# manoskary/analysisgnn

Hardware: AMD Instinct MI355X
Metric: subgraph-nodes/sec fwd+bwd, HybridGNN L=3 H=256 (higher is better)
Workload: dtype f32; 1 GPU; C2 (sampled, the batch a training step sees): HybridGNN L=3 H=256 out=128, 21 task heads, 32 neighbour-sampled subgraphs x (500 target notes + [5,5] hops) per GPU, per-hop counts passed (every layer trimmed); 16335 notes, 104099 edges per GPU; train step = fwd + objective (wloss) + bwd + allreduce + clip + AdamW, CSR rebuilt every step; hipGraph replay; workload_id=c2s, per_gpu_subgraphs=32, objective=wloss, parallelism=dp1, allreduce=none (one rank)

## Files before the change

### analysisgnn_amd/_lib.py

```python
from __future__ import annotations

import ctypes as C
import os
from typing import Optional, Sequence

import torch

from . import resident

_HERE = os.path.dirname(os.path.abspath(__file__))
LIB_PATH = os.path.join(_HERE, "libagnn_hip.so")
MAX_SEG = 32

SPMM_MEAN, SPMM_SKIP_SELF, SPMM_ACCUM = 1, 2, 4
INT32_MAX = 2 ** 31 - 1


class AgnnError(RuntimeError):
    pass


class CooSeg(C.Structure):
    _fields_ = [("row", C.c_void_p), ("col", C.c_void_p), ("etype", C.c_void_p),
                ("etype_code", C.c_int64), ("n_edges", C.c_int64), ("n_rows", C.c_int64)]


class RowendItem(C.Structure):
    _fields_ = [("rowptr", C.c_void_p), ("perm", C.c_void_p), ("rowend", C.c_void_p), ("n_rows", C.c_int32),
                ("e_limit", C.c_int32)]


ROWEND_MAX_ITEMS = 64


class Sampler(C.Structure):
    _fields_ = [("n_rel", C.c_int32), ("rowptr", C.c_void_p * 8), ("col", C.c_void_p * 8), ("win_start", C.c_void_p),
                ("n_sub", C.c_int32), ("n_targets", C.c_int32), ("n_hops", C.c_int32), ("fan", C.c_int32 * 4), ("cap", C.c_int32 * 4),
                ("rng", C.c_void_p), ("node_gid", C.c_void_p), ("edges", C.c_void_p * 8), ("e_cap", C.c_int64), ("status", C.c_void_p), ("drops", C.c_void_p), ("kept", C.c_void_p)]


class ReltItem(C.Structure):
    _fields_ = [("x", C.c_void_p), ("w", C.c_void_p), ("y", C.c_void_p), ("ld_x", C.c_int64), ("ld_y", C.c_int64)]


RELT_MAX_ITEMS = 4


class Rel(C.Structure):
    _fields_ = [("src", C.c_void_p), ("rowptr", C.c_void_p), ("rowend", C.c_void_p), ("col", C.c_void_p),
                ("ew", C.c_void_p), ("colscale", C.c_void_p), ("ld_src", C.c_int64)]


class HgtSrcItem(C.Structure):
    _fields_ = [("rowptr", C.c_void_p), ("rowend", C.c_void_p), ("col", C.c_void_p), ("perm", C.c_void_p), ("alpha", C.c_void_p),
                ("gs", C.c_void_p), ("dk", C.c_void_p), ("dv", C.c_void_p), ("ld_o", C.c_int64), ("n_src_rows", C.c_int32),
                ("col_limit", C.c_int32)]


class HgtDstItem(C.Structure):
    _fields_ = [("rels", C.c_void_p), ("n_rel", C.c_int32), ("q", C.c_void_p), ("ld_q", C.c_int64), ("n_rows", C.c_int64),
                ("out", C.c_void_p), ("ld_out", C.c_int64), ("m_out", C.c_void_p), ("linv_out", C.c_void_p)]


HGT_MAX_DST = 4


class HgtRel(C.Structure):
    _fields_ = [("k", C.c_void_p), ("v", C.c_void_p), ("rowptr", C.c_void_p), ("rowend", C.c_void_p),
                ("col", C.c_void_p), ("perm", C.c_void_p), ("pscale", C.c_void_p), ("ld", C.c_int64),
                ("alpha", C.c_void_p), ("gs", C.c_void_p), ("tdot", C.c_void_p), ("ld_tdot", C.c_int64)]


class Gated(C.Structure):
    _fields_ = [("rowptr", C.c_void_p), ("col", C.c_void_p), ("perm", C.c_void_p), ("a", C.c_void_p), ("b", C.c_void_p),
                ("h", C.c_void_p), ("c", C.c_void_p), ("ld", C.c_int64), ("ld_c", C.c_int64), ("n_rows", C.c_int64),
                ("H", C.c_int32)]


class WgradItem(C.Structure):
    _fields_ = [("dy", C.c_void_p), ("x", C.c_void_p), ("dw", C.c_void_p), ("db", C.c_void_p), ("ld_dy", C.c_int64), ("ld_x", C.c_int64),
                ("ld_dw", C.c_int64), ("n", C.c_int64), ("out_f", C.c_int32), ("in_f", C.c_int32)]


class ColsumItem(C.Structure):
    _fields_ = [("workspace", C.c_void_p), ("workspace_bytes", C.c_size_t), ("n", C.c_int64), ("H", C.c_int32), ("dgamma", C.c_void_p),
                ("dbeta", C.c_void_p)]


WGRAD_BATCH_MAX = 16
WGRAD_BATCH_MAX_ITEMS = 24
PACK_MAX_SRC = 8


class PackItem(C.Structure):
    _fields_ = [("dst", C.c_void_p), ("src", C.c_void_p * PACK_MAX_SRC), ("ld_dst", C.c_int64), ("ld_src", C.c_int64),
                ("rows", C.c_int32), ("cols", C.c_int32), ("n_src", C.c_int32), ("vec_ok", C.c_int32)]


LR_CONSTANT, LR_WARMUP_COSINE, LR_WARMUP_EXP = 0, 1, 2


class LrSchedule(C.Structure):
    _fields_ = [("kind", C.c_int32), ("warmup_steps", C.c_int32), ("count_offset", C.c_int32), ("swa_period", C.c_int32),
                ("swa_start", C.c_int64), ("swa_anneal", C.c_int32), ("base_lr", C.c_double), ("warmup_start_lr", C.c_double),
                ("eta_min", C.c_double), ("cos_a", C.c_double), ("cos_b", C.c_double), ("gamma", C.c_double),
                ("decay_steps", C.c_double), ("swa_lr", C.c_double)]


_lib: Optional[C.CDLL] = None

SIGNATURES = {
    "agnn_last_error": (C.c_char_p, []),
    "agnn_version": (C.c_int, []),
    "agnn_csr_workspace_bytes": (C.c_size_t, [C.c_int64, C.c_int64]),
    "agnn_csr_build": (C.c_int, [C.c_int, C.POINTER(CooSeg), C.c_void_p, C.c_void_p, C.c_void_p,
                                 C.c_void_p, C.c_size_t, C.c_void_p, C.c_void_p]),
    "agnn_check_status": (C.c_int, [C.c_void_p, C.c_void_p]),
    "agnn_csr_rowend": (C.c_int, [C.c_void_p, C.c_void_p, C.c_int64, C.c_int64, C.c_void_p, C.c_void_p]),
    "agnn_csr_rowend_batch": (C.c_int, [C.c_int, C.POINTER(RowendItem), C.c_void_p]),
    "agnn_spmm_f32": (C.c_int, [C.c_int, C.POINTER(Rel), C.c_int64, C.c_int32, C.c_void_p, C.c_int64,
                                C.c_int64, C.c_void_p, C.c_int64, C.c_void_p, C.c_int32, C.c_uint32,
                                C.c_void_p]),
    "agnn_spmm_root_f32": (C.c_int, [C.c_int, C.POINTER(Rel), C.c_int64, C.c_int32, C.c_void_p, C.c_int64,
                                     C.c_int64, C.c_void_p, C.c_int64, C.c_int64, C.c_void_p, C.c_int32, C.c_uint32,
                                     C.c_void_p]),
    "agnn_gru_fwd_f32": (C.c_int, [C.c_void_p, C.c_void_p, C.c_void_p, C.c_int64, C.c_int64, C.c_int32,
                                   C.c_void_p, C.c_void_p, C.c_void_p, C.c_void_p, C.c_void_p]),
    "agnn_gru_bwd_f32": (C.c_int, [C.c_void_p, C.c_void_p, C.c_void_p, C.c_void_p, C.c_int64, C.c_int64,
                                   C.c_int32, C.c_void_p, C.c_void_p, C.c_void_p, C.c_void_p, C.c_void_p]),
    "agnn_heads_fwd_f32": (C.c_int, [C.c_void_p, C.c_int64, C.c_int64, C.c_int32, C.c_int32, C.c_int32, C.c_void_p, C.c_void_p,
                                     C.c_void_p, C.c_void_p, C.c_float, C.c_void_p, C.c_void_p, C.c_void_p, C.POINTER(C.c_int32),
                                     C.c_void_p, C.c_void_p, C.c_int64, C.c_void_p, C.c_void_p, C.c_void_p, C.c_int64, C.c_void_p]),
    "agnn_gru_hprev_f32": (C.c_int, [C.c_void_p, C.c_int64, C.c_int64, C.c_int32, C.c_void_p, C.c_void_p]),
    "agnn_hgt_attn_fwd_multi_f32": (C.c_int, [C.c_int32, C.c_void_p, C.c_int32, C.c_int32, C.c_void_p]),
    "agnn_hgt_attn_fwd_f32": (C.c_int, [C.c_int, C.POINTER(HgtRel), C.c_void_p, C.c_int64, C.c_int64, C.c_int32,
                                        C.c_int32, C.c_void_p, C.c_int64, C.c_void_p, C.c_void_p, C.c_void_p]),
    "agnn_hgt_attn_bwd_dst_f32": (C.c_int, [C.c_int, C.POINTER(HgtRel), C.c_void_p, C.c_int64, C.c_void_p, C.c_int64,
                                            C.c_void_p, C.c_int64, C.c_void_p, C.c_void_p, C.c_int64, C.c_int32,
                                            C.c_int32, C.c_void_p, C.c_int64, C.c_void_p]),
    "agnn_hgt_attn_bwd_src_batch_f32": (C.c_int, [C.c_int32, C.POINTER(HgtSrcItem), C.c_void_p, C.c_int64, C.c_void_p, C.c_int64,
                                                  C.c_int32, C.c_int32, C.c_void_p]),
    "agnn_sampler_num_nodes": (C.c_int64, [C.POINTER(Sampler)]),
    "agnn_sampler_edge_capacity": (C.c_int64, [C.POINTER(Sampler)]),
    "agnn_sample_hops": (C.c_int, [C.POINTER(Sampler), C.c_void_p]),
    "agnn_sample_members": (C.c_int, [C.c_void_p, C.c_int64, C.c_void_p, C.c_void_p, C.c_void_p, C.c_int32, C.c_int32, C.c_int32,
                                      C.POINTER(C.c_int32), C.c_int32, C.c_void_p, C.c_void_p, C.c_void_p, C.c_void_p]),
    "agnn_sample_compact_nodes": (C.c_int64, [C.POINTER(Sampler), C.POINTER(C.c_int32)]),
    "agnn_sample_compact": (C.c_int, [C.POINTER(Sampler), C.POINTER(C.c_int32), C.c_void_p, C.c_void_p, C.c_void_p]),
    "agnn_gather_rows_f32": (C.c_int, [C.c_void_p, C.c_int64, C.c_void_p, C.c_int64, C.c_int32, C.c_void_p, C.c_int64, C.c_void_p]),
    "agnn_gather_i64": (C.c_int, [C.c_void_p, C.c_int64, C.c_void_p, C.c_int64, C.c_int32, C.c_int64, C.c_void_p, C.c_int64, C.c_void_p]),
    "agnn_relt_fwd_f32": (C.c_int, [C.c_int, C.POINTER(ReltItem), C.c_int32, C.c_int32, C.c_int32, C.c_int64, C.c_void_p]),
    "agnn_relt_bwd_f32": (C.c_int, [C.c_int, C.POINTER(ReltItem), C.c_int32, C.c_int32, C.c_int32, C.c_int64, C.c_void_p]),
    "agnn_relt_dw_workspace_bytes": (C.c_size_t, [C.c_int, C.c_int32, C.c_int32, C.c_int32, C.c_int64]),
    "agnn_relt_dw_f32": (C.c_int, [C.c_int, C.POINTER(ReltItem), C.c_int32, C.c_int32, C.c_int32, C.c_int64, C.c_void_p, C.c_size_t,
                                  C.c_void_p]),
    "agnn_wgrad_batch_workspace_bytes": (C.c_size_t, [C.c_int32, C.POINTER(WgradItem)]),
    "agnn_wgrad_batch_f32": (C.c_int, [C.c_int32, C.POINTER(WgradItem), C.c_void_p, C.c_size_t, C.c_void_p]),
    "agnn_gemm_nt_f32": (C.c_int, [C.c_void_p, C.c_int64, C.c_void_p, C.c_int64, C.c_void_p, C.c_int64, C.c_int32, C.c_int32, C.c_void_p,
                                   C.c_int64, C.c_void_p]),
    "agnn_gemm_nn_f32": (C.c_int, [C.c_void_p, C.c_int64, C.c_void_p, C.c_int64, C.c_void_p, C.c_int64, C.c_int32, C.c_int32, C.c_void_p,
                                   C.c_int64, C.c_void_p]),
    "agnn_gemm_nt2_f32": (C.c_int, [C.c_void_p, C.c_int64, C.c_int32, C.c_void_p, C.c_int64, C.c_int32, C.c_void_p, C.c_int64, C.c_void_p,
                                    C.c_int64, C.c_int32, C.c_void_p, C.c_int64, C.c_void_p]),
    "agnn_pool_cat_norm_f32": (C.c_int, [C.POINTER(Rel), C.c_void_p, C.c_int64, C.c_int64, C.c_int64, C.c_int32, C.c_int32, C.c_void_p,
                                         C.c_void_p, C.c_float, C.c_void_p, C.c_int64, C.c_void_p, C.c_int64, C.c_void_p, C.c_void_p,
                                         C.c_void_p, C.c_void_p]),
    "agnn_pool_cat_bwd_f32": (C.c_int, [C.POINTER(Rel), C.c_void_p, C.c_int64, C.c_void_p, C.c_int64, C.c_int64, C.c_int32, C.c_void_p,
                                        C.c_int64, C.c_void_p]),
    "agnn_absdiff_fwd_f32": (C.c_int, [C.c_void_p, C.c_void_p, C.c_void_p, C.c_int64, C.c_int64, C.c_int32, C.c_void_p, C.c_void_p, C.c_int64,
                                       C.c_void_p]),
    "agnn_absdiff_bwd_f32": (C.c_int, [C.c_void_p, C.c_void_p, C.c_void_p, C.c_int64, C.c_int64, C.c_int32, C.c_void_p, C.c_void_p, C.c_int64,
                                       C.c_int32, C.c_int32, C.c_void_p, C.c_int64, C.c_void_p]),
    "agnn_gated_fwd_f32": (C.c_int, [C.POINTER(Gated), C.c_void_p, C.c_int64, C.c_void_p]),
    "agnn_gated_bwd_dst_f32": (C.c_int, [C.POINTER(Gated), C.c_void_p, C.c_int64, C.c_void_p, C.c_void_p, C.c_void_p]),
    "agnn_gated_bwd_src_f32": (C.c_int, [C.POINTER(Gated), C.c_void_p, C.c_int64, C.c_void_p, C.c_void_p, C.c_void_p]),
    "agnn_norm_act_workspace_bytes": (C.c_size_t, [C.c_int32]),
    "agnn_norm_act_fwd_f32": (C.c_int, [C.c_void_p, C.c_int64, C.c_void_p, C.c_void_p, C.c_int32, C.c_int64, C.c_int32, C.c_float, C.c_float,
                                        C.c_uint32, C.c_void_p, C.c_uint32, C.c_void_p, C.c_int64, C.c_void_p, C.c_void_p, C.c_void_p,
                                        C.c_void_p]),
    "agnn_norm_act_bwd_f32": (C.c_int, [C.c_void_p, C.c_int64, C.c_void_p, C.c_void_p, C.c_int32, C.c_int64, C.c_int32, C.c_float, C.c_float,
                                        C.c_uint32, C.c_void_p, C.c_uint32, C.c_void_p, C.c_int64, C.c_void_p, C.c_void_p, C.c_void_p,
                                        C.c_int64, C.c_void_p, C.c_void_p, C.c_void_p, C.c_size_t, C.c_void_p]),
    "agnn_norm_act_colsum_batch_f32": (C.c_int, [C.c_int32, C.POINTER(ColsumItem), C.c_void_p]),
    "agnn_skip_act_workspace_bytes": (C.c_size_t, []),
    "agnn_skip_act_fwd_f32": (C.c_int, [C.c_void_p, C.c_int64, C.c_void_p, C.c_int64, C.c_void_p, C.c_int64, C.c_int32, C.c_float, C.c_uint32,
                                        C.c_void_p, C.c_uint32, C.c_void_p, C.c_int64, C.c_void_p, C.c_void_p]),
    "agnn_skip_act_bwd_f32": (C.c_int, [C.c_void_p, C.c_int64, C.c_void_p, C.c_int64, C.c_void_p, C.c_int64, C.c_int32, C.c_float, C.c_uint32,
                                        C.c_void_p, C.c_uint32, C.c_void_p, C.c_int64, C.c_void_p, C.c_int64, C.c_void_p, C.c_int64, C.c_void_p,
                                        C.c_void_p, C.c_size_t, C.c_void_p]),
    "agnn_norm_act_colsum_f32": (C.c_int, [C.c_void_p, C.c_size_t, C.c_int64, C.c_int32, C.c_void_p, C.c_void_p, C.c_void_p]),
    "agnn_wgrad_workspace_bytes": (C.c_size_t, [C.c_int64, C.c_int32, C.c_int32]),
    "agnn_wgrad_f32": (C.c_int, [C.c_void_p, C.c_int64, C.c_void_p, C.c_int64, C.c_int64, C.c_int32, C.c_int32, C.c_void_p,
                                 C.c_int64, C.c_void_p, C.c_void_p, C.c_size_t, C.c_void_p]),
    "agnn_pack_f32": (C.c_int, [C.c_int32, C.POINTER(PackItem), C.c_void_p]),
    "agnn_debug_stamp": (C.c_int, [C.c_void_p, C.c_void_p]),
    "agnn_gproj_fwd_f32": (C.c_int, [C.c_void_p, C.c_int64, C.c_void_p, C.c_void_p, C.c_void_p, C.c_int32, C.c_int32, C.c_int32,
                                     C.c_int64, C.c_void_p, C.c_int64, C.c_void_p]),
    "agnn_gproj_workspace_bytes": (C.c_size_t, [C.c_int64, C.c_int32, C.c_int32, C.c_int32]),
    "agnn_gproj_bwd_f32": (C.c_int, [C.c_void_p, C.c_int64, C.c_void_p, C.c_int64, C.c_void_p, C.c_void_p, C.c_int32, C.c_int32,
                                     C.c_int32, C.c_int32, C.c_int64, C.c_void_p, C.c_int64, C.c_void_p, C.c_void_p, C.c_void_p,
                                     C.c_size_t, C.c_void_p]),
    "agnn_spmm_self_grad_f32": (C.c_int, [C.c_void_p, C.c_int64, C.c_int64, C.c_int32, C.c_void_p, C.c_int64, C.c_int64, C.c_int32,
                                          C.c_void_p, C.c_int64, C.c_int32, C.c_void_p]),
    "agnn_embed_cat_fwd_f32": (C.c_int, [C.c_void_p, C.c_int64, C.c_int32, C.c_int64, C.c_int32, C.POINTER(C.c_void_p),
                                         C.POINTER(C.c_void_p), C.POINTER(C.c_int32), C.c_int32, C.c_void_p, C.c_int64, C.c_void_p]),
    "agnn_embed_workspace_bytes": (C.c_size_t, [C.c_int32, C.POINTER(C.c_int32), C.c_int32]),
    "agnn_embed_cat_bwd_f32": (C.c_int, [C.c_void_p, C.c_int64, C.c_int32, C.c_int64, C.c_int32, C.POINTER(C.c_void_p),
                                         C.POINTER(C.c_int32), C.c_int32, C.c_void_p, C.c_void_p, C.c_size_t, C.c_void_p]),
    "agnn_train_loss_workspace_bytes": (C.c_size_t, []),
    "agnn_train_loss_f32": (C.c_int, [C.c_void_p, C.c_int64, C.c_void_p, C.c_int32, C.c_void_p, C.c_int64, C.c_float, C.c_int64,
                                      C.c_void_p, C.c_int64, C.c_int32, C.c_float, C.c_void_p, C.c_float, C.c_void_p, C.c_void_p,
                                      C.c_void_p, C.c_void_p, C.c_void_p, C.c_void_p, C.c_void_p, C.c_void_p, C.c_size_t,
                                      C.c_void_p]),
    "agnn_train_loss_final_f32": (C.c_int, [C.c_void_p, C.c_int64, C.c_void_p, C.c_int32, C.c_void_p, C.c_int64, C.c_float, C.c_int64,
                                            C.c_void_p, C.c_int64, C.c_int32, C.c_float, C.c_void_p, C.c_float, C.c_void_p, C.c_void_p,
                                            C.c_void_p, C.c_void_p, C.c_void_p, C.c_void_p, C.c_void_p, C.c_void_p, C.c_int64, C.c_void_p,
                                            C.c_size_t, C.c_void_p]),
    "agnn_train_loss_bwd_f32": (C.c_int, [C.c_void_p, C.c_int64, C.c_void_p, C.c_int32, C.c_int64, C.c_int32, C.c_void_p, C.c_void_p,
                                          C.c_void_p, C.c_int64, C.c_void_p, C.c_int64, C.c_int32, C.c_float, C.c_void_p, C.c_int64,
                                          C.c_void_p]),
    "agnn_adamw_workspace_bytes": (C.c_size_t, []),
    "agnn_adamw_f32": (C.c_int, [C.c_void_p, C.c_void_p, C.c_void_p, C.c_void_p, C.c_int64, C.c_float, C.c_float, C.c_float,
                                 C.c_float, C.c_float, C.c_float, C.c_void_p, C.c_void_p, C.c_int32, C.c_void_p, C.c_size_t,
                                 C.c_void_p]),
    "agnn_lr_schedule_at": (C.c_double, [C.POINTER(LrSchedule), C.c_int64]),
    "agnn_adamw_sched_workspace_bytes": (C.c_size_t, []),
    "agnn_adamw_sched_f32": (C.c_int, [C.c_void_p, C.c_void_p, C.c_void_p, C.c_void_p, C.c_int64, C.POINTER(LrSchedule), C.c_float,
                                       C.c_float, C.c_float, C.c_float, C.c_float, C.c_void_p, C.c_void_p, C.c_void_p, C.c_void_p,
                                       C.c_int32, C.c_void_p, C.c_size_t, C.c_void_p]),
    "agnn_multitask_ce_f32": (C.c_int, [C.c_void_p, C.c_int64, C.c_void_p, C.c_int32, C.c_void_p, C.c_int64, C.c_float,
                                        C.c_int64, C.c_void_p, C.c_void_p, C.c_void_p, C.c_void_p, C.c_void_p]),
    "agnn_multitask_ce_scale_f32": (C.c_int, [C.c_void_p, C.c_int64, C.c_void_p, C.c_int32, C.c_int64, C.c_int32, C.c_void_p,
                                              C.c_void_p, C.c_int64, C.c_void_p]),
    "agnn_kd_workspace_bytes": (C.c_size_t, [C.c_int64, C.c_int32]),
    "agnn_multitask_kd_f32": (C.c_int, [C.c_void_p, C.c_int64, C.c_void_p, C.c_int64, C.c_void_p, C.c_void_p, C.c_int32, C.c_int64,
                                        C.c_int32, C.c_float, C.c_float, C.c_void_p, C.c_int64, C.c_void_p, C.c_void_p, C.c_void_p,
                                        C.c_size_t, C.c_void_p]),
    "agnn_ewc_workspace_bytes": (C.c_size_t, []),
    "agnn_ewc_f32": (C.c_int, [C.c_void_p, C.c_void_p, C.c_void_p, C.c_int64, C.c_float, C.c_void_p, C.c_void_p, C.c_void_p,
                               C.c_size_t, C.c_void_p]),
    "agnn_fisher_accum_f32": (C.c_int, [C.c_void_p, C.c_int64, C.c_float, C.c_void_p, C.c_void_p]),
    "agnn_eval_counts_len": (C.c_size_t, [C.c_int32, C.c_int32]),
    "agnn_multitask_eval_f32": (C.c_int, [C.c_void_p, C.c_int64, C.c_void_p, C.c_void_p, C.c_int32, C.c_int32, C.c_void_p, C.c_int64,
                                          C.c_int64, C.c_void_p, C.c_int32, C.c_uint32, C.c_void_p, C.c_void_p, C.c_void_p]),
}


def load() -> C.CDLL:
    global _lib
    if _lib is not None:
        return _lib
    if not os.path.exists(LIB_PATH):
        raise AgnnError(
            f"{LIB_PATH} not found: build it with `python -c 'import __graft_entry__ as g; g.build()'` "
            "(or `make -C analysisgnn_amd/csrc`). analysisgnn_amd has no CPU fallback.")
    lib = C.CDLL(LIB_PATH)
    for name, (res, args) in SIGNATURES.items():
        fn = getattr(lib, name)
        fn.restype = res
        fn.argtypes = args
    _lib = lib
    return lib


def check(rc: int, what: str) -> None:
    if rc != 0:
        msg = load().agnn_last_error()
        raise AgnnError(f"{what} failed ({rc}): {msg.decode() if msg else ''}")


def require_gpu(*tensors: Optional[torch.Tensor]) -> torch.device:
    dev = None
    for t in tensors:
        if t is None:
            continue
        if not t.is_cuda:
            raise AgnnError("analysisgnn_amd ops need tensors on a HIP device (no CPU fallback); "
                            f"got a tensor on {t.device}")
        if dev is None:
            dev = t.device
        elif t.device != dev:
            raise AgnnError(f"tensors on different devices: {dev} vs {t.device}")
    if dev is None:
        raise AgnnError("no tensor given")
    return dev


def status_word(device: torch.device) -> torch.Tensor:
    return resident.value(device, ("status word",), lambda: torch.zeros(1, dtype=torch.int32, device=device))


def check_device_status(device: torch.device) -> None:
    check(load().agnn_check_status(status_word(device).data_ptr(), stream_ptr(device)), "agnn_check_status")


def stream_ptr(device: torch.device) -> int:
    return torch.cuda.current_stream(device).cuda_stream


def ptr(t: Optional[torch.Tensor]) -> Optional[int]:
    return None if t is None else t.data_ptr()


def f32c(t: torch.Tensor) -> torch.Tensor:
    if t.dtype != torch.float32:
        raise AgnnError(f"fp32 expected, got {t.dtype}")
    if t.dim() != 2:
        raise AgnnError(f"2-D feature matrix expected, got shape {tuple(t.shape)}")
    if t.stride(1) != 1 or t.stride(0) % 4 != 0 or t.data_ptr() % 16 != 0 or (t.shape[0] > 1 and t.stride(0) < t.shape[1]):
        t = t.contiguous()
    return t


def make_rels(items: Sequence[dict]):
    arr = (Rel * len(items))()
    for i, it in enumerate(items):
        arr[i].src = it["src"]
        arr[i].rowptr = it["rowptr"]
        arr[i].rowend = it.get("rowend")
        arr[i].col = it["col"]
        arr[i].ew = it.get("ew")
        arr[i].colscale = it.get("colscale")
        arr[i].ld_src = it["ld_src"]
    return arr


STAMPS = {"on": bool(os.environ.get("AGNN_STAMPS")), "names": [], "buf": None,
          "only": [w for w in os.environ.get("AGNN_STAMPS", "").split(",") if w not in ("", "1", "all")]}


def stamp(name: str, device) -> None:
    if not STAMPS["on"] or (STAMPS["only"] and not any(w in name for w in STAMPS["only"])):
        return
    if STAMPS["buf"] is None:
        STAMPS["buf"] = torch.zeros(256, dtype=torch.int64, device=device)
    if name not in STAMPS["names"]:
        STAMPS["names"].append(name)
    k = STAMPS["names"].index(name)
    check(load().agnn_debug_stamp(STAMPS["buf"].data_ptr() + 8 * k, stream_ptr(torch.device(device))), "agnn_debug_stamp")
```

### analysisgnn_amd/csrc/pack.hip

```cpp
#include "agnn_common.h"

namespace {

struct PackTable {
  agnn_pack_item_t it[AGNN_PACK_MAX_ITEMS];
  int32_t first_block[AGNN_PACK_MAX_ITEMS + 1];
  int32_t n;
};

constexpr int kElemsPerBlock = 4096;

__global__ __launch_bounds__(256) void k_pack(PackTable t) {
  int i = 0;
  while (i + 1 < t.n && static_cast<int>(blockIdx.x) >= t.first_block[i + 1]) ++i;
  const agnn_pack_item_t& it = t.it[i];
  const int64_t total = static_cast<int64_t>(it.rows) * it.cols;
  const int64_t base = static_cast<int64_t>(blockIdx.x - t.first_block[i]) * kElemsPerBlock;
  const bool vec = (it.cols & 3) == 0 && it.vec_ok;
  if (vec) {
    const int c4 = it.cols >> 2;
#pragma unroll
    for (int u = 0; u < kElemsPerBlock / 1024; ++u) {
      const int64_t e = (base >> 2) + u * 256 + threadIdx.x;
      if (e >= (total >> 2)) break;
      const int64_t r = static_cast<uint32_t>(e) / static_cast<uint32_t>(c4);
      const int c = static_cast<int>(e - r * c4) * 4;
      float4 s = make_float4(0.f, 0.f, 0.f, 0.f);
      if (it.n_src > 0) s = *reinterpret_cast<const float4*>(it.src[0] + r * it.ld_src + c);
      for (int k = 1; k < it.n_src; ++k) {
        const float4 v = *reinterpret_cast<const float4*>(it.src[k] + r * it.ld_src + c);
        s.x += v.x; s.y += v.y; s.z += v.z; s.w += v.w;
      }
      *reinterpret_cast<float4*>(it.dst + r * it.ld_dst + c) = s;
    }
  } else {
#pragma unroll 4
    for (int u = 0; u < kElemsPerBlock / 256; ++u) {
      const int64_t e = base + u * 256 + threadIdx.x;
      if (e >= total) break;
      const int64_t r = static_cast<uint32_t>(e) / static_cast<uint32_t>(it.cols);
      const int c = static_cast<int>(e - r * it.cols);
      float s = it.n_src > 0 ? it.src[0][r * it.ld_src + c] : 0.f;
      for (int k = 1; k < it.n_src; ++k) s += it.src[k][r * it.ld_src + c];
      it.dst[r * it.ld_dst + c] = s;
    }
  }
}

}

extern "C" int agnn_pack_f32(int32_t n_items, const agnn_pack_item_t* items, agnn_stream_t stream_) {
  using namespace agnn;
  if (n_items < 0) return fail(AGNN_EINVAL, "pack: negative item count");
  if (n_items > 0 && !items) return fail(AGNN_EINVAL, "pack: null item table");
  hipStream_t s = static_cast<hipStream_t>(stream_);
  for (int32_t at = 0; at < n_items; at += AGNN_PACK_MAX_ITEMS) {
    PackTable t;
    t.n = 0;
    int32_t blocks = 0;
    for (int32_t i = at; i < n_items && t.n < AGNN_PACK_MAX_ITEMS; ++i) {
      agnn_pack_item_t it = items[i];
      if (it.rows < 0 || it.cols < 0 || it.n_src < 0 || it.n_src > AGNN_PACK_MAX_SRC)
        return fail(AGNN_EINVAL, "pack: item %d has rows=%d cols=%d n_src=%d", i, it.rows, it.cols, it.n_src);
      if (it.rows == 0 || it.cols == 0) continue;
      if (static_cast<int64_t>(it.rows) * it.cols >= (int64_t{1} << 31)) return fail(AGNN_EINVAL, "pack: item %d has 2^31 or more elements", i);
      if (!it.dst || it.ld_dst < it.cols || (it.n_src > 0 && it.ld_src < it.cols)) return fail(AGNN_EINVAL, "pack: item %d: null dst or ld < cols", i);
      if (it.n_src == 0) it.ld_src = it.ld_dst;
      bool v = aligned16(it.dst) && (it.ld_dst & 3) == 0 && (it.ld_src & 3) == 0;
      for (int k = 0; k < it.n_src; ++k) {
        if (!it.src[k]) return fail(AGNN_EINVAL, "pack: item %d: null source %d", i, k);
        v = v && aligned16(it.src[k]);
      }
      it.vec_ok = v ? 1 : 0;
      t.first_block[t.n] = blocks;
      const int64_t total = static_cast<int64_t>(it.rows) * it.cols;
      blocks += static_cast<int32_t>((total + kElemsPerBlock - 1) / kElemsPerBlock);
      t.it[t.n++] = it;
    }
    if (t.n == 0) continue;
    t.first_block[t.n] = blocks;
    hipLaunchKernelGGL(k_pack, dim3(blocks), dim3(256), 0, s, t);
    if (int rc = check_launch("pack")) return rc;
  }
  return AGNN_OK;
}

namespace {
__global__ void k_stamp(unsigned long long* slot) { *slot = wall_clock64(); }
}

extern "C" int agnn_debug_stamp(uint64_t* slot, agnn_stream_t stream_) {
  using namespace agnn;
  if (!slot) return fail(AGNN_EINVAL, "debug_stamp: null slot");
  hipLaunchKernelGGL(k_stamp, dim3(1), dim3(1), 0, static_cast<hipStream_t>(stream_), reinterpret_cast<unsigned long long*>(slot));
  return check_launch("debug_stamp");
}
```

### analysisgnn_amd/csrc/wgrad.hip

```cpp
#include "agnn_common.h"

namespace {

typedef float f32x16 __attribute__((ext_vector_type(16)));

struct WgArgs {
  const float* dy;
  const float* x;
  int64_t ld_dy, ld_x;
  int32_t n, out_f, in_f;
  int32_t rows_per_slice;
  int32_t tiles_in;
  float* slab;
  float* slab_b;
  int32_t out_pad, in_pad;
};

__device__ __forceinline__ void wgrad_tile(const WgArgs& a, const int tile, const int slice) {
  const int lane = threadIdx.x & 63;
  const int wave = threadIdx.x >> 6;
  const int wm = wave >> 1, wn = wave & 1;
  const int to = tile / a.tiles_in, ti = tile - to * a.tiles_in;
  const int kk = lane >> 5, c32 = lane & 31;
  const int ocol = to * 128 + wm * 64 + 2 * c32;
  const int icol = ti * 128 + wn * 64 + 2 * c32;
  const bool o_ok = ocol < a.out_f;
  const bool i_ok = icol < a.in_f;
  const int r0 = slice * a.rows_per_slice;
  int r1 = r0 + a.rows_per_slice;
  if (r1 > a.n) r1 = a.n;

  f32x16 acc00 = {0}, acc01 = {0}, acc10 = {0}, acc11 = {0};
  float bs0 = 0.f, bs1 = 0.f;
  const float* dy_s = a.dy + static_cast<int64_t>(r0) * a.ld_dy;
  const float* x_s = a.x + static_cast<int64_t>(r0) * a.ld_x;
  const uint32_t ldb_dy = static_cast<uint32_t>(a.ld_dy) * 4u, ldb_x = static_cast<uint32_t>(a.ld_x) * 4u;
  const uint32_t cb_dy = (o_ok ? ocol : 0) * 4u, cb_x = (i_ok ? icol : 0) * 4u;
  const int rel_last = a.n - 1 - r0;
  constexpr int CH = 8;
  constexpr int STEP = 2 * CH;
  float2 a0[CH], b0[CH], a1[CH], b1[CH], a2[CH], b2[CH];
  uint32_t o_dy = static_cast<uint32_t>(kk) * ldb_dy + cb_dy, o_x = static_cast<uint32_t>(kk) * ldb_x + cb_x;
  const uint32_t s_dy = 2u * ldb_dy, s_x = 2u * ldb_x;
  auto fetch_fast = [&](float2* ao, float2* bo) {
#pragma unroll
    for (int u = 0; u < CH; ++u) {
      ao[u] = *reinterpret_cast<const float2*>(reinterpret_cast<const char*>(dy_s) + o_dy);
      bo[u] = *reinterpret_cast<const float2*>(reinterpret_cast<const char*>(x_s) + o_x);
      o_dy += s_dy;
      o_x += s_x;
    }
    __builtin_amdgcn_sched_barrier(0);
  };
  auto fetch = [&](int chunk, float2* ao, float2* bo) {
#pragma unroll
    for (int u = 0; u < CH; ++u) {
      const uint32_t rel = static_cast<uint32_t>(min(chunk * STEP + 2 * u + kk, rel_last));
      ao[u] = *reinterpret_cast<const float2*>(reinterpret_cast<const char*>(dy_s) + (rel * ldb_dy + cb_dy));
      bo[u] = *reinterpret_cast<const float2*>(reinterpret_cast<const char*>(x_s) + (rel * ldb_x + cb_x));
    }
    o_dy += CH * s_dy;
    o_x += CH * s_x;
    __builtin_amdgcn_sched_barrier(0);
  };
  auto mma = [&](const float2* av, const float2* bv) {
#pragma unroll
    for (int u = 0; u < CH; ++u) {
      acc00 = __builtin_amdgcn_mfma_f32_32x32x2f32(av[u].x, bv[u].x, acc00, 0, 0, 0);
      acc01 = __builtin_amdgcn_mfma_f32_32x32x2f32(av[u].x, bv[u].y, acc01, 0, 0, 0);
      acc10 = __builtin_amdgcn_mfma_f32_32x32x2f32(av[u].y, bv[u].x, acc10, 0, 0, 0);
      acc11 = __builtin_amdgcn_mfma_f32_32x32x2f32(av[u].y, bv[u].y, acc11, 0, 0, 0);
      asm volatile("v_add_f32 %0, %0, %1" : "+v"(bs0) : "v"(av[u].x));
      asm volatile("v_add_f32 %0, %0, %1" : "+v"(bs1) : "v"(av[u].y));
    }
  };
  auto mma_tail = [&](int chunk, const float2* av, const float2* bv) {
#pragma unroll
    for (int u = 0; u < CH; ++u) {
      const float m = (r0 + chunk * STEP + 2 * u + kk < r1) ? 1.f : 0.f;
      const float ax = av[u].x * m, ay = av[u].y * m;
      acc00 = __builtin_amdgcn_mfma_f32_32x32x2f32(ax, bv[u].x, acc00, 0, 0, 0);
      acc01 = __builtin_amdgcn_mfma_f32_32x32x2f32(ax, bv[u].y, acc01, 0, 0, 0);
      acc10 = __builtin_amdgcn_mfma_f32_32x32x2f32(ay, bv[u].x, acc10, 0, 0, 0);
      acc11 = __builtin_amdgcn_mfma_f32_32x32x2f32(ay, bv[u].y, acc11, 0, 0, 0);
      bs0 += ax;
      bs1 += ay;
    }
  };
  const int nfull = (r1 - r0) / STEP;
  const int nchunks = (r1 - r0 + STEP - 1) / STEP;
  fetch(0, a0, b0);
  fetch(1, a1, b1);
  int c = 0;
  const int safe = (rel_last + 1) / STEP;
  for (; c + 3 <= nfull && c + 5 <= safe; c += 3) {
    fetch_fast(a2, b2);
    mma(a0, b0);
    fetch_fast(a0, b0);
    mma(a1, b1);
    fetch_fast(a1, b1);
    mma(a2, b2);
  }
  for (; c + 3 <= nfull; c += 3) {
    fetch(c + 2, a2, b2);
    mma(a0, b0);
    fetch(c + 3, a0, b0);
    mma(a1, b1);
    fetch(c + 4, a1, b1);
    mma(a2, b2);
  }
  fetch(c + 2, a2, b2);
  if (c < nchunks) mma_tail(c, a0, b0);
  if (c + 1 < nchunks) mma_tail(c + 1, a1, b1);
  if (c + 2 < nchunks) mma_tail(c + 2, a2, b2);
  float* slab = a.slab + (static_cast<int64_t>(slice) * a.out_pad) * a.in_pad;
  const int ob = to * 128 + wm * 64, ib = ti * 128 + wn * 64;
#pragma unroll
  for (int r = 0; r < 16; ++r) {
    const int i = (r & 3) + 8 * (r >> 2) + 4 * kk;
    float* row0 = slab + static_cast<int64_t>(ob + 2 * i) * a.in_pad + ib + 2 * c32;
    float* row1 = row0 + a.in_pad;
    *reinterpret_cast<float2*>(row0) = make_float2(acc00[r], acc01[r]);
    *reinterpret_cast<float2*>(row1) = make_float2(acc10[r], acc11[r]);
  }
  if (a.slab_b != nullptr && wn == 0) {
    bs0 += __shfl_xor(bs0, 32, 64);
    bs1 += __shfl_xor(bs1, 32, 64);
    if (kk == 0 && ti == 0)
      *reinterpret_cast<float2*>(a.slab_b + static_cast<int64_t>(slice) * a.out_pad + ocol) = make_float2(bs0, bs1);
  }
}

__global__ __launch_bounds__(256) void k_wgrad(WgArgs a) { wgrad_tile(a, blockIdx.x, blockIdx.y); }

constexpr int kWgBatchMax = 24;

struct WgBatch {
  WgArgs it[kWgBatchMax];
  int32_t first[kWgBatchMax + 1];
  int32_t tiles[kWgBatchMax];
  int32_t n;
};

__global__ __launch_bounds__(256) void k_wgrad_batch(WgBatch b) {
  int i = 0;
  const int blk = blockIdx.x;
  while (i + 1 < b.n && blk >= b.first[i + 1]) ++i;
  const int local = blk - b.first[i];
  const int tiles = b.tiles[i];
  const int slice = local / tiles;
  wgrad_tile(b.it[i], local - slice * tiles, slice);
}


__device__ __forceinline__ void wgrad_reduce_blocks(const float* __restrict__ slab, const float* __restrict__ slab_b, int S, int out_f, int in_f,
                                                    int out_pad, int in_pad, float* __restrict__ dw, int64_t ld_dw, float* __restrict__ db,
                                                    const int block, const int n_blocks) {
  __shared__ float2 part[8][32];
  const int col = threadIdx.x & 31, sg = threadIdx.x >> 5;
  const int half_in = in_f >> 1;
  const int64_t total = static_cast<int64_t>(out_f) * half_in;
  const int64_t plane = static_cast<int64_t>(out_pad) * in_pad;
  for (int64_t e0 = static_cast<int64_t>(block) * 32; e0 < total; e0 += static_cast<int64_t>(n_blocks) * 32) {
    const int64_t e = e0 + col;
    float2 s = make_float2(0.f, 0.f);
    int o = 0, i = 0;
    if (e < total) {
      o = static_cast<int>(e / half_in);
      i = static_cast<int>(e - static_cast<int64_t>(o) * half_in) * 2;
      const float* p = slab + static_cast<int64_t>(o) * in_pad + i;
      for (int k = sg; k < S; k += 8) {
        const float2 v = *reinterpret_cast<const float2*>(p + k * plane);
        s.x += v.x;
        s.y += v.y;
      }
    }
    part[sg][col] = s;
    __syncthreads();
    if (sg == 0 && e < total) {
      float2 t = part[0][col];
#pragma unroll
      for (int g = 1; g < 8; ++g) { t.x += part[g][col].x; t.y += part[g][col].y; }
      *reinterpret_cast<float2*>(dw + static_cast<int64_t>(o) * ld_dw + i) = t;
    }
    __syncthreads();
  }
  if (db != nullptr) {
    __shared__ float partb[8][32];
    for (int e0 = block * 32; e0 < out_f; e0 += n_blocks * 32) {
      const int e = e0 + col;
      float s = 0.f;
      if (e < out_f)
        for (int k = sg; k < S; k += 8) s += slab_b[static_cast<int64_t>(k) * out_pad + e];
      partb[sg][col] = s;
      __syncthreads();
      if (sg == 0 && e < out_f) {
        float t = partb[0][col];
#pragma unroll
        for (int g = 1; g < 8; ++g) t += partb[g][col];
        db[e] = t;
      }
      __syncthreads();
    }
  }
}

__global__ __launch_bounds__(256) void k_wgrad_reduce(const float* __restrict__ slab, const float* __restrict__ slab_b, int S,
                                                      int out_f, int in_f, int out_pad, int in_pad, float* __restrict__ dw,
                                                      int64_t ld_dw, float* __restrict__ db) {
  wgrad_reduce_blocks(slab, slab_b, S, out_f, in_f, out_pad, in_pad, dw, ld_dw, db, blockIdx.x, gridDim.x);
}

struct RedItem {
  const float* slab;
  const float* slab_b;
  float* dw;
  float* db;
  int64_t ld_dw;
  int32_t S, out_f, in_f, out_pad, in_pad;
};
struct RedBatch {
  RedItem it[kWgBatchMax];
  int32_t first[kWgBatchMax + 1];
  int32_t n;
};

__global__ __launch_bounds__(256) void k_wgrad_reduce_batch(RedBatch b) {
  int i = 0;
  const int blk = blockIdx.x;
  while (i + 1 < b.n && blk >= b.first[i + 1]) ++i;
  const RedItem& r = b.it[i];
  wgrad_reduce_blocks(r.slab, r.slab_b, r.S, r.out_f, r.in_f, r.out_pad, r.in_pad, r.dw, r.ld_dw, r.db, blk - b.first[i], b.first[i + 1] - b.first[i]);
}

struct Plan {
  int tiles_out, tiles_in, S, rows_per_slice, out_pad, in_pad;
};

Plan make_plan(int64_t n, int out_f, int in_f) {
  Plan p;
  p.tiles_out = (out_f + 127) / 128;
  p.tiles_in = (in_f + 127) / 128;
  p.out_pad = p.tiles_out * 128;
  p.in_pad = p.tiles_in * 128;
  const int tiles = p.tiles_out * p.tiles_in;
  int64_t S = 512 / tiles;
  const int64_t max_s = (n + 63) / 64;
  if (S > max_s) S = max_s;
  if (S > 64) S = 64;
  if (S < 1) S = 1;
  int64_t rps = (n + S - 1) / S;
  rps = (rps + 1) & ~int64_t{1};
  p.rows_per_slice = static_cast<int>(rps);
  p.S = static_cast<int>((n + rps - 1) / rps);
  return p;
}

}

int agnn::launch_slab_reduce(const float* slab, const float* slab_b, int S, int out_f, int in_f, int out_pad, int in_pad,
                             float* dw, int64_t ld_dw, float* db, hipStream_t s) {
  const int64_t total = static_cast<int64_t>(out_f) * (in_f >> 1);
  int blocks = static_cast<int>((total + 31) / 32);
  if (blocks > 4096) blocks = 4096;
  if (blocks < 1) blocks = 1;
  hipLaunchKernelGGL(k_wgrad_reduce, dim3(blocks), dim3(256), 0, s, slab, slab_b, S, out_f, in_f, out_pad, in_pad, dw, ld_dw, db);
  return check_launch("slab_reduce");
}

extern "C" size_t agnn_wgrad_workspace_bytes(int64_t n, int32_t out_f, int32_t in_f) {
  if (n <= 0 || out_f <= 0 || in_f <= 0) return 0;
  const Plan p = make_plan(n, out_f, in_f);
  return (static_cast<size_t>(p.S) * p.out_pad * p.in_pad + static_cast<size_t>(p.S) * p.out_pad) * sizeof(float) + 256;
}

extern "C" int agnn_wgrad_f32(const float* dy, int64_t ld_dy, const float* x, int64_t ld_x, int64_t n, int32_t out_f,
                              int32_t in_f, float* dw, int64_t ld_dw, float* db, void* workspace, size_t workspace_bytes,
                              agnn_stream_t stream_) {
  using namespace agnn;
  if (n <= 0 || n >= (int64_t{1} << 31) || out_f <= 0 || in_f <= 0) return fail(AGNN_EINVAL, "wgrad: bad sizes n=%lld out=%d in=%d", (long long)n, out_f, in_f);
  if ((out_f & 1) || (in_f & 1) || (ld_dy & 1) || (ld_x & 1) || (ld_dw & 1)) return fail(AGNN_EALIGN, "wgrad: widths and leading dimensions must be even");
  if (!dy || !x || !dw || !workspace) return fail(AGNN_EINVAL, "wgrad: null argument");
  if ((reinterpret_cast<uintptr_t>(dy) | reinterpret_cast<uintptr_t>(x) | reinterpret_cast<uintptr_t>(dw) | reinterpret_cast<uintptr_t>(db)) & 7u)
    return fail(AGNN_EALIGN, "wgrad: pointers must be 8-byte aligned");
  if (ld_dy < out_f || ld_x < in_f || ld_dw < in_f) return fail(AGNN_EINVAL, "wgrad: leading dimension smaller than the width");
  const size_t need = agnn_wgrad_workspace_bytes(n, out_f, in_f);
  if (workspace_bytes < need) return fail(AGNN_ENOMEM, "wgrad: workspace %zu < %zu bytes", workspace_bytes, need);
  const Plan p = make_plan(n, out_f, in_f);
  if ((static_cast<int64_t>(p.rows_per_slice) + 128) * (ld_dy > ld_x ? ld_dy : ld_x) * 4 >= (int64_t{1} << 32))
    return fail(AGNN_EINVAL, "wgrad: a row slice (%d rows x ld) exceeds the kernel's 32-bit byte offsets", p.rows_per_slice);
  char* ws = reinterpret_cast<char*>((reinterpret_cast<uintptr_t>(workspace) + 255) & ~uintptr_t{255});
  float* slab = reinterpret_cast<float*>(ws);
  float* slab_b = slab + static_cast<size_t>(p.S) * p.out_pad * p.in_pad;
  WgArgs a{dy, x, ld_dy, ld_x, static_cast<int32_t>(n), out_f, in_f, p.rows_per_slice, p.tiles_in, slab,
           db ? slab_b : nullptr, p.out_pad, p.in_pad};
  hipStream_t s = static_cast<hipStream_t>(stream_);
  hipLaunchKernelGGL(k_wgrad, dim3(p.tiles_out * p.tiles_in, p.S), dim3(256), 0, s, a);
  if (int rc = check_launch("wgrad")) return rc;
  return launch_slab_reduce(slab, db ? slab_b : nullptr, p.S, out_f, in_f, p.out_pad, p.in_pad, dw, ld_dw, db, s);
}

namespace {
struct BatchPlan {
  int n;
  int tiles_out[kWgBatchMax], tiles_in[kWgBatchMax], S[kWgBatchMax], rps[kWgBatchMax];
  size_t slab_off[kWgBatchMax], slabb_off[kWgBatchMax], total_floats;
};

int batch_plan(int n_items, const agnn_wgrad_item_t* items, BatchPlan& bp) {
  using namespace agnn;
  if (n_items <= 0 || n_items > kWgBatchMax || !items) return fail(AGNN_EINVAL, "wgrad_batch: %d items (1 .. %d)", n_items, kWgBatchMax);
  bp.n = n_items;
  int64_t tiles = 0;
  for (int i = 0; i < n_items; ++i) {
    const agnn_wgrad_item_t& it = items[i];
    if (it.n <= 0 || it.n >= (int64_t{1} << 31) || it.out_f <= 0 || it.in_f <= 0) return fail(AGNN_EINVAL, "wgrad_batch: item %d: bad sizes", i);
    bp.tiles_out[i] = (it.out_f + 127) / 128;
    bp.tiles_in[i] = (it.in_f + 127) / 128;
    tiles += static_cast<int64_t>(bp.tiles_out[i]) * bp.tiles_in[i];
  }
  int64_t S = 384 / tiles;
  if (S > 64) S = 64;
  if (S < 1) S = 1;
  size_t off = 0;
  for (int i = 0; i < n_items; ++i) {
    const agnn_wgrad_item_t& it = items[i];
    int64_t s_i = S;
    const int64_t max_s = (it.n + 63) / 64;
    if (s_i > max_s) s_i = max_s;
    int64_t rps = (it.n + s_i - 1) / s_i;
    rps = (rps + 1) & ~int64_t{1};
    bp.rps[i] = static_cast<int>(rps);
    bp.S[i] = static_cast<int>((it.n + rps - 1) / rps);
    const size_t plane = static_cast<size_t>(bp.tiles_out[i]) * 128 * bp.tiles_in[i] * 128;
    bp.slab_off[i] = off;
    off += static_cast<size_t>(bp.S[i]) * plane;
    bp.slabb_off[i] = off;
    off += static_cast<size_t>(bp.S[i]) * bp.tiles_out[i] * 128;
    off = (off + 63) & ~size_t{63};
  }
  bp.total_floats = off;
  return AGNN_OK;
}
}

extern "C" size_t agnn_wgrad_batch_workspace_bytes(int32_t n_items, const agnn_wgrad_item_t* items) {
  BatchPlan bp;
  if (batch_plan(n_items, items, bp) != AGNN_OK) return 0;
  return bp.total_floats * sizeof(float) + 256;
}

extern "C" int agnn_wgrad_batch_f32(int32_t n_items, const agnn_wgrad_item_t* items, void* workspace, size_t workspace_bytes,
                                    agnn_stream_t stream_) {
  using namespace agnn;
  BatchPlan bp;
  if (int rc = batch_plan(n_items, items, bp)) return rc;
  if (!workspace || workspace_bytes < bp.total_floats * sizeof(float) + 256) return fail(AGNN_ENOMEM, "wgrad_batch: workspace too small");
  float* ws = reinterpret_cast<float*>((reinterpret_cast<uintptr_t>(workspace) + 255) & ~uintptr_t{255});
  WgBatch wb{};
  RedBatch rb{};
  wb.n = rb.n = n_items;
  int wg = 0, red = 0;
  for (int i = 0; i < n_items; ++i) {
    const agnn_wgrad_item_t& it = items[i];
    if ((it.out_f & 1) || (it.in_f & 1) || (it.ld_dy & 1) || (it.ld_x & 1) || (it.ld_dw & 1)) return fail(AGNN_EALIGN, "wgrad_batch: item %d: widths and leading dimensions must be even", i);
    if (!it.dy || !it.x || !it.dw) return fail(AGNN_EINVAL, "wgrad_batch: item %d: null argument", i);
    if ((reinterpret_cast<uintptr_t>(it.dy) | reinterpret_cast<uintptr_t>(it.x) | reinterpret_cast<uintptr_t>(it.dw) | reinterpret_cast<uintptr_t>(it.db)) & 7u)
      return fail(AGNN_EALIGN, "wgrad_batch: item %d: pointers must be 8-byte aligned", i);
    if (it.ld_dy < it.out_f || it.ld_x < it.in_f || it.ld_dw < it.in_f) return fail(AGNN_EINVAL, "wgrad_batch: item %d: leading dimension smaller than the width", i);
    if ((static_cast<int64_t>(bp.rps[i]) + 128) * (it.ld_dy > it.ld_x ? it.ld_dy : it.ld_x) * 4 >= (int64_t{1} << 32))
      return fail(AGNN_EINVAL, "wgrad_batch: item %d: a row slice (%d rows x ld) exceeds the kernel's 32-bit byte offsets", i, bp.rps[i]);
    const int out_pad = bp.tiles_out[i] * 128, in_pad = bp.tiles_in[i] * 128;
    float* slab = ws + bp.slab_off[i];
    float* slab_b = ws + bp.slabb_off[i];
    wb.it[i] = WgArgs{it.dy, it.x, it.ld_dy, it.ld_x, static_cast<int32_t>(it.n), it.out_f, it.in_f, bp.rps[i], bp.tiles_in[i], slab,
                      it.db ? slab_b : nullptr, out_pad, in_pad};
    wb.tiles[i] = bp.tiles_out[i] * bp.tiles_in[i];
    wb.first[i] = wg;
    wg += wb.tiles[i] * bp.S[i];
    rb.it[i] = RedItem{slab, it.db ? slab_b : nullptr, it.dw, it.db, it.ld_dw, bp.S[i], it.out_f, it.in_f, out_pad, in_pad};
    rb.first[i] = red;
    int64_t blocks = (static_cast<int64_t>(it.out_f) * (it.in_f >> 1) + 31) / 32;
    if (blocks > 1024) blocks = 1024;
    red += static_cast<int>(blocks);
  }
  wb.first[n_items] = wg;
  rb.first[n_items] = red;
  hipStream_t s = static_cast<hipStream_t>(stream_);
  hipLaunchKernelGGL(k_wgrad_batch, dim3(static_cast<unsigned>(wg)), dim3(256), 0, s, wb);
  if (int rc = check_launch("wgrad_batch")) return rc;
  hipLaunchKernelGGL(k_wgrad_reduce_batch, dim3(static_cast<unsigned>(red)), dim3(256), 0, s, rb);
  return check_launch("wgrad_batch(reduce)");
}
```

### analysisgnn_amd/dp.py

```python
from __future__ import annotations

import os
from typing import Iterable, List, Optional, Sequence

import torch
import torch.distributed as dist


def init_distributed(backend: Optional[str] = None) -> tuple:
    world = int(os.environ.get("WORLD_SIZE", "1"))
    rank = int(os.environ.get("RANK", "0"))
    local = int(os.environ.get("LOCAL_RANK", "0"))
    if world > 1 and not dist.is_initialized():
        os.environ.setdefault("MASTER_ADDR", "127.0.0.1")
        os.environ.setdefault("MASTER_PORT", "29500")
        if backend is None:
            backend = os.environ.get("AGNN_DIST_BACKEND") or ("nccl" if torch.cuda.is_available() else "gloo")
        if backend == "nccl":
            torch.cuda.set_device(local)
            dist.init_process_group(backend, rank=rank, world_size=world, device_id=torch.device("cuda", local))
        else:
            dist.init_process_group(backend, rank=rank, world_size=world)
    return rank, local, world


def shard_units(n_units: int, rank: int, world: int) -> List[int]:
    return list(range(rank, n_units, world))


def _aligned_offsets(sizes: Sequence[int], align: int = 4, tight: Optional[Sequence[bool]] = None) -> List[int]:
    offs, end = [], 0
    for i, k in enumerate(sizes):
        start = end if (tight is not None and tight[i] and i > 0) else (end + align - 1) // align * align
        offs.append(start)
        end = start + k
    offs.append((end + align - 1) // align * align)
    return offs


def plan_parameters(model: torch.nn.Module, late: Iterable[torch.nn.Parameter] = ()):
    groups = []
    for m in model.modules():
        fn = getattr(m, "adjacent_parameter_groups", None)
        if fn is not None:
            groups.extend([[p for p in g] for g in fn()])
    late_ids = {id(p) for p in late}
    seen, params, tight = set(), [], set()
    for g in groups:
        if any(id(p) in late_ids for p in g):
            raise ValueError("plan_parameters: an adjacency group cannot hold late parameters")
        g = [p for p in g if p.requires_grad and id(p) not in seen]
        for i, p in enumerate(g):
            seen.add(id(p))
            params.append(p)
            if i > 0:
                tight.add(id(p))
    for want_late in (False, True):
        for p in model.parameters():
            if p.requires_grad and id(p) not in seen and (id(p) in late_ids) == want_late:
                seen.add(id(p))
                params.append(p)
    return params, tight


class FlatGradBuffer:

    def __init__(self, params: Iterable[torch.nn.Parameter], views: bool = True, tight: Optional[set] = None,
                 late: Iterable[torch.nn.Parameter] = ()):
        self.params: List[torch.nn.Parameter] = [p for p in params if p.requires_grad]
        if not self.params:
            raise ValueError("no trainable parameters")
        dev = self.params[0].device
        self.sizes = [p.numel() for p in self.params]
        self.offsets = _aligned_offsets(self.sizes, tight=[tight is not None and id(p) in tight for p in self.params])
        n = self.offsets[-1]
        self.views = views
        for p in self.params:
            if p.dtype != torch.float32 or p.device != dev:
                raise ValueError("FlatGradBuffer: fp32 parameters on one device expected")
        self.flat = torch.zeros(n, dtype=torch.float32, device=dev)
        self._pad = torch.zeros(4, dtype=torch.float32, device=dev)
        self._none = torch.zeros(max(self.sizes) if self.sizes else 1, dtype=torch.float32, device=dev)
        late_ids = {id(p) for p in late}
        self.n_early = len(self.params)
        if late_ids:
            flags = [id(p) in late_ids for p in self.params]
            self.n_early = flags.index(True) if True in flags else len(flags)
            if not all(flags[self.n_early:]) or sum(flags) != len(late_ids):
                raise ValueError("FlatGradBuffer: the late parameters must be the last ones of the buffer (dp.plan_parameters(model, late=...))")
        self.cut = self.offsets[self.n_early]
        if views:
            self._assign_views()

    def _assign_views(self) -> None:
        for p, k, o in zip(self.params, self.sizes, self.offsets):
            p.grad = self.flat[o:o + k].view_as(p)

    def zero(self) -> None:
        if self.views:
            self.flat.zero_()
        else:
            for p in self.params:
                p.grad = None
            self._packed = set()

    def pack(self, part: Optional[str] = None) -> None:
        from .linear import join_wgrad
        join_wgrad()
        if self.views:
            return
        done = getattr(self, "_packed", set())
        if not isinstance(done, set):
            done = {"early", "late"} if done else set()
        for name, lo, hi in (("early", 0, self.n_early), ("late", self.n_early, len(self.params))):
            if (part is not None and part != name) or name in done or lo == hi:
                done.add(name) if lo == hi else None
                continue
            parts = []
            for i in range(lo, hi):
                p, k, o, o_next = self.params[i], self.sizes[i], self.offsets[i], self.offsets[i + 1]
                parts.append(p.grad.reshape(-1) if p.grad is not None else self._none[:k])
                if o_next - o > k:
                    parts.append(self._pad[: o_next - o - k])
            torch.cat(parts, out=self.flat[self.offsets[lo]:self.offsets[hi]])
            for i in range(lo, hi):
                p, k, o = self.params[i], self.sizes[i], self.offsets[i]
                p.grad = self.flat[o:o + k].view_as(p)
            done.add(name)
        self._packed = done

    def all_reduce_mean(self, world: Optional[int] = None) -> None:
        self.pack()
        if dist.is_initialized() and dist.get_world_size() > 1:
            dist.all_reduce(self.flat, op=dist.ReduceOp.SUM)
            self.flat.div_(dist.get_world_size())

    def all_reduce_early_async(self):
        self.pack("early")
        if dist.is_initialized() and dist.get_world_size() > 1 and self.cut > 0:
            return dist.all_reduce(self.flat[:self.cut], op=dist.ReduceOp.SUM, async_op=True)
        return None

    def all_reduce_late_and_finish(self, work) -> None:
        self.pack("late")
        if dist.is_initialized() and dist.get_world_size() > 1:
            if self.cut < self.flat.numel():
                dist.all_reduce(self.flat[self.cut:], op=dist.ReduceOp.SUM)
            if work is not None:
                work.wait()
            self.flat.div_(dist.get_world_size())

    def clip_norm_(self, max_norm: float) -> torch.Tensor:
        total = torch.linalg.vector_norm(self.flat)
        self.flat.mul_(torch.clamp(max_norm / (total + 1e-6), max=1.0))
        return total


class LRSchedule:
    FIELDS = ("kind", "warmup_steps", "count_offset", "base_lr", "warmup_start_lr", "eta_min", "cos_a", "cos_b", "gamma", "decay_steps")

    def __init__(self, kind: int, base_lr: float, warmup_steps: int = 0, count_offset: int = 0, warmup_start_lr: float = 0.0,
                 eta_min: float = 0.0, cos_a: float = 0.0, cos_b: float = 1.0, gamma: float = 1.0, decay_steps: float = 1.0):
        self.kind, self.warmup_steps, self.count_offset = int(kind), int(warmup_steps), int(count_offset)
        self.base_lr, self.warmup_start_lr, self.eta_min = float(base_lr), float(warmup_start_lr), float(eta_min)
        self.cos_a, self.cos_b, self.gamma, self.decay_steps = float(cos_a), float(cos_b), float(gamma), float(decay_steps)
        self.lr_at(0)

    @classmethod
    def constant(cls, lr: float) -> "LRSchedule":
        from . import _lib
        return cls(_lib.LR_CONSTANT, lr)

    @classmethod
    def warmup_cosine(cls, base_lr: float, warmup_steps: int, total_steps: int, eta_min: float = 0.0) -> "LRSchedule":
        from . import _lib
        return cls(_lib.LR_WARMUP_COSINE, base_lr, warmup_steps, 0, 0.0, eta_min, cos_a=warmup_steps, cos_b=total_steps)

    @classmethod
    def reference_cosine(cls, base_lr: float, warmup_steps: int, max_epochs: int, eta_min: float = 0.0,
                         warmup_start_lr: float = 0.0) -> "LRSchedule":
        from . import _lib
        if warmup_steps < 3:
            raise ValueError(f"reference_cosine: warmup_steps={warmup_steps}: the reference's class fails for warm-ups shorter than 3 "
                             "steps (it reads steps_per_epoch before its third step() call has set it)")
        return cls(_lib.LR_WARMUP_COSINE, base_lr, warmup_steps, 1, warmup_start_lr, eta_min, cos_a=warmup_steps / 3.0, cos_b=max_epochs)

    @classmethod
    def reference_exponential(cls, base_lr: float, warmup_steps: int, decay_steps: int, gamma: float = 0.999, eta_min: float = 0.0,
                              warmup_start_lr: float = 0.0) -> "LRSchedule":
        from . import _lib
        return cls(_lib.LR_WARMUP_EXP, base_lr, warmup_steps, 1, warmup_start_lr, eta_min, gamma=gamma, decay_steps=decay_steps)

    def to_dict(self) -> dict:
        return {k: getattr(self, k) for k in self.FIELDS}

    @classmethod
    def from_dict(cls, d: dict) -> "LRSchedule":
        return cls(**{k: d[k] for k in cls.FIELDS})

    def struct(self, swa: Optional["SWA"] = None):
        from . import _lib
        s = _lib.LrSchedule(**self.to_dict())
        s.swa_start, s.swa_period, s.swa_anneal, s.swa_lr = -1, 1, 0, 0.0
        if swa is not None:
            s.swa_start, s.swa_period, s.swa_anneal, s.swa_lr = swa.start_step, swa.period, swa.anneal_epochs, swa.swa_lr
        return s

    def lr_at(self, k: int, swa: Optional["SWA"] = None) -> float:
        import ctypes
        import math
        from . import _lib
        lib = _lib.load()
        lr = float(lib.agnn_lr_schedule_at(ctypes.byref(self.struct(swa)), int(k)))
        if math.isnan(lr):
            raise _lib.AgnnError(f"agnn_lr_schedule_at failed: {(lib.agnn_last_error() or b'').decode()}")
        return lr


class SWA:

    def __init__(self, start_step: int, period: int, anneal_epochs: int = 10, swa_lr: float = 5e-5):
        if start_step < 0 or period <= 0 or anneal_epochs < 0:
            raise ValueError(f"SWA: start_step={start_step}, period={period}, anneal_epochs={anneal_epochs}")
        self.start_step, self.period, self.anneal_epochs, self.swa_lr = int(start_step), int(period), int(anneal_epochs), float(swa_lr)

    def to_dict(self) -> dict:
        return dict(start_step=self.start_step, period=self.period, anneal_epochs=self.anneal_epochs, swa_lr=self.swa_lr)


class FlatAdamW:

    def __init__(self, params: Iterable[torch.nn.Parameter], grads: FlatGradBuffer, lr=1e-3, betas=(0.9, 0.999),
                 eps=1e-8, weight_decay=1e-2, swa: Optional[SWA] = None):
        self.params = [p for p in params if p.requires_grad]
        assert [id(p) for p in self.params] == [id(p) for p in grads.params], "same parameter order as the gradient buffer"
        self.grads = grads
        self.lr, self.betas, self.eps, self.wd = lr, betas, eps, weight_decay
        dev = self.params[0].device
        self.flat = torch.zeros(grads.offsets[-1], dtype=torch.float32, device=dev)
        for p, o in zip(self.params, grads.offsets):
            self.flat[o:o + p.numel()] = p.detach().reshape(-1)
            p.data = self.flat[o:o + p.numel()].view_as(p)
        self.m = torch.zeros_like(self.flat)
        self.v = torch.zeros_like(self.flat)
        self.schedule = lr if isinstance(lr, LRSchedule) else None
        self.swa = swa
        if self.schedule is None:
            if swa is not None:
                raise ValueError("FlatAdamW: swa needs lr=LRSchedule (LRSchedule.constant(lr) for a fixed rate)")
            return
        self._sched = self.schedule.struct(swa)
        self._t = torch.zeros((), dtype=torch.float32, device=dev)
        self._state = torch.zeros(2, dtype=torch.float32, device=dev)
        self._state[0] = self.schedule.lr_at(0, swa)
        self.last_norm = torch.zeros((), dtype=torch.float32, device=dev)
        self.swa_flat = torch.zeros_like(self.flat) if swa is not None else None
        if self.flat.is_cuda:
            from . import _lib
            self._ws = torch.empty(int(_lib.load().agnn_adamw_sched_workspace_bytes()), dtype=torch.uint8, device=dev)

    @property
    def last_lr(self) -> torch.Tensor:
        return self._scheduled("last_lr")._state[0]

    @property
    def n_averaged(self) -> torch.Tensor:
        return self._scheduled("n_averaged")._state[1]

    def current_lr(self) -> float:
        if self.schedule is None:
            return float(self.lr)
        return self.schedule.lr_at(int(self._t.item()), self.swa)

    def _scheduled(self, what: str) -> "FlatAdamW":
        if self.schedule is None:
            raise AttributeError(f"FlatAdamW.{what} needs lr=LRSchedule")
        return self

    @torch.no_grad()
    def swap_swa_(self) -> None:
        if self.swa is None:
            raise AttributeError("FlatAdamW.swap_swa_ needs swa=SWA(...)")
# ... 123 lines not shown
```

### analysisgnn_amd/fused.py

```python
from __future__ import annotations

import itertools
from typing import Optional

import torch
import torch.nn as nn
import torch.nn.functional as F

from . import _lib, resident
from .linear import ColsumItem, all_steal, defer, deferring, leaf_refs

PRE_RELU, POST_RELU = 1, 2
ENABLED = True
_CALL_IDS = itertools.count(1)


def rng_state(device) -> torch.Tensor:
    return resident.value(device, ("dropout counter",), lambda: torch.tensor([int(torch.initial_seed()) & 0x7FFFFFFFFFFFFFFF, 0],
                                                                             dtype=torch.int64, device=device))


def advance_rng(device) -> None:
    rng_state(device)[1:2].add_(1)


def _al16(t: torch.Tensor) -> torch.Tensor:
    return t if t.data_ptr() % 16 == 0 else t.clone()


class _NormAct(torch.autograd.Function):
    @staticmethod
    def forward(ctx, x, gamma, beta, eps, p, flags, call_id, seg=0, defer_ok=False, steal_refs=None, pre=None):
        dev = _lib.require_gpu(x, gamma, beta)
        ctx.defer_ok = bool(defer_ok) or (gamma.is_leaf and beta.is_leaf)
        ctx.steal_refs = leaf_refs(gamma, beta) if steal_refs is None else tuple(steal_refs)
        lib = _lib.load()
        x = x if (x.stride(1) == 1 and x.stride(0) % 4 == 0 and x.data_ptr() % 16 == 0) else x.contiguous()
        n, H = x.shape
        seg = int(seg) if seg else H
        rng = rng_state(dev) if p > 0 else None
        used = torch.empty(2, dtype=torch.int64, device=dev) if p > 0 else None
        gamma, beta = _al16(gamma.contiguous()), _al16(beta.contiguous())
        if pre is not None:
            y, mean, rstd = pre
        else:
            y = torch.empty((n, H), dtype=torch.float32, device=dev)
            mean = torch.empty((max(n, 1) * (H // seg),), dtype=torch.float32, device=dev)
            rstd = torch.empty((max(n, 1) * (H // seg),), dtype=torch.float32, device=dev)
            _lib.check(lib.agnn_norm_act_fwd_f32(x.data_ptr(), x.stride(0), gamma.data_ptr(), beta.data_ptr(), seg, n, H, float(eps), float(p),
                                                 int(flags), _lib.ptr(rng), int(call_id), y.data_ptr(), y.stride(0), mean.data_ptr(),
                                                 rstd.data_ptr(), _lib.ptr(used), _lib.stream_ptr(dev)), "agnn_norm_act_fwd_f32")
        ctx.save_for_backward(x, gamma, beta, mean, rstd, *([used] if used is not None else []))
        ctx.cfg = (float(eps), float(p), int(flags), int(call_id), seg)
        return y

    @staticmethod
    def backward(ctx, dy):
        x, gamma, beta, mean, rstd, *used = ctx.saved_tensors
        eps, p, flags, call_id, seg = ctx.cfg
        dev = dy.device
        lib = _lib.load()
        dy = dy if (dy.stride(1) == 1 and dy.stride(0) % 4 == 0 and dy.data_ptr() % 16 == 0) else dy.contiguous()
        n, H = x.shape
        dx = torch.empty_like(x)
        dgamma = torch.empty_like(gamma)
        dbeta = torch.empty_like(beta)
        nws = int(lib.agnn_norm_act_workspace_bytes(H))
        ws = torch.empty(nws, dtype=torch.uint8, device=dev)
        rng = used[0] if p > 0 else None
        later = ctx.defer_ok and deferring(dy) and all_steal(ctx.steal_refs)
        _lib.check(lib.agnn_norm_act_bwd_f32(x.data_ptr(), x.stride(0), gamma.data_ptr(), beta.data_ptr(), seg, n, H, eps, p, flags,
                                             _lib.ptr(rng), call_id, dy.data_ptr(), dy.stride(0), mean.data_ptr(), rstd.data_ptr(),
                                             dx.data_ptr(), dx.stride(0), None if later else dgamma.data_ptr(),
                                             None if later else dbeta.data_ptr(), ws.data_ptr(), nws, _lib.stream_ptr(dev)),
                   "agnn_norm_act_bwd_f32")
        if later:
            dg_k, db_k = dgamma.detach(), dbeta.detach()
            defer(ColsumItem(ws, n, H, dg_k, db_k), dev)
        return dx, dgamma, dbeta, None, None, None, None, None, None, None, None


def _ok16(t: torch.Tensor) -> bool:
    return t.dtype == torch.float32 and t.dim() == 2 and t.stride(1) == 1 and t.stride(0) % 4 == 0 and t.data_ptr() % 16 == 0


class _SkipAct(torch.autograd.Function):

    @staticmethod
    def forward(ctx, o, x, skip, relu: bool, p: float, call_id: int):
        dev = _lib.require_gpu(o)
        lib = _lib.load()
        o = o if _ok16(o) else o.float().contiguous()
        if x is not None:
            x = x if _ok16(x) else x.float().contiguous()
        n, H = o.shape
        z = torch.empty((n, H), dtype=torch.float32, device=dev)
        rng = rng_state(dev) if p > 0 else None
        used = torch.empty(2, dtype=torch.int64, device=dev) if p > 0 else None
        sk = skip.detach().reshape(-1)[:1].contiguous() if skip is not None else None
        flags = 1 if relu else 0
        _lib.check(lib.agnn_skip_act_fwd_f32(_lib.ptr(x), x.stride(0) if x is not None else 0, o.data_ptr(), o.stride(0), _lib.ptr(sk), n, H,
                                             float(p), flags, _lib.ptr(rng), int(call_id), z.data_ptr(), z.stride(0), _lib.ptr(used),
                                             _lib.stream_ptr(dev)), "agnn_skip_act_fwd_f32")
        ctx.save_for_backward(o, *([x, sk] if x is not None else []), *([used] if used is not None else []))
        ctx.cfg = (bool(relu), float(p), int(call_id), x is not None, tuple(skip.shape) if skip is not None else None)
        ctx.set_materialize_grads(False)
        return z

    @staticmethod
    def backward(ctx, dz):
        if dz is None:
            return None, None, None, None, None, None
        relu, p, call_id, has_x, skip_shape = ctx.cfg
        saved = list(ctx.saved_tensors)
        o = saved.pop(0)
        x, sk = (saved.pop(0), saved.pop(0)) if has_x else (None, None)
        used = saved.pop(0) if p > 0 else None
        dev = dz.device
        lib = _lib.load()
        dz = dz if _ok16(dz) else dz.float().contiguous()
        n, H = o.shape
        do = torch.empty_like(o)
        want_dx = has_x and ctx.needs_input_grad[1]
        want_ds = has_x and ctx.needs_input_grad[2]
        dx = torch.empty((n, H), dtype=torch.float32, device=dev) if want_dx else None
        ds = torch.empty(1, dtype=torch.float32, device=dev) if want_ds else None
        ws = resident.scratch(dev, "skip_act", int(lib.agnn_skip_act_workspace_bytes()), zeroed=True) if want_ds else None
        _lib.check(lib.agnn_skip_act_bwd_f32(_lib.ptr(x), x.stride(0) if has_x else 0, o.data_ptr(), o.stride(0), _lib.ptr(sk), n, H, p,
                                             1 if relu else 0, _lib.ptr(used), call_id, dz.data_ptr(), dz.stride(0), _lib.ptr(dx),
                                             dx.stride(0) if dx is not None else 0, do.data_ptr(), do.stride(0), _lib.ptr(ds), _lib.ptr(ws),
                                             int(lib.agnn_skip_act_workspace_bytes()) if ws is not None else 0, _lib.stream_ptr(dev)),
                   "agnn_skip_act_bwd_f32")
        return do, dx, (ds.reshape(skip_shape) if ds is not None else None), None, None, None


def skip_act(o: torch.Tensor, x: Optional[torch.Tensor], skip: Optional[torch.Tensor], relu: bool, p: float, training: bool) -> torch.Tensor:
    p = float(p) if training else 0.0
    if not (ENABLED and o.is_cuda and o.dim() == 2 and o.shape[1] % 4 == 0 and o.shape[1] <= 2048 and o.shape[0] > 0 and
            (x is None or tuple(x.shape) == tuple(o.shape))):
        y = o if x is None else torch.lerp(x, o, torch.sigmoid(skip))
        y = F.relu(y) if relu else y
        return F.dropout(y, p, True) if p > 0 else y
    if x is None and not relu and p == 0.0:
        return o
    return _SkipAct.apply(o, x, skip if x is not None else None, relu, p, next(_CALL_IDS) & 0xFFFFFFFF)


def norm_act(x: torch.Tensor, ln: nn.LayerNorm, pre_relu: bool = False, post_relu: bool = False, p: float = 0.0,
             training: bool = False, pre=None) -> torch.Tensor:
    H = x.shape[-1]
    usable = (ENABLED and x.is_cuda and x.dtype == torch.float32 and H % 4 == 0 and H <= 1024 and ln.elementwise_affine
              and tuple(ln.normalized_shape) == (H,))
    if pre is not None:
        if not usable or pre_relu or post_relu or (p > 0 and training) or x.dim() != 2:
            raise _lib.AgnnError("norm_act: precomputed results stand for a plain LayerNorm on the kernel path")
        if not (torch.is_grad_enabled() and (x.requires_grad or ln.weight.requires_grad or ln.bias.requires_grad)):
            return pre[0]
        return _NormAct.apply(x, ln.weight, ln.bias, ln.eps, 0.0, 0, next(_CALL_IDS) & 0xFFFFFFFF, 0, False, None, pre)
    if not usable:
        y = F.relu(x) if pre_relu else x
        y = ln(y)
        y = F.relu(y) if post_relu else y
        return F.dropout(y, p, training)
    x2 = x.reshape(-1, H)
    flags = (PRE_RELU if pre_relu else 0) | (POST_RELU if post_relu else 0)
    y = _NormAct.apply(x2, ln.weight, ln.bias, ln.eps, p if training else 0.0, flags, next(_CALL_IDS) & 0xFFFFFFFF)
    return y.view(x.shape)


def grouped_norm_act(x: torch.Tensor, gamma: torch.Tensor, beta: torch.Tensor, eps: float, pre_relu: bool = False, pre=None) -> torch.Tensor:
    N, G, H = x.shape
    W = G * H
    gl = H // 4
    ok = (ENABLED and x.is_cuda and x.dtype == torch.float32 and H % 4 == 0 and 256 % H == 0 and (gl & (gl - 1)) == 0 and W <= 2048)
    if not ok:
        if pre is not None:
            raise _lib.AgnnError("grouped_norm_act: precomputed results need the kernel path")
        y = F.relu(x) if pre_relu else x
        return F.layer_norm(y, (H,), None, None, eps) * gamma + beta
    view_only = all(t.is_leaf or getattr(t, "_agnn_wgrad_deferrable", False) for t in (gamma, beta))
    y = _NormAct.apply(x.reshape(N, W), gamma.reshape(W), beta.reshape(W), eps, 0.0, PRE_RELU if pre_relu else 0,
                       next(_CALL_IDS) & 0xFFFFFFFF, H, view_only, leaf_refs(gamma, beta), pre)
    return y.view(N, G, H)


class FusedSequential(nn.Sequential):

    def forward(self, x, pre=None):
        mods = list(self)
        i = 0
        if pre is not None:
            if not mods or not isinstance(mods[0], nn.LayerNorm) or (len(mods) > 1 and isinstance(mods[1], (nn.ReLU, nn.Dropout))):
                raise _lib.AgnnError("FusedSequential: precomputed results need a leading plain LayerNorm")
            x = norm_act(x, mods[0], pre=pre)
            i = 1
        while i < len(mods):
            m = mods[i]
            nxt = mods[i + 1] if i + 1 < len(mods) else None
            nn2 = mods[i + 2] if i + 2 < len(mods) else None
            if isinstance(m, nn.ReLU) and isinstance(nxt, nn.LayerNorm):
                p, used = (nn2.p, 3) if isinstance(nn2, nn.Dropout) else (0.0, 2)
                x = norm_act(x, nxt, pre_relu=True, p=p, training=self.training)
                i += used
            elif isinstance(m, nn.LayerNorm):
                post = isinstance(nxt, nn.ReLU)
                d = mods[i + 1 + int(post)] if i + 1 + int(post) < len(mods) else None
                p = d.p if isinstance(d, nn.Dropout) else 0.0
                x = norm_act(x, m, post_relu=post, p=p, training=self.training)
                i += 1 + int(post) + int(isinstance(d, nn.Dropout))
            else:
                x = m(x)
                i += 1
        return x
```

### analysisgnn_amd/gru.py

```python
from __future__ import annotations

import torch
import torch.nn as nn
import torch.nn.functional as F

from . import _lib, resident
from .linear import (WgItem, all_steal, defer, defer_home, deferring, leaf_refs, mark_wgrad_async, weight_grad, weight_grad_batch,
                     wgrad_stream)

KERNEL_HIDDEN = (64, 128)


YIELD_TO_PROJECTIONS = True
PROJECTION_EVENTS: list = []


def wait_for_projections(device) -> None:
    device = torch.device(device)
    if device.type != "cuda":
        return
    idx = device.index if device.index is not None else torch.cuda.current_device()
    mine = [e for e in PROJECTION_EVENTS if e[0] == idx]
    PROJECTION_EVENTS[:] = [e for e in PROJECTION_EVENTS if e[0] != idx]
    for _, ev in mine:
        torch.cuda.current_stream(device).wait_event(ev)


class _GRULayer(torch.autograd.Function):
    @staticmethod
    def forward(ctx, x, w_ih, w_hh, b_ih, b_hh, last_in_backward=False, drop_scale=None):
        ctx.last_in_backward = bool(last_in_backward)
        dev = _lib.require_gpu(x, w_ih, w_hh, b_ih, b_hh)
        B, T, I = x.shape
        Hh = w_hh.shape[2]
        x2 = x.reshape(B * T, I)
        gi = torch.addmm(b_ih.reshape(-1), x2, w_ih.reshape(6 * Hh, I).t())
        dev_idx = dev.index if dev.index is not None else torch.cuda.current_device()
        if last_in_backward:
            PROJECTION_EVENTS[:] = [e for e in PROJECTION_EVENTS if e[0] != dev_idx]
        elif YIELD_TO_PROJECTIONS:
            ev = torch.cuda.Event()
            ev.record(torch.cuda.current_stream(dev))
            PROJECTION_EVENTS.append((dev_idx, ev))
        w_hh_c = w_hh.contiguous()
        b_hh_c = b_hh.contiguous()
        y = torch.empty((B, T, 2 * Hh), dtype=torch.float32, device=dev)
        saved = torch.empty((B, T, 2, 4, Hh), dtype=torch.float32, device=dev)
        lib = _lib.load()
        out = y
        if drop_scale is not None:
            if tuple(drop_scale.shape) != (B, T, 2 * Hh) or drop_scale.dtype != torch.float32 or not drop_scale.is_contiguous():
                raise _lib.AgnnError("gru: drop_scale must be a contiguous fp32 [B, T, 2*hidden] tensor")
            out = torch.empty_like(y)
        _lib.check(lib.agnn_gru_fwd_f32(gi.data_ptr(), w_hh_c.data_ptr(), b_hh_c.data_ptr(), B, T, Hh,
                                        y.data_ptr(), saved.data_ptr(), _lib.ptr(drop_scale), out.data_ptr() if drop_scale is not None else None,
                                        _lib.stream_ptr(dev)), "agnn_gru_fwd_f32")
        ctx.save_for_backward(x2, w_ih, w_hh_c, y, saved, *([drop_scale] if drop_scale is not None else []))
        ctx.dims = (B, T, I, Hh)
        ctx.wg_async = all(getattr(t, "_agnn_wgrad_async", False) or t.is_leaf for t in (w_ih, w_hh, b_ih, b_hh))
        ctx.steal_refs = leaf_refs(w_ih, w_hh, b_ih, b_hh)
        return out

    @staticmethod
    def backward(ctx, dy):
        x2, w_ih, w_hh, y, saved, *drop = ctx.saved_tensors
        drop_scale = drop[0] if drop else None
        B, T, I, Hh = ctx.dims
        dev = dy.device
        dy = dy.contiguous()
        dgi = torch.empty((B, T, 2, 3 * Hh), dtype=torch.float32, device=dev)
        dgh = torch.empty((B, T, 2, 3 * Hh), dtype=torch.float32, device=dev)
        hp = torch.empty((B, T, 2, Hh), dtype=torch.float32, device=dev)
        lib = _lib.load()
        _lib.check(lib.agnn_gru_bwd_f32(dy.data_ptr(), y.data_ptr(), saved.data_ptr(), w_hh.data_ptr(), B, T, Hh,
                                        dgi.data_ptr(), dgh.data_ptr(), _lib.ptr(drop_scale), hp.data_ptr(), _lib.stream_ptr(dev)), "agnn_gru_bwd_f32")
        dgi2 = dgi.view(B * T, 6 * Hh)
        wf = w_ih.reshape(6 * Hh, I)
        dx = (dgi2 @ wf).view(B, T, I) if ctx.needs_input_grad[0] else None
        dw_ih = torch.empty((6 * Hh, I), dtype=torch.float32, device=dev)
        db_ih = torch.empty((6 * Hh,), dtype=torch.float32, device=dev)
        dw_hh = torch.empty((2, 3 * Hh, Hh), dtype=torch.float32, device=dev)
        db_hh = torch.empty((2, 3 * Hh), dtype=torch.float32, device=dev)

        def weight_grads():
            items = []
            if I % 2 == 0:
                items.append(WgItem(dgi2, x2, True, dw_ih, db_ih))
            else:
                dw, db = weight_grad(dgi2, x2, True)
                dw_ih.copy_(dw)
                db_ih.copy_(db)
            dgh2, hp2 = dgh.view(B * T, 6 * Hh), hp.view(B * T, 2 * Hh)
            for d in range(2):
                items.append(WgItem(dgh2[:, d * 3 * Hh:(d + 1) * 3 * Hh], hp2[:, d * Hh:(d + 1) * Hh], True, dw_hh[d], db_hh[d]))
            weight_grad_batch(items)

        off_chain = ctx.wg_async and all_steal(ctx.steal_refs)

        def forked():
            with wgrad_stream(dev, dgi, dgh, y, x2, hp, dw_ih, db_ih, dw_hh, db_hh, active=off_chain, kind="sequence"):
                weight_grads()
        if ctx.last_in_backward and off_chain and deferring(dy):
            defer(forked, dev)
        elif not (off_chain and deferring(dy) and defer_home(weight_grads, dev, (dgi, dgh, y, x2, hp, dw_ih, db_ih, dw_hh, db_hh))):
            forked()
        return dx, dw_ih.view(2, 3 * Hh, I), dw_hh, db_ih.view(2, 3 * Hh), db_hh, None, None


def kernel_applicable(rnn: nn.GRU) -> bool:
    return (isinstance(rnn, nn.GRU) and rnn.hidden_size in KERNEL_HIDDEN and rnn.bidirectional and rnn.batch_first
            and rnn.bias and getattr(rnn, "proj_size", 0) == 0)


def gru_forward(rnn: nn.GRU, x: torch.Tensor, training: bool) -> torch.Tensor:
    _lib.require_gpu(x)
    if not kernel_applicable(rnn):
        return rnn(x)[0]
    y = x
    stacked = _stack_gru_params(rnn)
    for layer in range(rnn.num_layers):
        w_ih, w_hh, b_ih, b_hh = stacked[4 * layer:4 * layer + 4]
        drop = None
        if layer < rnn.num_layers - 1 and rnn.dropout > 0 and training:
            B, T = y.shape[0], y.shape[1]
            drop = F.dropout(_ones((B, T, 2 * rnn.hidden_size), y.device), rnn.dropout, True)
        y = _GRULayer.apply(y.contiguous(), w_ih, w_hh, b_ih, b_hh, layer == 0, drop)
    return y


def _ones(shape, device) -> torch.Tensor:
    return resident.value(device, ("ones", tuple(shape)), lambda: torch.ones(shape, dtype=torch.float32, device=device), fill=True)


class _StackPairs(torch.autograd.Function):

    @staticmethod
    def forward(ctx, *params):
        from .params import pack
        dev = params[0].device
        outs, items = [], []
        for i in range(0, len(params), 2):
            a, b = params[i], params[i + 1]
            o = torch.empty((2,) + tuple(a.shape), dtype=torch.float32, device=dev)
            outs.append(o)
            for k, src in enumerate((a, b)):
                src = src.detach()
                items.append((o[k].reshape(1, -1) if src.dim() == 1 else o[k], [src.reshape(1, -1) if src.dim() == 1 else src]))
        pack(items, dev)
        return tuple(outs)

    @staticmethod
    def backward(ctx, *grads):
        out = []
        for g in grads:
            out.extend(g.unbind(0))
        return tuple(out)


def _stack_gru_params(rnn: nn.GRU):
    names = ("weight_ih", "weight_hh", "bias_ih", "bias_hh")
    flat = []
    for layer in range(rnn.num_layers):
        for n in names:
            flat.append(getattr(rnn, f"{n}_l{layer}"))
            flat.append(getattr(rnn, f"{n}_l{layer}_reverse"))
    from .params import adjacent, stack_rows
    if all(adjacent(flat[i:i + 2]) for i in range(0, len(flat), 2)):
        outs = tuple(stack_rows(flat[i:i + 2]) for i in range(0, len(flat), 2))
        leaves = all(t.is_leaf for t in flat)
    elif flat[0].is_cuda and all(t.is_contiguous() and t.dtype == torch.float32 for t in flat):
        outs = _StackPairs.apply(*flat)
        leaves = all(t.is_leaf for t in flat)
    else:
        outs = tuple(torch.stack((flat[i], flat[i + 1])) for i in range(0, len(flat), 2))
        leaves = all(t.is_leaf for t in flat)
    if leaves:
        for i, o in enumerate(outs):
            mark_wgrad_async(o, leaves=flat[2 * i:2 * i + 2])
    return outs
```

### analysisgnn_amd/heads.py

```python
from __future__ import annotations

from typing import Dict, List, Optional, Sequence, Tuple

import torch
import torch.nn as nn
import torch.nn.functional as F

from . import _lib, resident
from .fused import grouped_norm_act
from .linear import all_steal, defer, deferring, leaf_refs, linear, mark_wgrad_async, wgrad_stream
from .params import cat_rows, stack_rows


def fused_head_logits(clf_dict: nn.ModuleDict, x: torch.Tensor, tasks: Sequence[str]) -> Tuple[torch.Tensor, List[int]]:
    mods = [clf_dict[t] for t in tasks]
    T = len(mods)
    h2 = mods[0][0].out_features
    W1 = _cat_params([m[0].weight for m in mods])
    b1 = _cat_params([m[0].bias for m in mods])
    gamma = _cat_params([m[2].weight for m in mods], stack=True)
    beta = _cat_params([m[2].bias for m in mods], stack=True)
    offs = [0]
    for m in mods:
        offs.append(offs[-1] + m[3].out_features)
    b2 = _cat_params([m[3].bias for m in mods])
    eps = mods[0][2].eps
    if (HEADS_FUSED and x.is_cuda and x.dim() == 2 and x.dtype == torch.float32 and x.shape[1] == HEADS_IN and h2 == HEADS_HIDDEN
            and T <= _lib.MAX_SEG and x.shape[0] > 0 and x.shape[0] * max(T * h2, offs[-1]) < 2 ** 30 - 2 ** 20):
        W2 = _cat_params([m[3].weight for m in mods])
        z, y, mean, rstd, logits = heads_forward(x, W1, b1, gamma, beta, eps, W2, b2, offs, h2)
        a = linear(x, W1, b1, pre=[z])
        a = grouped_norm_act(a.view(-1, T, h2), gamma, beta, eps, pre_relu=True, pre=[y, mean, rstd])
        return grouped_projection(a.reshape(-1, T * h2), W2, b2, offs, h2, pre=[logits]), offs
    a = linear(x, W1, b1)
    a = grouped_norm_act(a.view(-1, T, h2), gamma, beta, eps, pre_relu=True)
    a = a.reshape(-1, T * h2)
    if a.is_cuda and h2 in GPROJ_K and T <= _lib.MAX_SEG and GPROJ_ENABLED:
        W2 = _cat_params([m[3].weight for m in mods])
        logits = grouped_projection(a, W2, b2, offs, h2)
    else:
        W2 = torch.block_diag(*[m[3].weight for m in mods])
        logits = linear(a, W2, b2)
    return logits, offs


def _cat_params(ps, stack: bool = False) -> torch.Tensor:
    ps = list(ps)
    t = stack_rows(ps) if stack else cat_rows(ps)
    return mark_wgrad_async(t, deferrable=True, leaves=ps) if all(p.is_leaf for p in ps) else t


HEADS_FUSED = False
HEADS_IN, HEADS_HIDDEN = 128, 64
_OFFS_HOST: dict = {}


def heads_forward(x, W1, b1, gamma, beta, eps, W2, b2, offs, h2):
    dev = _lib.require_gpu(x, W1, W2)
    with torch.no_grad():
        xc = x.detach()
        xc = xc if (xc.stride(1) == 1 and xc.stride(0) % 4 == 0 and xc.data_ptr() % 16 == 0) else xc.contiguous()
        al = lambda t: t if (t.is_contiguous() and t.data_ptr() % 16 == 0) else t.contiguous().clone()
        w1, w2 = al(W1.detach()), al(W2.detach())
        c = lambda t: t.detach().reshape(-1).contiguous()
        T = len(offs) - 1
        N = xc.shape[0]
        key = tuple(int(o) for o in offs)
        oh = _OFFS_HOST.get(key)
        if oh is None:
            oh = _OFFS_HOST[key] = (_lib.C.c_int32 * len(key))(*key)
        z = torch.empty((N, T * h2), dtype=torch.float32, device=dev)
        y = torch.empty((N, T * h2), dtype=torch.float32, device=dev)
        mean = torch.empty((N * T,), dtype=torch.float32, device=dev)
        rstd = torch.empty((N * T,), dtype=torch.float32, device=dev)
        logits = torch.empty((N, key[-1]), dtype=torch.float32, device=dev)
        b2c = c(b2) if b2 is not None else None
        _lib.check(_lib.load().agnn_heads_fwd_f32(xc.data_ptr(), xc.stride(0), N, xc.shape[1], h2, T, w1.data_ptr(), c(b1).data_ptr(),
                                                  c(gamma).data_ptr(), c(beta).data_ptr(), float(eps), w2.data_ptr(), _lib.ptr(b2c),
                                                  _offs_tensor(offs, dev).data_ptr(), oh, z.data_ptr(), y.data_ptr(), z.stride(0),
                                                  mean.data_ptr(), rstd.data_ptr(), logits.data_ptr(), logits.stride(0),
                                                  _lib.stream_ptr(dev)), "agnn_heads_fwd_f32")
    return z, y, mean, rstd, logits


GPROJ_K = (32, 64, 128)
GPROJ_ENABLED = True


def _offs_tensor(offs: Sequence[int], device) -> torch.Tensor:
    return resident.value(device, ("offset table", tuple(offs)), lambda: torch.tensor(list(offs), dtype=torch.int32, device=device))


class _GroupedProj(torch.autograd.Function):
    @staticmethod
    def forward(ctx, a, w, b, offs_t, offs, K, pre=None):
        dev = _lib.require_gpu(a, w, offs_t)
        ctx._wg_async_in = all(t is None or t.is_leaf or getattr(t, "_agnn_wgrad_async", False) for t in (w, b))
        ctx._wg_defer_in = all(t is None or t.is_leaf or getattr(t, "_agnn_wgrad_deferrable", False) for t in (w, b))
        ctx.steal_refs = leaf_refs(w, b)
        a = _lib.f32c(a)
        w = _lib.f32c(w)
        if w.data_ptr() % 16:
            w = w.clone()
        G = len(offs) - 1
        sum_c = offs[-1]
        tiles = sum((offs[i + 1] - offs[i] + 31) // 32 for i in range(G))
        N = a.shape[0]
        if pre is not None:
            out = pre[0]
        else:
            out = torch.empty((N, sum_c), dtype=torch.float32, device=dev)
            lib = _lib.load()
            bb = b.float().contiguous() if b is not None else None
            _lib.check(lib.agnn_gproj_fwd_f32(a.data_ptr(), a.stride(0), w.data_ptr(), _lib.ptr(bb), offs_t.data_ptr(), G, K, tiles, N,
                                              out.data_ptr(), out.stride(0), _lib.stream_ptr(dev)), "agnn_gproj_fwd_f32")
        ctx.save_for_backward(a, w, offs_t)
        ctx.meta = (G, K, tiles, sum_c, b is not None)
        ctx.wg_async = ctx._wg_async_in
        ctx.wg_defer = ctx._wg_defer_in
        return out

    @staticmethod
    def backward(ctx, dout):
        a, w, offs_t = ctx.saved_tensors
        G, K, tiles, sum_c, has_b = ctx.meta
        dev = a.device
        dout = _lib.f32c(dout)
        N = a.shape[0]
        lib = _lib.load()
        need_w = ctx.needs_input_grad[1] or (has_b and ctx.needs_input_grad[2])
        dw = db = None
        if need_w:
            dw = torch.empty_like(w)
            db = torch.empty((sum_c,), dtype=torch.float32, device=dev) if has_b else None
            dw_k, db_k = dw.detach(), (db.detach() if db is not None else None)

            def weight_grads():
                nws = int(lib.agnn_gproj_workspace_bytes(N, sum_c, K, tiles))
                ws = torch.empty(max(nws, 1), dtype=torch.uint8, device=dev)
                _lib.check(lib.agnn_gproj_bwd_f32(dout.data_ptr(), dout.stride(0), a.data_ptr(), a.stride(0), w.data_ptr(),
                                                  offs_t.data_ptr(), G, K, tiles, sum_c, N, None, 0, dw_k.data_ptr(), _lib.ptr(db_k),
                                                  ws.data_ptr(), nws, _lib.stream_ptr(dev)), "agnn_gproj_bwd_f32")
            off_chain = ctx.wg_async and all_steal(ctx.steal_refs)
            if off_chain and ctx.wg_defer and deferring(dout):
                defer(weight_grads, dev)
            else:
                with wgrad_stream(dev, dout, a, dw_k, db_k, active=off_chain):
                    weight_grads()
        da = None
        if ctx.needs_input_grad[0]:
            da = torch.empty_like(a)
            _lib.check(lib.agnn_gproj_bwd_f32(dout.data_ptr(), dout.stride(0), a.data_ptr(), a.stride(0), w.data_ptr(),
                                              offs_t.data_ptr(), G, K, tiles, sum_c, N, da.data_ptr(), da.stride(0), None, None,
                                              None, 0, _lib.stream_ptr(dev)), "agnn_gproj_bwd_f32")
        return da, dw, db, None, None, None, None


def grouped_projection(a: torch.Tensor, w: torch.Tensor, b: Optional[torch.Tensor], offs: Sequence[int], K: int, pre=None) -> torch.Tensor:
    return _GroupedProj.apply(a, w, b, _offs_tensor(offs, a.device), tuple(int(o) for o in offs), int(K), pre)


class _GroupedInProj(torch.autograd.Function):

    @staticmethod
    def forward(ctx, x, w, offs_t, offs, K):
        dev = _lib.require_gpu(x, w, offs_t)
        x = _lib.f32c(x)
        w = _lib.f32c(w)
        if w.data_ptr() % 16:
            w = w.clone()
        G = len(offs) - 1
        sum_c = offs[-1]
        tiles = sum((offs[i + 1] - offs[i] + 31) // 32 for i in range(G))
        N = x.shape[0]
        out = torch.empty((N, G * K), dtype=torch.float32, device=dev)
        lib = _lib.load()
        _lib.check(lib.agnn_gproj_bwd_f32(x.data_ptr(), x.stride(0), out.data_ptr(), out.stride(0), w.data_ptr(), offs_t.data_ptr(), G, K,
                                          tiles, sum_c, N, out.data_ptr(), out.stride(0), None, None, None, 0, _lib.stream_ptr(dev)),
                   "agnn_gproj_bwd_f32(dx as forward)")
        ctx.save_for_backward(x, w, offs_t)
        ctx.meta = (G, K, tiles, sum_c)
        return out

    @staticmethod
    def backward(ctx, dout):
        x, w, offs_t = ctx.saved_tensors
        G, K, tiles, sum_c = ctx.meta
        dev = x.device
        dout = _lib.f32c(dout)
        N = x.shape[0]
        lib = _lib.load()
        dx = dw = None
        if ctx.needs_input_grad[0]:
            dx = torch.empty_like(x)
            _lib.check(lib.agnn_gproj_fwd_f32(dout.data_ptr(), dout.stride(0), w.data_ptr(), None, offs_t.data_ptr(), G, K, tiles, N,
                                              dx.data_ptr(), dx.stride(0), _lib.stream_ptr(dev)), "agnn_gproj_fwd_f32(as input gradient)")
        if ctx.needs_input_grad[1]:
            dw = torch.empty_like(w)
            nws = int(lib.agnn_gproj_workspace_bytes(N, sum_c, K, tiles))
            ws = torch.empty(max(nws, 1), dtype=torch.uint8, device=dev)
            _lib.check(lib.agnn_gproj_bwd_f32(x.data_ptr(), x.stride(0), dout.data_ptr(), dout.stride(0), w.data_ptr(), offs_t.data_ptr(),
                                              G, K, tiles, sum_c, N, None, 0, dw.data_ptr(), None, ws.data_ptr(), nws,
                                              _lib.stream_ptr(dev)), "agnn_gproj_bwd_f32(dw)")
        return dx, dw, None, None, None


def grouped_in_projection(x: torch.Tensor, w: torch.Tensor, offs: Sequence[int], K: int) -> torch.Tensor:
    return _GroupedInProj.apply(x, w, _offs_tensor(offs, x.device), tuple(int(o) for o in offs), int(K))


class CrossTaskTransformer(nn.Module):

    def __init__(self, proj_dim, num_heads=4, dropout=0.1):
        super().__init__()
        self.multihead_attn = nn.MultiheadAttention(proj_dim, num_heads, dropout=dropout, batch_first=True)
        self.norm = nn.LayerNorm(proj_dim)

    def forward(self, task_projections):
        from .fused import norm_act
        mha = self.multihead_attn
        N, T, E = task_projections.shape
        h = mha.num_heads
        x2 = task_projections.reshape(N * T, E)
        qkv = linear(x2, mha.in_proj_weight, mha.in_proj_bias).view(N, T, 3, h, E // h)
        q, k, v = (qkv[:, :, i].transpose(1, 2) for i in range(3))
        att = F.scaled_dot_product_attention(q, k, v, dropout_p=mha.dropout if self.training else 0.0)
        att = att.transpose(1, 2).reshape(N * T, E)
        out = linear(att, mha.out_proj.weight, mha.out_proj.bias, acc=x2)
        return norm_act(out, self.norm).view(N, T, E)


def fused_logit_fusion(proj_layers: nn.ModuleDict, transformer: nn.Module, fusion_layers: nn.ModuleDict, logits: torch.Tensor,
                       offs: Sequence[int], tasks: Sequence[str], training: bool) -> torch.Tensor:
    T = len(tasks)
    pm = [proj_layers[t] for t in tasks]
    K = pm[0][0].out_features
    N = logits.shape[0]
    _lib.require_gpu(logits)
    if not (K in GPROJ_K and T <= _lib.MAX_SEG):
        proj = [pm[i](logits[:, offs[i]:offs[i + 1]]) for i in range(T)]
        enh = transformer(torch.stack(proj, dim=1))
        return torch.cat([fusion_layers[t](enh[:, i]) for i, t in enumerate(tasks)], dim=1)
    Wp = torch.cat([m[0].weight.t() for m in pm], dim=0)
    bp = cat_rows([m[0].bias for m in pm])
    a = grouped_in_projection(logits, Wp, offs, K) + bp
    gamma = _cat_params([m[2].weight for m in pm], stack=True)
    beta = _cat_params([m[2].bias for m in pm], stack=True)
    a = grouped_norm_act(a.view(N, T, K), gamma, beta, pm[0][2].eps, pre_relu=True)
    enh = transformer(a)
    Wf = cat_rows([fusion_layers[t].weight for t in tasks])
    bf = cat_rows([fusion_layers[t].bias for t in tasks])
    return grouped_projection(enh.reshape(N, T * K), Wf, bf, offs, K)


class _MultiTaskCE(torch.autograd.Function):
    @staticmethod
    def forward(ctx, logits, labels, offs_t, eps: float, ignore_index: int, full_cover: bool = False):
        dev = _lib.require_gpu(logits, labels, offs_t)
        if logits.dtype != torch.float32 or logits.stride(1) != 1:
            logits = logits.float().contiguous()
        N = logits.shape[0]
        T = offs_t.numel() - 1
        labels = _check_labels(labels, T, N)
        row_loss = torch.empty((T, N), dtype=torch.float32, device=dev)
        loss = torch.zeros((T,), dtype=torch.float32, device=dev)
        inv_cnt = torch.ones((T,), dtype=torch.float32, device=dev)
        dlogits = torch.empty_like(logits) if full_cover else torch.zeros_like(logits)
        lib = _lib.load()
        _lib.check(lib.agnn_multitask_ce_f32(logits.data_ptr(), logits.stride(0), offs_t.data_ptr(), T, labels.data_ptr(), N,
                                             float(eps), int(ignore_index), row_loss.data_ptr(), dlogits.data_ptr(),
                                             loss.data_ptr(), inv_cnt.data_ptr(), _lib.stream_ptr(dev)), "agnn_multitask_ce_f32")
        ctx.save_for_backward(dlogits, offs_t, inv_cnt)
        return loss

    @staticmethod
    def backward(ctx, g):
        dlogits, offs_t, inv_cnt = ctx.saved_tensors
        dev = dlogits.device
        T = offs_t.numel() - 1
        scale = (g.to(torch.float32) * inv_cnt).contiguous()
        out = torch.empty_like(dlogits)
        lib = _lib.load()
        _lib.check(lib.agnn_multitask_ce_scale_f32(dlogits.data_ptr(), dlogits.stride(0), offs_t.data_ptr(), T, dlogits.shape[0],
                                                   dlogits.shape[1], scale.data_ptr(), out.data_ptr(), out.stride(0),
                                                   _lib.stream_ptr(dev)),
                   "agnn_multitask_ce_scale_f32")
        return out, None, None, None, None, None


def multitask_cross_entropy(logits: torch.Tensor, offs: Sequence[int], labels: torch.Tensor, label_smoothing: float = 0.1,
                            ignore_index: int = -1) -> torch.Tensor:
    full = len(offs) > 1 and offs[0] == 0 and offs[-1] == logits.shape[1] and all(offs[i] < offs[i + 1] for i in range(len(offs) - 1))
    return _MultiTaskCE.apply(logits, labels, _offs_tensor(offs, logits.device), label_smoothing, ignore_index, full)


def _check_labels(labels: torch.Tensor, T: int, N: int) -> torch.Tensor:
# ... 140 lines not shown
```

### analysisgnn_amd/linear.py

```python
from __future__ import annotations

from typing import Optional

import torch
import torch.nn as nn
import torch.nn.functional as F

from . import _lib, resident

MIN_ROWS = 2048
MAX_OUT_IN = 512 * 1024
ENABLED = True


_WG = {"enabled": False, "scope": "all", "dirty": set()}


def enable_wgrad_overlap(flag: bool = True, scope="all") -> None:
    _WG["enabled"] = bool(flag)
    _WG["scope"] = scope if scope == "all" else frozenset([scope] if isinstance(scope, str) else scope)


def wgrad_overlap_enabled() -> bool:
    return _WG["enabled"]


def mark_wgrad_async(t: torch.Tensor, deferrable: bool = False, leaves=()) -> torch.Tensor:
    t._agnn_wgrad_async = True
    t._agnn_wgrad_deferrable = bool(deferrable)
    t._agnn_leaves = tuple(leaves)
    return t


def _deferrable(t: Optional[torch.Tensor]) -> bool:
    return t is None or t.is_leaf or getattr(t, "_agnn_wgrad_deferrable", False)


def _async_ok(t: Optional[torch.Tensor]) -> bool:
    return t is None or t.is_leaf or getattr(t, "_agnn_wgrad_async", False)


def _steals(p: Optional[torch.Tensor]) -> bool:
    if p is None:
        return True
    if not p.is_leaf:
        return all(_steals(q) for q in getattr(p, "_agnn_leaves", ()))
    return p.grad is None and not p._backward_hooks and not getattr(p, "_post_accumulate_grad_hooks", None)


def leaf_refs(*ts) -> tuple:
    out = []
    for t in ts:
        if t is None:
            continue
        out.extend((t,) if t.is_leaf else getattr(t, "_agnn_leaves", ()))
    return tuple(out)


def all_steal(refs) -> bool:
    if all(_steals(p) for p in refs):
        return True
    if _DEFER["pending"] or _WG["dirty"] or _WG.get("join"):
        join_wgrad()
    return False


class wgrad_stream:

    def __init__(self, dev, *inputs, active: bool = True, kind: str = "linear"):
        self.on = bool(_WG["enabled"] and active and torch.device(dev).type == "cuda" and (_WG["scope"] == "all" or kind in _WG["scope"]))
        self.dev, self.inputs = torch.device(dev), inputs

    def __enter__(self):
        if not self.on:
            return self
        idx = resident.device_index(self.dev)
        ws = resident.stream(idx, "wgrad")
        cur = torch.cuda.current_stream(self.dev)
        if cur.cuda_stream != ws.cuda_stream:
            ws.wait_stream(cur)
        self.ws = ws
        self.ctx = torch.cuda.stream(ws)
        self.ctx.__enter__()
        _WG["dirty"].add(idx)
        return self

    def __exit__(self, *exc):
        if self.on:
            self.ctx.__exit__(*exc)
            for t in self.inputs:
                if t is not None:
                    t.record_stream(self.ws)
        return False


_DEFER = {"on": False, "pending": {}}


def defer_weight_grads(flag: bool = True) -> None:
    _DEFER["on"] = bool(flag)
    if not flag:
        flush_all_deferred()


def deferring(t: torch.Tensor) -> bool:
    return bool(_DEFER["on"] and t.is_cuda)


def defer(fn, dev, here: bool = False) -> None:
    s = torch.cuda.current_stream(dev)
    home = _DEFER.get("home")
    if ITEMS_HOME and not here and isinstance(fn, (WgItem, ColsumItem)) and home is not None and (home.device.index, home.cuda_stream) != (s.device.index, s.cuda_stream):
        fn.event = torch.cuda.Event()
        fn.event.record(s)
        defer_on(home, fn)
        return
    _DEFER["pending"].setdefault((s.device.index, s.cuda_stream), (s, []))[1].append(fn)


ITEMS_HOME = True


def defer_on(stream, fn) -> None:
    _DEFER["pending"].setdefault((stream.device.index, stream.cuda_stream), (stream, []))[1].append(fn)


def set_home_stream(stream) -> None:
    _DEFER["home"] = stream


def defer_home(fn, dev, tensors=()) -> bool:
    home = _DEFER.get("home")
    cur = torch.cuda.current_stream(dev)
    if home is None or (home.device.index, home.cuda_stream) == (cur.device.index, cur.cuda_stream):
        return False
    ev = torch.cuda.Event()
    ev.record(cur)

    def run():
        here = torch.cuda.current_stream(dev)
        here.wait_event(ev)
        fn()
        for t in tensors:
            if t is not None:
                t.record_stream(here)
    run.handed_over = True
    defer_on(home, run)
    return True


def _run_deferred(fns) -> None:
    items = [f for f in fns if isinstance(f, WgItem)]
    sums = [f for f in fns if isinstance(f, ColsumItem)]
    foreign = [f for f in items + sums if f.event is not None]
    if foreign:
        here = torch.cuda.current_stream(foreign[0].tensors()[0].device)
        for f in foreign:
            here.wait_event(f.event)
            for t in f.tensors():
                if t is not None:
                    t.record_stream(here)
    with torch.no_grad():
        if items:
            weight_grad_batch(items)
        if sums:
            colsum_batch(sums)
        for fn in fns:
            if not isinstance(fn, (WgItem, ColsumItem)):
                fn()


FLUSH_KEEP = 1.0


def _spill(fns, keep: float, other) -> list:
    cost = lambda u: sum(2.0 * f.dy.shape[0] * f.dy.shape[1] * f.x.shape[1] for f in u if isinstance(f, WgItem))
    units, cur = [], []
    for f in fns:
        if isinstance(f, WgItem) and not (f.follows and cur and isinstance(cur[-1], WgItem) and cur[-1].dy is f.dy):
            units.append(cur)
            cur = [f]
        else:
            cur.append(f)
    units.append(cur)
    movable = lambda u: (u and isinstance(u[0], WgItem) and u[0].event is None
                         and not any(getattr(f, "event", None) is not None or getattr(f, "handed_over", False) for f in u[1:]))
    total = sum(cost(u) for u in units if u and isinstance(u[0], WgItem))
    if total <= 0:
        return fns
    moved, out = 0.0, set()
    for i in range(len(units) - 1, 0, -1):
        u = units[i]
        if not movable(u):
            continue
        if moved + cost(u) > (1.0 - keep) * total + 1e-9:
            break
        moved += cost(u)
        out.add(i)
    if not out:
        return fns
    ev = torch.cuda.Event()
    ev.record(torch.cuda.current_stream(other.device))
    for i in sorted(out):
        for f in units[i]:
            if isinstance(f, (WgItem, ColsumItem)):
                f.event = ev
            defer_on(other, f)
    return [f for i, u in enumerate(units) if i not in out for f in u]


def flush_deferred(dev=None, spill_to=None) -> None:
    s = torch.cuda.current_stream(dev)
    entry = _DEFER["pending"].pop((s.device.index, s.cuda_stream), None)
    if entry is not None:
        fns = entry[1]
        if spill_to is not None and FLUSH_KEEP < 1.0:
            fns = _spill(fns, FLUSH_KEEP, spill_to)
        _run_deferred(fns)
        join_later(s)


def flush_all_deferred() -> None:
    cur = torch.cuda.current_stream() if torch.cuda.is_available() else None
    for key in list(_DEFER["pending"]):
        s, fns = _DEFER["pending"].pop(key)
        with torch.cuda.stream(s):
            _run_deferred(fns)
        if cur is not None and (s.device.index, s.cuda_stream) != (cur.device.index, cur.cuda_stream):
            torch.cuda.current_stream(s.device).wait_stream(s)


def join_later(stream) -> None:
    _WG.setdefault("join", {})[(stream.device.index, stream.cuda_stream)] = stream


def join_wgrad() -> None:
    flush_all_deferred()
    for idx in list(_WG["dirty"]):
        torch.cuda.current_stream(idx).wait_stream(resident.stream(idx, "wgrad"))
    _WG["dirty"].clear()
    for s in list(_WG.get("join", {}).values()):
        cur = torch.cuda.current_stream(s.device)
        if (cur.device.index, cur.cuda_stream) != (s.device.index, s.cuda_stream):
            cur.wait_stream(s)
    _WG.get("join", {}).clear()


def _ok(t: torch.Tensor) -> bool:
    return (t.dtype == torch.float32 and t.dim() == 2 and t.stride(1) == 1 and t.stride(0) % 2 == 0
            and t.shape[1] % 2 == 0 and t.data_ptr() % 8 == 0)


def _dw_ok(dw: torch.Tensor) -> bool:
    return dw.dim() == 2 and dw.stride(1) == 1 and dw.stride(0) >= dw.shape[1] and dw.stride(0) % 2 == 0 and dw.data_ptr() % 8 == 0


def weight_grad(dy: torch.Tensor, x: torch.Tensor, want_bias: bool, dw_out: Optional[torch.Tensor] = None,
                db_out: Optional[torch.Tensor] = None):
    n, out_f = dy.shape
    in_f = x.shape[1]
    in_k = in_f
    if in_f & 1 and x.dim() == 2 and x.stride(1) == 1 and x.stride(0) > in_f:
        in_k = in_f + 1
        x = x.as_strided((n, in_k), (x.stride(0), 1), x.storage_offset())
    if not (ENABLED and dy.is_cuda and n >= MIN_ROWS and out_f * in_k <= MAX_OUT_IN and _ok(dy) and _ok(x)):
        if in_k != in_f:
            x = x[:, :in_f]
        if dw_out is not None:
            torch.mm(dy.t(), x, out=dw_out)
            if want_bias:
                torch.sum(dy, dim=0, out=db_out)
            return dw_out, (db_out if want_bias else None)
        return dy.t() @ x, (dy.sum(dim=0) if want_bias else None)
    lib = _lib.load()
    dev = dy.device
    if dw_out is not None:
        if in_k != in_f or tuple(dw_out.shape) != (out_f, in_f) or not _dw_ok(dw_out) or (want_bias and (db_out is None or not db_out.is_contiguous())):
            raise _lib.AgnnError("weight_grad: dw_out / db_out must be [out, in] (rows contiguous, even stride) / contiguous [out] with an even `in`")
        dw, db = dw_out, (db_out if want_bias else None)
    else:
        dw = torch.empty((out_f, in_k), dtype=torch.float32, device=dev)
        db = torch.empty((out_f,), dtype=torch.float32, device=dev) if want_bias else None
    nws = int(lib.agnn_wgrad_workspace_bytes(n, out_f, in_k))
    ws = torch.empty(nws, dtype=torch.uint8, device=dev)
    _lib.check(lib.agnn_wgrad_f32(dy.data_ptr(), dy.stride(0), x.data_ptr(), x.stride(0), n, out_f, in_k, dw.data_ptr(),
                                  dw.stride(0), _lib.ptr(db), ws.data_ptr(), nws, _lib.stream_ptr(dev)), "agnn_wgrad_f32")
    return (dw if in_k == in_f else dw[:, :in_f].contiguous()), db


class WgItem:
    __slots__ = ("dy", "x", "want_bias", "dw_out", "db_out", "event", "follows")

    def __init__(self, dy, x, want_bias, dw_out, db_out, follows=False):
        self.dy, self.x, self.want_bias, self.dw_out, self.db_out, self.event = dy, x, bool(want_bias), dw_out, db_out, None
        self.follows = bool(follows)

    def tensors(self):
        return (self.dy, self.x, self.dw_out, self.db_out)

    def __call__(self):
        weight_grad(self.dy, self.x, self.want_bias, dw_out=self.dw_out, db_out=self.db_out)


class ColsumItem:
    __slots__ = ("ws", "n", "H", "dgamma", "dbeta", "event")

    def __init__(self, ws, n, H, dgamma, dbeta):
        self.ws, self.n, self.H, self.dgamma, self.dbeta, self.event = ws, int(n), int(H), dgamma, dbeta, None

    def tensors(self):
        return (self.ws, self.dgamma, self.dbeta)

    def __call__(self):
        _lib.check(_lib.load().agnn_norm_act_colsum_f32(self.ws.data_ptr(), self.ws.numel(), self.n, self.H, self.dgamma.data_ptr(),
                                                        self.dbeta.data_ptr(), _lib.stream_ptr(self.ws.device)), "agnn_norm_act_colsum_f32")


def colsum_batch(items) -> None:
    if not BATCH or len(items) == 1:
        for it in items:
            it()
        return
    lib = _lib.load()
    for i in range(0, len(items), _lib.WGRAD_BATCH_MAX):
        grp = items[i:i + _lib.WGRAD_BATCH_MAX]
        arr = (_lib.ColsumItem * len(grp))()
        for a, it in zip(arr, grp):
            a.workspace, a.workspace_bytes, a.n, a.H = it.ws.data_ptr(), it.ws.numel(), it.n, it.H
            a.dgamma, a.dbeta = it.dgamma.data_ptr(), it.dbeta.data_ptr()
        _lib.check(lib.agnn_norm_act_colsum_batch_f32(len(grp), arr, _lib.stream_ptr(grp[0].ws.device)), "agnn_norm_act_colsum_batch_f32")


BATCH = True


def weight_grad_batch(items) -> None:
    lib = None
    group = []
    products = 0

    def fits(it):
        n, out_f = it.dy.shape
        in_f = it.x.shape[1]
        return (BATCH and ENABLED and it.dy.is_cuda and it.dy.dim() == 2 and it.x.dim() == 2 and n >= MIN_ROWS and out_f * in_f <= MAX_OUT_IN and in_f % 2 == 0
                and _ok(it.dy) and _ok(it.x) and it.dw_out is not None and tuple(it.dw_out.shape) == (out_f, in_f) and _dw_ok(it.dw_out)
                and (not it.want_bias or (it.db_out is not None and it.db_out.is_contiguous() and it.db_out.data_ptr() % 8 == 0)))

    def run(group):
        if len(group) == 1:
            group[0]()
            return
        nonlocal lib
        lib = lib or _lib.load()
        dev = group[0].dy.device
        arr = (_lib.WgradItem * len(group))()
        for a, it in zip(arr, group):
            a.dy, a.x, a.dw = it.dy.data_ptr(), it.x.data_ptr(), it.dw_out.data_ptr()
            a.db = it.db_out.data_ptr() if it.want_bias else None
            a.ld_dy, a.ld_x, a.ld_dw, a.n = it.dy.stride(0), it.x.stride(0), it.dw_out.stride(0), it.dy.shape[0]
            a.out_f, a.in_f = it.dy.shape[1], it.x.shape[1]
        nws = int(lib.agnn_wgrad_batch_workspace_bytes(len(group), arr))
        ws = torch.empty(nws, dtype=torch.uint8, device=dev)
        _lib.check(lib.agnn_wgrad_batch_f32(len(group), arr, ws.data_ptr(), nws, _lib.stream_ptr(dev)), "agnn_wgrad_batch_f32")

    for it in items:
        if fits(it):
            joins = it.follows and group and group[-1].dy is it.dy
            if group and ((products == _lib.WGRAD_BATCH_MAX and not joins) or len(group) == _lib.WGRAD_BATCH_MAX_ITEMS):
                run(group)
                group, products, joins = [], 0, False
            group.append(it)
            products += 0 if joins else 1
        else:
            it()
    if group:
        run(group)


HAND_GEMM = True
HAND_GEMM_DX = False
HAND_GEMM_MIN_ROWS = 4096
HAND_GEMM_MIN_K, HAND_GEMM_MIN_N = 256, 256
HAND_GEMM_MAX_K = 1536


def _hand_gemm_dx_ok(dy, w) -> bool:
    return (dy.is_cuda and dy.dim() == 2 and dy.dtype == torch.float32 and w.dtype == torch.float32 and dy.shape[0] >= HAND_GEMM_MIN_ROWS
            and w.shape[1] % 64 == 0 and w.shape[0] % 16 == 0 and dy.stride(1) == 1 and w.stride(1) == 1 and dy.stride(0) % 4 == 0
            and w.stride(0) % 4 == 0 and dy.stride(0) >= dy.shape[1] and w.stride(0) >= w.shape[1] and dy.data_ptr() % 16 == 0 and w.data_ptr() % 16 == 0)


def _hand_gemm_ok(x, w, b) -> bool:
    return (x.is_cuda and x.dim() == 2 and x.dtype == torch.float32 and w.dtype == torch.float32 and x.shape[0] >= HAND_GEMM_MIN_ROWS
            and HAND_GEMM_MIN_K <= x.shape[1] <= HAND_GEMM_MAX_K and w.shape[0] >= HAND_GEMM_MIN_N and w.shape[0] % 64 == 0 and x.shape[1] % 16 == 0 and x.stride(1) == 1 and w.stride(1) == 1 and x.stride(0) % 4 == 0
            and w.stride(0) % 4 == 0 and x.stride(0) >= x.shape[1] and w.stride(0) >= w.shape[1] and x.data_ptr() % 16 == 0 and w.data_ptr() % 16 == 0 and (b is None or (b.dtype == torch.float32 and b.is_contiguous())))


def hand_gemm(x: torch.Tensor, w: torch.Tensor, b: Optional[torch.Tensor]) -> torch.Tensor:
    y = torch.empty((x.shape[0], w.shape[0]), dtype=torch.float32, device=x.device)
    _lib.check(_lib.load().agnn_gemm_nt_f32(x.data_ptr(), x.stride(0), w.data_ptr(), w.stride(0), _lib.ptr(b), x.shape[0], w.shape[0], x.shape[1],
                                            y.data_ptr(), y.stride(0), _lib.stream_ptr(x.device)), "agnn_gemm_nt_f32")
    return y


class _LinearFn(torch.autograd.Function):
    @staticmethod
    def forward(ctx, x, w, b, acc, pre=None):
        ctx.save_for_backward(x, w)
        ctx.has_bias = b is not None
        ctx.wg_async = _async_ok(w) and _async_ok(b)
        ctx.wg_defer = _deferrable(w) and _deferrable(b)
        ctx.steal_refs = leaf_refs(w, b)
        ctx.grad_cols = getattr(x, "_agnn_grad_cols", None) if x.dim() == 2 else None
        ctx.set_materialize_grads(False)
        if pre is not None:
            return pre[0]
        if acc is not None:
            y = torch.addmm(acc, x, w.t())
            return y + b if b is not None else y
        if HAND_GEMM and _hand_gemm_ok(x, w, b):
            return hand_gemm(x, w, b)
        return torch.addmm(b, x, w.t()) if b is not None else x @ w.t()

    @staticmethod
    def backward(ctx, dy):
        if dy is None:
            return None, None, None, None, None
        x, w = ctx.saved_tensors
        dw = db = None
        want_w = ctx.needs_input_grad[1] or (ctx.has_bias and ctx.needs_input_grad[2])
        want_b = ctx.has_bias and ctx.needs_input_grad[2]
        steals = ctx.wg_async and all_steal(ctx.steal_refs)
        in_f = x.shape[1]
        padded = bool(in_f & 1) and x.dim() == 2 and x.stride(1) == 1 and x.stride(0) > in_f
        if want_w and steals and ctx.wg_defer and (in_f % 2 == 0 or padded) and deferring(dy):
            dw = torch.empty((dy.shape[1], in_f), dtype=torch.float32, device=dy.device)
            db = torch.empty((dy.shape[1],), dtype=torch.float32, device=dy.device) if want_b else None
            dw_k, db_k = dw.detach(), (db.detach() if db is not None else None)
            if padded:
                dw_wide = torch.empty((dy.shape[1], in_f + 1), dtype=torch.float32, device=dy.device)
                defer(WgItem(dy, x.as_strided((x.shape[0], in_f + 1), (x.stride(0), 1), x.storage_offset()), want_b, dw_wide, db_k), dy.device, here=True)
                defer(lambda: dw_k.copy_(dw_wide[:, :in_f]), dy.device)
            else:
                defer(WgItem(dy, x, want_b, dw_k, db_k), dy.device)
        elif want_w:
            with wgrad_stream(dy.device, dy, x, active=steals):
                dw, db = weight_grad(dy, x, want_b)
        dx = None
        if ctx.needs_input_grad[0]:
            gc = ctx.grad_cols
            if gc is not None and x.stride(1) == 1 and x.stride(0) >= x.shape[1] and w.stride(1) == 1 and dy.is_cuda:
                c0, c1 = gc
                full = torch.empty((dy.shape[0], x.stride(0)), dtype=dy.dtype, device=dy.device)
                torch.mm(dy, w[:, c0:c1], out=full[:, c0:c1])
                dx = full[:, :x.shape[1]]
            elif HAND_GEMM and HAND_GEMM_DX and _hand_gemm_dx_ok(dy, w):
                dx = torch.empty((dy.shape[0], w.shape[1]), dtype=torch.float32, device=dy.device)
                _lib.check(_lib.load().agnn_gemm_nn_f32(dy.data_ptr(), dy.stride(0), w.data_ptr(), w.stride(0), None, dy.shape[0], w.shape[1], w.shape[0],
                                                        dx.data_ptr(), dx.stride(0), _lib.stream_ptr(dy.device)), "agnn_gemm_nn_f32")
            else:
                dx = dy @ w
        return dx, dw, db, (dy if ctx.needs_input_grad[3] else None), None


def linear(x: torch.Tensor, w: torch.Tensor, b: Optional[torch.Tensor] = None, acc: Optional[torch.Tensor] = None, pre=None) -> torch.Tensor:
    if pre is not None:
        if torch.is_grad_enabled() and (x.requires_grad or w.requires_grad or (b is not None and b.requires_grad)):
            return _LinearFn.apply(x, w, b, None, pre)
        return pre[0]
    if x.is_cuda and torch.is_grad_enabled() and (w.requires_grad or (b is not None and b.requires_grad)):
        if x.dim() == 2 and x.shape[0] >= MIN_ROWS:
            return _LinearFn.apply(x, w, b, acc)
        if x.dim() == 3 and x.shape[0] * x.shape[1] >= MIN_ROWS and acc is None:
            return _LinearFn.apply(x.reshape(-1, x.shape[-1]), w, b, None).view(x.shape[0], x.shape[1], -1)
    y = F.linear(x, w, b)
    return y + acc if acc is not None else y


def _hand_gemm2_ok(x0, x1, w, b) -> bool:
    k0, k1 = x0.shape[1], x1.shape[1]
    blk = lambda t: (t.is_cuda and t.dim() == 2 and t.dtype == torch.float32 and t.shape[1] % 16 == 0 and t.shape[1] > 0 and t.stride(1) == 1
                     and t.stride(0) % 4 == 0 and t.stride(0) >= t.shape[1] and t.data_ptr() % 16 == 0)
    return (blk(x0) and blk(x1) and x0.shape[0] == x1.shape[0] and x0.shape[0] >= HAND_GEMM_MIN_ROWS and w.dtype == torch.float32 and w.dim() == 2
            and w.shape[1] == k0 + k1 and HAND_GEMM_MIN_K <= k0 + k1 <= HAND_GEMM_MAX_K and w.shape[0] >= HAND_GEMM_MIN_N and w.shape[0] % 64 == 0
            and w.stride(1) == 1 and w.stride(0) % 4 == 0 and w.stride(0) >= w.shape[1] and w.data_ptr() % 16 == 0
            and (b is None or (b.dtype == torch.float32 and b.is_contiguous())))


def hand_gemm2(x0: torch.Tensor, x1: torch.Tensor, w: torch.Tensor, b: Optional[torch.Tensor]) -> torch.Tensor:
    y = torch.empty((x0.shape[0], w.shape[0]), dtype=torch.float32, device=x0.device)
    _lib.check(_lib.load().agnn_gemm_nt2_f32(x0.data_ptr(), x0.stride(0), x0.shape[1], x1.data_ptr(), x1.stride(0), x1.shape[1], w.data_ptr(),
                                             w.stride(0), _lib.ptr(b), x0.shape[0], w.shape[0], y.data_ptr(), y.stride(0),
                                             _lib.stream_ptr(x0.device)), "agnn_gemm_nt2_f32")
    return y


class _Linear2Fn(torch.autograd.Function):

    @staticmethod
    def forward(ctx, x0, x1, w, b):
        ctx.save_for_backward(x0, x1, w)
        ctx.has_bias = b is not None
        ctx.wg_async = _async_ok(w) and _async_ok(b)
        ctx.wg_defer = _deferrable(w) and _deferrable(b)
        ctx.steal_refs = leaf_refs(w, b)
        ctx.set_materialize_grads(False)
        return hand_gemm2(x0, x1, w, b)

    @staticmethod
    def backward(ctx, dy):
        if dy is None:
            return None, None, None, None
        x0, x1, w = ctx.saved_tensors
        k0 = x0.shape[1]
        dw = db = None
        want_w = ctx.needs_input_grad[2] or (ctx.has_bias and ctx.needs_input_grad[3])
        want_b = ctx.has_bias and ctx.needs_input_grad[3]
        steals = ctx.wg_async and all_steal(ctx.steal_refs)
        if want_w:
            dw = torch.empty((dy.shape[1], w.shape[1]), dtype=torch.float32, device=dy.device)
            db = torch.empty((dy.shape[1],), dtype=torch.float32, device=dy.device) if want_b else None
            dw_k, db_k = dw.detach(), (db.detach() if db is not None else None)
            if steals and ctx.wg_defer and deferring(dy):
                defer(WgItem(dy, x0, want_b, dw_k[:, :k0], db_k), dy.device)
                defer(WgItem(dy, x1, False, dw_k[:, k0:], None, follows=True), dy.device)
            else:
                with wgrad_stream(dy.device, dy, x0, x1, active=steals):
                    weight_grad(dy, x0, want_b, dw_out=dw_k[:, :k0], db_out=db_k)
                    weight_grad(dy, x1, False, dw_out=dw_k[:, k0:])
        dx0 = dx1 = None
        if ctx.needs_input_grad[0] or ctx.needs_input_grad[1]:
            dx = dy @ w
            dx0 = dx[:, :k0] if ctx.needs_input_grad[0] else None
            dx1 = dx[:, k0:] if ctx.needs_input_grad[1] else None
        return dx0, dx1, dw, db


def linear2(x0: torch.Tensor, x1: torch.Tensor, w: torch.Tensor, b: Optional[torch.Tensor] = None) -> Optional[torch.Tensor]:
    if not (HAND_GEMM and _hand_gemm2_ok(x0, x1, w, b)):
        return None
    if torch.is_grad_enabled() and (x0.requires_grad or x1.requires_grad or w.requires_grad or (b is not None and b.requires_grad)):
        return _Linear2Fn.apply(x0, x1, w, b)
    return hand_gemm2(x0, x1, w, b)


class Linear(nn.Linear):
    def forward(self, x):
        return linear(x, self.weight, self.bias)
```

### analysisgnn_amd/params.py

```python
from __future__ import annotations

from typing import List, Sequence, Tuple

import torch

from . import _lib
from .linear import all_steal, defer, deferring, mark_wgrad_async, wgrad_stream


def pack(items: Sequence[Tuple[torch.Tensor, Sequence[torch.Tensor]]], device) -> None:
    arr = (_lib.PackItem * len(items))()
    for i, (dst, srcs) in enumerate(items):
        if len(srcs) > _lib.PACK_MAX_SRC:
            raise _lib.AgnnError(f"pack: {len(srcs)} sources (max {_lib.PACK_MAX_SRC})")
        rows, cols = dst.shape
        ld_src = (srcs[0].stride(0) if rows > 1 else max(cols, 1)) if srcs else max(cols, 1)
        for t in (dst, *srcs):
            if t.dtype != torch.float32 or t.dim() != 2 or (cols > 1 and t.stride(1) != 1) or tuple(t.shape) != (rows, cols):
                raise _lib.AgnnError("pack: fp32 2-D pieces of one shape with unit inner stride expected")
        for k, t in enumerate(srcs):
            if rows > 1 and t.stride(0) != ld_src:
                raise _lib.AgnnError("pack: the sources of an item must share their row stride")
            arr[i].src[k] = t.data_ptr()
        arr[i].dst = dst.data_ptr()
        arr[i].ld_dst = dst.stride(0) if rows > 1 else max(cols, 1)
        arr[i].ld_src = ld_src
        arr[i].rows, arr[i].cols, arr[i].n_src = rows, cols, len(srcs)
    lib = _lib.load()
    _lib.check(lib.agnn_pack_f32(len(items), arr, _lib.stream_ptr(device)), "agnn_pack_f32")


class _SageOperands(torch.autograd.Function):

    @staticmethod
    def forward(ctx, R: int, *params):
        w_l, b_l, w_r = params[:R], params[R:2 * R], params[2 * R:]
        dev = _lib.require_gpu(*params)
        out_f, in_f = w_l[0].shape
        W_l = torch.empty((out_f, R * in_f), dtype=torch.float32, device=dev)
        b = torch.empty((out_f,), dtype=torch.float32, device=dev)
        W_r = torch.empty((out_f, in_f), dtype=torch.float32, device=dev)
        items = [(W_l[:, r * in_f:(r + 1) * in_f], [w_l[r].detach()]) for r in range(R)]
        items.append((b.view(1, -1), [t.detach().view(1, -1) for t in b_l]))
        items.append((W_r, [t.detach() for t in w_r]))
        pack(items, dev)
        ctx.R = R
        ctx.shape = (out_f, in_f)
        ctx.leaves = all(t.is_leaf for t in params)
        ctx.param_refs = tuple(params)
        return W_l, b, W_r

    @staticmethod
    def backward(ctx, dW_l, db, dW_r):
        R = ctx.R
        out_f, in_f = ctx.shape
        dev = dW_l.device
        G_l = torch.empty((R, out_f, in_f), dtype=torch.float32, device=dev)
        G_b = torch.empty((R, out_f), dtype=torch.float32, device=dev)
        G_r = torch.empty((R, out_f, in_f), dtype=torch.float32, device=dev)
        def fan_out():
            dW_l_, db_, dW_r_ = _lib.f32c(dW_l), db.contiguous(), _lib.f32c(dW_r)
            items = []
            for r in range(R):
                items.append((G_l[r], [dW_l_[:, r * in_f:(r + 1) * in_f]]))
                items.append((G_b[r].view(1, -1), [db_.view(1, -1)]))
                items.append((G_r[r], [dW_r_]))
            pack(items, dev)
        off_chain = ctx.leaves and all_steal(ctx.param_refs)
        if off_chain and deferring(dW_l):
            defer(fan_out, dev)
        else:
            with wgrad_stream(dev, dW_l, db, dW_r, active=off_chain):
                fan_out()
        return (None, *G_l.unbind(0), *G_b.unbind(0), *G_r.unbind(0))


class _SageOperandsCat(torch.autograd.Function):

    @staticmethod
    def forward(ctx, R: int, with_l: bool, *params):
        w_l, b_l, w_r = params[:R], params[R:2 * R], params[2 * R:]
        dev = _lib.require_gpu(*params)
        out_f, in_f = w_r[0].shape
        nl = R if with_l else 0
        W = torch.empty((out_f, (nl + 1) * in_f), dtype=torch.float32, device=dev)
        b = torch.empty((out_f,), dtype=torch.float32, device=dev)
        items = [(W[:, r * in_f:(r + 1) * in_f], [w_l[r].detach()]) for r in range(nl)]
        items.append((b.view(1, -1), [t.detach().view(1, -1) for t in b_l]))
        items.append((W[:, nl * in_f:], [t.detach() for t in w_r]))
        pack(items, dev)
        ctx.R, ctx.nl = R, nl
        ctx.shape = (out_f, in_f)
        ctx.leaves = all(t.is_leaf for t in params)
        ctx.param_refs = tuple(params)
        return W, b

    @staticmethod
    def backward(ctx, dW, db):
        R, nl = ctx.R, ctx.nl
        out_f, in_f = ctx.shape
        dev = dW.device
        G_l = torch.empty((nl, out_f, in_f), dtype=torch.float32, device=dev)
        G_b = torch.empty((R, out_f), dtype=torch.float32, device=dev)
        G_r = torch.empty((R, out_f, in_f), dtype=torch.float32, device=dev)
        if not nl:
            G_l = torch.zeros((R, out_f, in_f), dtype=torch.float32, device=dev)

        def fan_out():
            dW_, db_ = _lib.f32c(dW), db.contiguous()
            items = []
            for r in range(R):
                if r < nl:
                    items.append((G_l[r], [dW_[:, r * in_f:(r + 1) * in_f]]))
                items.append((G_b[r].view(1, -1), [db_.view(1, -1)]))
                items.append((G_r[r], [dW_[:, nl * in_f:]]))
            pack(items, dev)
        off_chain = ctx.leaves and all_steal(ctx.param_refs)
        if off_chain and deferring(dW):
            defer(fan_out, dev)
        else:
            with wgrad_stream(dev, dW, db, active=off_chain):
                fan_out()
        return (None, None, *G_l.unbind(0), *G_b.unbind(0), *G_r.unbind(0))


def sage_operands_cat(w_l: List[torch.Tensor], b_l: List[torch.Tensor], w_r: List[torch.Tensor], with_l: bool = True):
    R = len(w_l)
    ok = (w_l[0].is_cuda and R <= _lib.PACK_MAX_SRC and all(t is not None for t in b_l)
          and all(t.shape == w_l[0].shape and t.is_contiguous() for t in (*w_l, *w_r)))
    if not ok:
        return None
    ops_ = _SageOperandsCat.apply(R, with_l, *w_l, *b_l, *w_r)
    if all(t.is_leaf for t in (*w_l, *b_l, *w_r)):
        for t in ops_:
            mark_wgrad_async(t, deferrable=True, leaves=(*w_l, *b_l, *w_r))
    return ops_


def sage_operands(w_l: List[torch.Tensor], b_l: List[torch.Tensor], w_r: List[torch.Tensor]):
    R = len(w_l)
    ok = (w_l[0].is_cuda and R <= _lib.PACK_MAX_SRC and all(t is not None for t in b_l)
          and all(t.shape == w_l[0].shape and t.is_contiguous() for t in (*w_l, *w_r)))
    if not ok:
        return torch.cat(w_l, dim=1), (sum(b_l) if all(t is not None for t in b_l) else None), sum(w_r)
    ops_ = _SageOperands.apply(R, *w_l, *b_l, *w_r)
    if all(t.is_leaf for t in (*w_l, *b_l, *w_r)):
        for t in ops_:
            mark_wgrad_async(t, deferrable=True, leaves=(*w_l, *b_l, *w_r))
    return ops_


def adjacent(ts: Sequence[torch.Tensor]) -> bool:
    t0 = ts[0]
    if not all(t.is_contiguous() and t.dtype == t0.dtype and t.device == t0.device for t in ts):
        return False
    base = t0.untyped_storage().data_ptr()
    off = t0.storage_offset()
    for t in ts:
        if t.untyped_storage().data_ptr() != base or t.storage_offset() != off:
            return False
        off += t.numel()
    return True


class _AdjacentCat(torch.autograd.Function):

    @staticmethod
    def forward(ctx, *params):
        p0 = params[0]
        rows = [int(p.shape[0]) for p in params]
        ctx.rows = rows
        return p0.detach().as_strided((sum(rows),) + tuple(p0.shape[1:]), p0.stride(), p0.storage_offset())

    @staticmethod
    def backward(ctx, g):
        return tuple(g.split(ctx.rows, dim=0))


def cat_rows(params: Sequence[torch.Tensor]) -> torch.Tensor:
    if len(params) > 1 and all(p.shape[1:] == params[0].shape[1:] for p in params) and adjacent(params):
        return _AdjacentCat.apply(*params)
    return torch.cat(list(params), dim=0)


def stack_rows(params: Sequence[torch.Tensor]) -> torch.Tensor:
    if len(params) > 1 and all(p.shape == params[0].shape for p in params) and adjacent(params):
        return _AdjacentCat.apply(*[p.unsqueeze(0) for p in params])
    return torch.stack(list(params))
```

### include/agnn.h

```cpp
#ifndef AGNN_H_
#define AGNN_H_

#include <stddef.h>
#include <stdint.h>

#ifdef __cplusplus
extern "C" {
#endif

typedef void* agnn_stream_t;

#define AGNN_OK        0
#define AGNN_EINVAL  (-22)
#define AGNN_EALIGN  (-14)
#define AGNN_ENOMEM  (-12)
#define AGNN_ERUNTIME (-5)

#define AGNN_MAX_SEG 32

const char* agnn_last_error(void);
int agnn_version(void);

typedef struct {
  const int64_t* row;
// ... 63 lines not shown
                          int64_t pool_rows, int32_t H, float* dx, int64_t ld_dx, agnn_stream_t stream);

int agnn_gru_fwd_f32(const float* gi, const float* w_hh, const float* b_hh, int64_t B, int64_t T,
                     int32_t hidden, float* y, float* saved, const float* drop_scale, float* y_drop,
                     agnn_stream_t stream);
int agnn_gru_bwd_f32(const float* dy, const float* y, const float* saved, const float* w_hh,
                     int64_t B, int64_t T, int32_t hidden, float* dgi, float* dgh, const float* drop_scale, float* hprev,
                     agnn_stream_t stream);
int agnn_gru_hprev_f32(const float* y, int64_t B, int64_t T, int32_t hidden, float* hp, agnn_stream_t stream);

typedef struct {
  const float* k;
  const float* v;
  const int32_t* rowptr;
  const int32_t* rowend;
  const int32_t* col;
  const int32_t* perm;
  const float* pscale;
  int64_t ld;
  float* alpha;
  float* gs;
  float* tdot;
  int64_t ld_tdot;
} agnn_hgt_rel_t;

int agnn_hgt_attn_fwd_f32(int n_rel, const agnn_hgt_rel_t* rels , const float* q, int64_t ld_q,
                          int64_t n_rows, int32_t H, int32_t heads, float* out, int64_t ld_out,
                          float* m_out, float* linv_out, agnn_stream_t stream);
#define AGNN_HGT_MAX_DST 4
typedef struct {
  const agnn_hgt_rel_t* rels;
  int32_t n_rel;
  const float* q;
  int64_t ld_q;
  int64_t n_rows;
  float* out;
  int64_t ld_out;
  float* m_out;
  float* linv_out;
} agnn_hgt_dst_item_t;
int agnn_hgt_attn_fwd_multi_f32(int32_t n_items, const agnn_hgt_dst_item_t* items , int32_t H, int32_t heads,
                                agnn_stream_t stream);
int agnn_hgt_attn_bwd_dst_f32(int n_rel, const agnn_hgt_rel_t* rels , const float* q, int64_t ld_q,
                              const float* dm, int64_t ld_dm, const float* out, int64_t ld_out,
                              const float* m_in, const float* linv_in, int64_t n_rows, int32_t H,
                              int32_t heads, float* dq, int64_t ld_dq, agnn_stream_t stream);
typedef struct {
  const int32_t* rowptr;
  const int32_t* rowend;
  const int32_t* col;
  const int32_t* perm;
  const float* alpha;
  const float* gs;
  float* dk;
  float* dv;
  int64_t ld_o;
  int32_t n_src_rows;
  int32_t col_limit;
} agnn_hgt_src_item_t;
int agnn_hgt_attn_bwd_src_batch_f32(int32_t n_items, const agnn_hgt_src_item_t* items , const float* q, int64_t ld_q,
                                    const float* dm, int64_t ld_dm, int32_t H, int32_t heads, agnn_stream_t stream);


typedef struct {
  const int32_t* rowptr;
  const int32_t* col;
  const int32_t* perm;
  const float* a;
  const float* b;
  const float* h;
  const float* c;
  int64_t ld, ld_c;
  int64_t n_rows;
  int32_t H;
} agnn_gated_t;

int agnn_gated_fwd_f32(const agnn_gated_t* g , float* out, int64_t ld_out, agnn_stream_t stream);
int agnn_gated_bwd_dst_f32(const agnn_gated_t* g , const float* ds, int64_t ld_ds, float* da,
                           float* dc, agnn_stream_t stream);
int agnn_gated_bwd_src_f32(const agnn_gated_t* g , const float* ds, int64_t ld_ds, float* db,
                           float* dh, agnn_stream_t stream);

int agnn_gemm_nn_f32(const float* a, int64_t ld_a, const float* w , int64_t ld_w, const float* bias, int64_t M, int32_t N,
                     int32_t K, float* c, int64_t ld_c, agnn_stream_t stream);
int agnn_gemm_nt_f32(const float* a, int64_t ld_a, const float* w, int64_t ld_w, const float* bias, int64_t M, int32_t N,
                     int32_t K, float* c, int64_t ld_c, agnn_stream_t stream);
int agnn_gemm_nt2_f32(const float* a0, int64_t ld_a0, int32_t K0, const float* a1, int64_t ld_a1, int32_t K1, const float* w,
                      int64_t ld_w, const float* bias, int64_t M, int32_t N, float* c, int64_t ld_c, agnn_stream_t stream);

int agnn_absdiff_fwd_f32(const int32_t* rowptr, const int32_t* col, const float* h, int64_t ld, int64_t n_rows, int32_t H,
                         float* out_s, float* out_d, int64_t ld_out, agnn_stream_t stream);
int agnn_absdiff_bwd_f32(const int32_t* rowptr, const int32_t* col, const float* h, int64_t ld, int64_t n_rows, int32_t H,
                         const float* gd, const float* gs, int64_t ld_g, int32_t by_col, int32_t accumulate, float* out,
                         int64_t ld_out, agnn_stream_t stream);

#define AGNN_NA_PRE_RELU  1u
#define AGNN_NA_POST_RELU 2u
size_t agnn_norm_act_workspace_bytes(int32_t H);
int agnn_norm_act_fwd_f32(const float* x, int64_t ld_x, const float* gamma, const float* beta, int32_t seg,
                          int64_t n, int32_t H, float eps, float p, uint32_t flags, const int64_t* rng_state, uint32_t call_id, float* y,
                          int64_t ld_y, float* mean, float* rstd, int64_t* rng_used, agnn_stream_t stream);
int agnn_norm_act_bwd_f32(const float* x, int64_t ld_x, const float* gamma, const float* beta, int32_t seg,
                          int64_t n, int32_t H, float eps, float p, uint32_t flags, const int64_t* rng_state, uint32_t call_id,
                          const float* dy, int64_t ld_dy, const float* mean, const float* rstd, float* dx,
                          int64_t ld_dx, float* dgamma, float* dbeta, void* workspace, size_t workspace_bytes,
                          agnn_stream_t stream);

typedef struct {
  const void* workspace;
  size_t workspace_bytes;
  int64_t n;
  int32_t H;
  float* dgamma;
  float* dbeta;
} agnn_colsum_item_t;
int agnn_norm_act_colsum_batch_f32(int32_t n_items, const agnn_colsum_item_t* items , agnn_stream_t stream);

size_t agnn_skip_act_workspace_bytes(void);
int agnn_skip_act_fwd_f32(const float* x, int64_t ld_x, const float* o, int64_t ld_o, const float* skip, int64_t n, int32_t H, float p,
                          uint32_t flags, const int64_t* rng_state, uint32_t call_id, float* z, int64_t ld_z, int64_t* rng_used,
                          agnn_stream_t stream);
int agnn_skip_act_bwd_f32(const float* x, int64_t ld_x, const float* o, int64_t ld_o, const float* skip, int64_t n, int32_t H, float p,
                          uint32_t flags, const int64_t* rng_state, uint32_t call_id, const float* dz, int64_t ld_dz, float* dx,
                          int64_t ld_dx, float* dout, int64_t ld_do, float* dskip, void* workspace, size_t workspace_bytes,
                          agnn_stream_t stream);
int agnn_norm_act_colsum_f32(const void* workspace, size_t workspace_bytes, int64_t n, int32_t H, float* dgamma, float* dbeta,
                             agnn_stream_t stream);

size_t agnn_wgrad_workspace_bytes(int64_t n, int32_t out_f, int32_t in_f);
int agnn_wgrad_f32(const float* dy, int64_t ld_dy, const float* x, int64_t ld_x, int64_t n, int32_t out_f,
                   int32_t in_f, float* dw, int64_t ld_dw, float* db, void* workspace, size_t workspace_bytes,
                   agnn_stream_t stream);
typedef struct {
  const float* dy;
  const float* x;
  float* dw;
  float* db;
  int64_t ld_dy, ld_x, ld_dw, n;
  int32_t out_f, in_f;
} agnn_wgrad_item_t;
size_t agnn_wgrad_batch_workspace_bytes(int32_t n_items, const agnn_wgrad_item_t* items );
int agnn_wgrad_batch_f32(int32_t n_items, const agnn_wgrad_item_t* items , void* workspace, size_t workspace_bytes,
                         agnn_stream_t stream);

#define AGNN_PACK_MAX_SRC   8
#define AGNN_PACK_MAX_ITEMS 24
typedef struct {
  float* dst;
  const float* src[AGNN_PACK_MAX_SRC];
  int64_t ld_dst, ld_src;
  int32_t rows, cols, n_src, vec_ok;
} agnn_pack_item_t;
int agnn_pack_f32(int32_t n_items, const agnn_pack_item_t* items , agnn_stream_t stream);

int agnn_debug_stamp(uint64_t* slot , agnn_stream_t stream);

#define AGNN_EMBED_MAX_TABLES 4
int agnn_embed_cat_fwd_f32(const float* x, int64_t ld_x, int32_t in_x, int64_t n_rows, int32_t n_tab,
                           const int64_t* const* idx, const float* const* tables, const int32_t* vocab, int32_t dim,
                           float* out, int64_t ld_out, agnn_stream_t stream);
size_t agnn_embed_workspace_bytes(int32_t n_tab, const int32_t* vocab, int32_t dim);
int agnn_embed_cat_bwd_f32(const float* dout, int64_t ld_dout, int32_t col0, int64_t n_rows, int32_t n_tab,
                           const int64_t* const* idx, const int32_t* vocab, int32_t dim, float* dtables,
                           void* workspace, size_t workspace_bytes, agnn_stream_t stream);

int agnn_heads_fwd_f32(const float* x, int64_t ld_x, int64_t n_rows, int32_t in_f, int32_t hidden, int32_t T, const float* w1,
                       const float* b1, const float* gamma, const float* beta, float eps, const float* w2, const float* b2,
                       const int32_t* offs_dev, const int32_t* offs_host, float* z, float* y, int64_t ld_h, float* mean,
                       float* rstd, float* logits, int64_t ld_o, agnn_stream_t stream);

int agnn_gproj_fwd_f32(const float* a, int64_t ld_a, const float* w, const float* b, const int32_t* seg_off,
                       int32_t n_groups, int32_t K, int32_t n_tiles32, int64_t n_rows, float* out, int64_t ld_out,
                       agnn_stream_t stream);
size_t agnn_gproj_workspace_bytes(int64_t n_rows, int32_t sum_c, int32_t K, int32_t n_tiles32);
int agnn_gproj_bwd_f32(const float* dout, int64_t ld_dout, const float* a, int64_t ld_a, const float* w,
                       const int32_t* seg_off, int32_t n_groups, int32_t K, int32_t n_tiles32, int32_t sum_c,
                       int64_t n_rows, float* da, int64_t ld_da, float* dw, float* db, void* workspace,
                       size_t workspace_bytes, agnn_stream_t stream);

int agnn_multitask_ce_f32(const float* logits, int64_t ld, const int32_t* seg_off, int32_t n_tasks,
                          const int64_t* labels, int64_t n_rows, float label_smoothing,
                          int64_t ignore_index, float* row_loss, float* dlogits, float* loss, float* inv_count,
                          agnn_stream_t stream);
int agnn_multitask_ce_scale_f32(const float* dlogits, int64_t ld, const int32_t* seg_off, int32_t n_tasks,
                                int64_t n_rows, int32_t n_cols, const float* scale, float* out, int64_t ld_out,
                                agnn_stream_t stream);

size_t agnn_train_loss_workspace_bytes(void);
int agnn_train_loss_f32(const float* logits, int64_t ld, const int32_t* seg_off, int32_t n_tasks, const int64_t* labels,
                        int64_t n_rows, float label_smoothing, int64_t ignore_index, const float* feat, int64_t ld_feat,
                        int32_t feat_cols, float lambda_feat, const float* task_param, float ce_scale, float* row_loss,
                        float* dlogits, float* loss, float* inv_count, float* total, float* wscale, float* dparam,
                        void* workspace, size_t workspace_bytes, agnn_stream_t stream);
int agnn_train_loss_final_f32(const float* logits, int64_t ld, const int32_t* seg_off, int32_t n_tasks, const int64_t* labels,
                              int64_t n_rows, float label_smoothing, int64_t ignore_index, const float* feat, int64_t ld_feat,
                              int32_t feat_cols, float lambda_feat, const float* task_param, float ce_scale, float* row_loss,
                              float* dlogits, float* loss, float* inv_count, float* total, float* wscale, float* dparam,
                              float* dfeat, int64_t ld_dfeat, void* workspace, size_t workspace_bytes, agnn_stream_t stream);
int agnn_train_loss_bwd_f32(const float* dlogits, int64_t ld, const int32_t* seg_off, int32_t n_tasks, int64_t n_rows,
                            int32_t n_cols, const float* inv_count, const float* g, float* out, int64_t ld_out,
                            const float* feat, int64_t ld_feat, int32_t feat_cols, float lambda_feat, float* dfeat,
                            int64_t ld_dfeat, agnn_stream_t stream);

#define AGNN_SAMPLER_MAX_REL 8
#define AGNN_SAMPLER_MAX_HOPS 4
#define AGNN_SAMPLER_MAX_FAN 16
#define AGNN_SAMPLER_MAX_CAP 256
typedef struct {
  int32_t n_rel;
  const int32_t* rowptr[AGNN_SAMPLER_MAX_REL];
  const int32_t* col[AGNN_SAMPLER_MAX_REL];
  const int32_t* win_start;
  int32_t n_sub, n_targets, n_hops;
  int32_t fan[AGNN_SAMPLER_MAX_HOPS];
  int32_t cap[AGNN_SAMPLER_MAX_HOPS];
  const int64_t* rng;
  int32_t* node_gid;
  int64_t* edges[AGNN_SAMPLER_MAX_REL];
  int64_t e_cap;
  int32_t* status;
  int32_t* drops;
  int32_t* kept;
} agnn_sampler_t;
int64_t agnn_sampler_num_nodes(const agnn_sampler_t* cfg );
int64_t agnn_sampler_edge_capacity(const agnn_sampler_t* cfg );
int agnn_sample_hops(const agnn_sampler_t* cfg , agnn_stream_t stream);
int agnn_sample_members(const int32_t* node_gid, int64_t n_nodes, const int64_t* batch ,
                        const int32_t* group_of, const int32_t* win_start, int32_t n_sub, int32_t n_targets, int32_t n_hops,
                        const int32_t* cap , int32_t cap_g, int32_t* group_gid, int64_t* edges, int32_t* drops,
                        agnn_stream_t stream);
int64_t agnn_sample_compact_nodes(const agnn_sampler_t* cfg , const int32_t* pool );
int agnn_sample_compact(const agnn_sampler_t* cfg , const int32_t* pool , int32_t* node_gid_out,
                        int64_t* batch_out, agnn_stream_t stream);
int agnn_gather_rows_f32(const float* src, int64_t ld_src, const int32_t* gid, int64_t n, int32_t H, float* out,
                         int64_t ld_out, agnn_stream_t stream);
int agnn_gather_i64(const int64_t* src, int64_t ld_src, const int32_t* gid, int64_t n, int32_t n_vec, int64_t fill,
                    int64_t* out, int64_t ld_out, agnn_stream_t stream);

#define AGNN_RELT_MAX_ITEMS 4
typedef struct {
  const float* x;
  const float* w;
  float* y;
  int64_t ld_x, ld_y;
} agnn_relt_item_t;
int agnn_relt_fwd_f32(int n_items, const agnn_relt_item_t* items , int32_t n_rel, int32_t heads, int32_t D,
                      int64_t n_rows, agnn_stream_t stream);
int agnn_relt_bwd_f32(int n_items, const agnn_relt_item_t* items , int32_t n_rel, int32_t heads, int32_t D,
                      int64_t n_rows, agnn_stream_t stream);
size_t agnn_relt_dw_workspace_bytes(int n_items, int32_t n_rel, int32_t heads, int32_t D, int64_t n_rows);
int agnn_relt_dw_f32(int n_items, const agnn_relt_item_t* items , int32_t n_rel, int32_t heads, int32_t D,
                     int64_t n_rows, void* workspace, size_t workspace_bytes, agnn_stream_t stream);

size_t agnn_adamw_workspace_bytes(void);
int agnn_adamw_f32(float* p, float* g, float* m, float* v, int64_t n, float lr, float beta1, float beta2, float eps,
                   float weight_decay, float max_norm, float* step, float* norm_out, int32_t write_clipped_grad,
                   void* workspace, size_t workspace_bytes, agnn_stream_t stream);

#define AGNN_LR_CONSTANT      0
#define AGNN_LR_WARMUP_COSINE 1
#define AGNN_LR_WARMUP_EXP    2
typedef struct {
  int32_t kind;
  int32_t warmup_steps;
  int32_t count_offset;
  int32_t swa_period;
  int64_t swa_start;
  int32_t swa_anneal;
  double base_lr, warmup_start_lr, eta_min, cos_a, cos_b, gamma, decay_steps, swa_lr;
} agnn_lr_schedule_t;

double agnn_lr_schedule_at(const agnn_lr_schedule_t* sched , int64_t k);
size_t agnn_adamw_sched_workspace_bytes(void);
int agnn_adamw_sched_f32(float* p, float* g, float* m, float* v, int64_t n, const agnn_lr_schedule_t* sched ,
                         float beta1, float beta2, float eps, float weight_decay, float max_norm, float* step, float* swa_avg,
                         float* state, float* norm_out, int32_t write_clipped_grad, void* workspace, size_t workspace_bytes,
                         agnn_stream_t stream);

size_t agnn_kd_workspace_bytes(int64_t n_rows, int32_t n_tasks);
int agnn_multitask_kd_f32(const float* student, int64_t ld_s, const float* teacher, int64_t ld_t, const int32_t* seg_off,
                          const int32_t* seg_end, int32_t n_tasks, int64_t n_rows, int32_t n_cols, float temperature,
                          float weight, float* dstudent, int64_t ld_d, float* kd, float* total, void* workspace,
                          size_t workspace_bytes, agnn_stream_t stream);

size_t agnn_ewc_workspace_bytes(void);
int agnn_ewc_f32(const float* p, const float* mean, const float* fisher, int64_t n, float lambda, float* g, float* penalty,
                 void* workspace, size_t workspace_bytes, agnn_stream_t stream);
int agnn_fisher_accum_f32(const float* g, int64_t n, float scale, float* fisher, agnn_stream_t stream);

#define AGNN_EVAL_MAX_COLS 800
size_t agnn_eval_counts_len(int32_t n_tasks, int32_t n_cols);
int agnn_multitask_eval_f32(const float* logits, int64_t ld, const int32_t* seg_off, const int32_t* seg_end, int32_t n_tasks,
                            int32_t n_cols, const int64_t* labels, int64_t n_rows, int64_t ignore_index,
                            const uint8_t* row_mask, int32_t gate_task, uint32_t group_mask, int32_t* pred, int64_t* counts,
                            agnn_stream_t stream);

#ifdef __cplusplus
}
#endif
#endif
```

Before: 5.679 million subgraph-nodes/s.

## Fuse weight-gradient reduction, fan-out to parameter slots, and norm colsums into one epilogue

Adds a grad-epilogue kernel that reduces the batched weight-gradient slabs and writes the results straight into every per-parameter gradient destination (column slices, bias copies). The same launch also computes the layernorm gamma/beta column sums. Autograd functions for SAGE operand concatenation now carry 'boxes' of preallocated slots, so backward returns those directly and skips the separate pack/fan-out copies. A multi-item gather kernel is also added. The aim is fewer launches and fewer intermediate gradient buffers and copies in the backward pass, at the cost of substantial bookkeeping complexity and alias checks.

Measured after the change: 5.748 million subgraph-nodes/s, median of 6. 1.2% higher.

```diff
diff --git a/analysisgnn_amd/_lib.py b/analysisgnn_amd/_lib.py
--- a/analysisgnn_amd/_lib.py
+++ b/analysisgnn_amd/_lib.py
@@ -95,6 +95,23 @@
 class PackItem(C.Structure):
     _fields_ = [("dst", C.c_void_p), ("src", C.c_void_p * PACK_MAX_SRC), ("ld_dst", C.c_int64), ("ld_src", C.c_int64),
                 ("rows", C.c_int32), ("cols", C.c_int32), ("n_src", C.c_int32), ("vec_ok", C.c_int32)]
+
+
+PACK_MAX_ITEMS = 24
+GRAD_MAX_SUMS = 16
+
+
+class GatherItem(C.Structure):
+    _fields_ = [("dst", C.c_void_p), ("src", C.c_void_p), ("n", C.c_int64)]
+
+
+class GradDst(C.Structure):
+    _fields_ = [("p", C.c_void_p), ("ld", C.c_int64), ("c0", C.c_int32), ("c1", C.c_int32)]
+
+
+class GradItem(C.Structure):
+    _fields_ = [("dy", C.c_void_p), ("x", C.c_void_p), ("ld_dy", C.c_int64), ("ld_x", C.c_int64), ("n", C.c_int64), ("out_f", C.c_int32),
+                ("in_f", C.c_int32), ("n_dw", C.c_int32), ("n_db", C.c_int32), ("dw", GradDst * PACK_MAX_SRC), ("db", C.c_void_p * PACK_MAX_SRC)]
 
 
 LR_CONSTANT, LR_WARMUP_COSINE, LR_WARMUP_EXP = 0, 1, 2
@@ -156,6 +173,8 @@
                                   C.c_void_p]),
     "agnn_wgrad_batch_workspace_bytes": (C.c_size_t, [C.c_int32, C.POINTER(WgradItem)]),
     "agnn_wgrad_batch_f32": (C.c_int, [C.c_int32, C.POINTER(WgradItem), C.c_void_p, C.c_size_t, C.c_void_p]),
+    "agnn_grad_epilogue_workspace_bytes": (C.c_size_t, [C.c_int32, C.POINTER(GradItem)]),
+    "agnn_grad_epilogue_f32": (C.c_int, [C.c_int32, C.POINTER(GradItem), C.c_int32, C.POINTER(ColsumItem), C.c_void_p, C.c_size_t, C.c_void_p]),
     "agnn_gemm_nt_f32": (C.c_int, [C.c_void_p, C.c_int64, C.c_void_p, C.c_int64, C.c_void_p, C.c_int64, C.c_int32, C.c_int32, C.c_void_p,
                                    C.c_int64, C.c_void_p]),
     "agnn_gemm_nn_f32": (C.c_int, [C.c_void_p, C.c_int64, C.c_void_p, C.c_int64, C.c_void_p, C.c_int64, C.c_int32, C.c_int32, C.c_void_p,
@@ -193,6 +212,7 @@
     "agnn_wgrad_f32": (C.c_int, [C.c_void_p, C.c_int64, C.c_void_p, C.c_int64, C.c_int64, C.c_int32, C.c_int32, C.c_void_p,
                                  C.c_int64, C.c_void_p, C.c_void_p, C.c_size_t, C.c_void_p]),
     "agnn_pack_f32": (C.c_int, [C.c_int32, C.POINTER(PackItem), C.c_void_p]),
+    "agnn_gather_f32": (C.c_int, [C.c_int32, C.POINTER(GatherItem), C.c_void_p]),
     "agnn_debug_stamp": (C.c_int, [C.c_void_p, C.c_void_p]),
     "agnn_gproj_fwd_f32": (C.c_int, [C.c_void_p, C.c_int64, C.c_void_p, C.c_void_p, C.c_void_p, C.c_int32, C.c_int32, C.c_int32,
                                      C.c_int64, C.c_void_p, C.c_int64, C.c_void_p]),
diff --git a/analysisgnn_amd/csrc/pack.hip b/analysisgnn_amd/csrc/pack.hip
--- a/analysisgnn_amd/csrc/pack.hip
+++ b/analysisgnn_amd/csrc/pack.hip
@@ -86,6 +86,77 @@
 }
 
 namespace {
+
+struct GatherTable {
+  float* dst[AGNN_GATHER_MAX_ITEMS];
+  const float* src[AGNN_GATHER_MAX_ITEMS];
+  int32_t n[AGNN_GATHER_MAX_ITEMS];
+  int32_t first_block[AGNN_GATHER_MAX_ITEMS + 1];
+  int32_t count;
+};
+static_assert(sizeof(GatherTable) <= 4096, "GatherTable travels as a kernel argument");
+
+__global__ __launch_bounds__(256) void k_gather(GatherTable t) {
+  int lo = 0, hi = t.count - 1;
+  while (lo < hi) {
+    const int mid = (lo + hi + 1) >> 1;
+    if (static_cast<int>(blockIdx.x) >= t.first_block[mid]) lo = mid; else hi = mid - 1;
+  }
+  float* dst = t.dst[lo];
+  const float* src = t.src[lo];
+  const int n = t.n[lo];
+  const bool vec = ((reinterpret_cast<uintptr_t>(dst) | reinterpret_cast<uintptr_t>(src)) & 15u) == 0;
+  const int base = (static_cast<int>(blockIdx.x) - t.first_block[lo]) * (kElemsPerBlock / 4);
+#pragma unroll
+  for (int u = 0; u < kElemsPerBlock / 1024; ++u) {
+    const int64_t e = (static_cast<int64_t>(base) + u * 256 + threadIdx.x) * 4;
+    if (e >= n) break;
+    if (vec && e + 3 < n) {
+      *reinterpret_cast<float4*>(dst + e) = src ? *reinterpret_cast<const float4*>(src + e) : make_float4(0.f, 0.f, 0.f, 0.f);
+    } else {
+      for (int k = 0; k < 4 && e + k < n; ++k) dst[e + k] = src ? src[e + k] : 0.f;
+    }
+  }
+}
+
+}
+
+extern "C" int agnn_gather_f32(int32_t n_items, const agnn_gather_item_t* items, agnn_stream_t stream_) {
+  using namespace agnn;
+  if (n_items < 0) return fail(AGNN_EINVAL, "gather: negative item count");
+  if (n_items > 0 && !items) return fail(AGNN_EINVAL, "gather: null item table");
+  for (int32_t i = 0; i < n_items; ++i) {
+    const agnn_gather_item_t& it = items[i];
+    if (it.n < 0 || it.n >= (int64_t{1} << 31)) return fail(AGNN_EINVAL, "gather: item %d has %lld floats", i, (long long)it.n);
+    if (it.n > 0 && !it.dst) return fail(AGNN_EINVAL, "gather: item %d: null destination", i);
+    if ((reinterpret_cast<uintptr_t>(it.dst) | reinterpret_cast<uintptr_t>(it.src)) & 3u) return fail(AGNN_EALIGN, "gather: item %d is not float-aligned", i);
+  }
+  hipStream_t s = static_cast<hipStream_t>(stream_);
+  int32_t at = 0;
+  while (at < n_items) {
+    GatherTable t;
+    t.count = 0;
+    int64_t blocks = 0;
+    for (; at < n_items && t.count < AGNN_GATHER_MAX_ITEMS; ++at) {
+      const agnn_gather_item_t& it = items[at];
+      if (it.n == 0) continue;
+      const int64_t b = (it.n + kElemsPerBlock - 1) / kElemsPerBlock;
+      if (blocks + b >= (int64_t{1} << 31)) return fail(AGNN_EINVAL, "gather: too many floats in one call");
+      t.dst[t.count] = it.dst;
+      t.src[t.count] = it.src;
+      t.n[t.count] = static_cast<int32_t>(it.n);
+      t.first_block[t.count++] = static_cast<int32_t>(blocks);
+      blocks += b;
+    }
+    if (t.count == 0) continue;
+    t.first_block[t.count] = static_cast<int32_t>(blocks);
+    hipLaunchKernelGGL(k_gather, dim3(static_cast<unsigned>(blocks)), dim3(256), 0, s, t);
+    if (int rc = check_launch("gather")) return rc;
+  }
+  return AGNN_OK;
+}
+
+namespace {
 __global__ void k_stamp(unsigned long long* slot) { *slot = wall_clock64(); }
 }
 
diff --git a/analysisgnn_amd/csrc/wgrad.hip b/analysisgnn_amd/csrc/wgrad.hip
--- a/analysisgnn_amd/csrc/wgrad.hip
+++ b/analysisgnn_amd/csrc/wgrad.hip
@@ -153,9 +153,10 @@
 }
 
 
-__device__ __forceinline__ void wgrad_reduce_blocks(const float* __restrict__ slab, const float* __restrict__ slab_b, int S, int out_f, int in_f,
-                                                    int out_pad, int in_pad, float* __restrict__ dw, int64_t ld_dw, float* __restrict__ db,
-                                                    const int block, const int n_blocks) {
+template <typename StoreW, typename StoreB>
+__device__ __forceinline__ void wgrad_reduce_sums(const float* __restrict__ slab, const float* __restrict__ slab_b, int S, int out_f, int in_f,
+                                                  int out_pad, int in_pad, const bool with_bias, const int block, const int n_blocks,
+                                                  StoreW store_w, StoreB store_b) {
   __shared__ float2 part[8][32];
   const int col = threadIdx.x & 31, sg = threadIdx.x >> 5;
   const int half_in = in_f >> 1;
@@ -181,11 +182,11 @@
       float2 t = part[0][col];
 #pragma unroll
       for (int g = 1; g < 8; ++g) { t.x += part[g][col].x; t.y += part[g][col].y; }
-      *reinterpret_cast<float2*>(dw + static_cast<int64_t>(o) * ld_dw + i) = t;
+      store_w(o, i, t);
     }
     __syncthreads();
   }
-  if (db != nullptr) {
+  if (with_bias) {
     __shared__ float partb[8][32];
     for (int e0 = block * 32; e0 < out_f; e0 += n_blocks * 32) {
       const int e = e0 + col;
@@ -198,11 +199,19 @@
         float t = partb[0][col];
 #pragma unroll
         for (int g = 1; g < 8; ++g) t += partb[g][col];
-        db[e] = t;
+        store_b(e, t);
       }
       __syncthreads();
     }
   }
+}
+
+__device__ __forceinline__ void wgrad_reduce_blocks(const float* __restrict__ slab, const float* __restrict__ slab_b, int S, int out_f, int in_f,
+                                                    int out_pad, int in_pad, float* __restrict__ dw, int64_t ld_dw, float* __restrict__ db,
+                                                    const int block, const int n_blocks) {
+  wgrad_reduce_sums(slab, slab_b, S, out_f, in_f, out_pad, in_pad, db != nullptr, block, n_blocks,
+                    [=](int o, int i, float2 t) { *reinterpret_cast<float2*>(dw + static_cast<int64_t>(o) * ld_dw + i) = t; },
+                    [=](int e, float t) { db[e] = t; });
 }
 
 __global__ __launch_bounds__(256) void k_wgrad_reduce(const float* __restrict__ slab, const float* __restrict__ slab_b, int S,
@@ -392,3 +401,264 @@
   hipLaunchKernelGGL(k_wgrad_reduce_batch, dim3(static_cast<unsigned>(red)), dim3(256), 0, s, rb);
   return check_launch("wgrad_batch(reduce)");
 }
+
+namespace {
+
+constexpr int kEpiRecMax = 64;
+constexpr int kEpiDbMax = 48;
+constexpr int kEpiSumMax = AGNN_GRAD_MAX_SUMS;
+constexpr int kEpiPartRows = 1024;
+
+struct EpiRec {
+  float* p;
+  int32_t ld, c0, c1, scalar;
+};
+struct EpiItem {
+  const float* slab;
+  const float* slab_b;
+  int32_t S, out_f, in_f, out_pad, in_pad;
+  int16_t rec0, rec1, db0, db1;
+};
+struct EpiSum {
+  const float* part;
+  float* dgamma;
+  float* dbeta;
+  int32_t n_rows, H;
+};
+struct EpiBatch {
+  EpiItem it[kWgBatchMax];
+  EpiRec rec[kEpiRecMax];
+  float* db[kEpiDbMax];
+  EpiSum sum[kEpiSumMax];
+  int32_t first[kWgBatchMax + kEpiSumMax + 1];
+  int32_t n_items, n_all;
+};
+static_assert(sizeof(EpiBatch) <= 4096, "EpiBatch travels as a kernel argument");
+
+__device__ __forceinline__ void epi_product(const EpiBatch& b, const EpiItem& r, const int block, const int n_blocks) {
+  const int rec0 = r.rec0, rec1 = r.rec1, db0 = r.db0, db1 = r.db1;
+  wgrad_reduce_sums(
+      r.slab, r.slab_b, r.S, r.out_f, r.in_f, r.out_pad, r.in_pad, db1 > db0, block, n_blocks,
+      [&](int o, int i, float2 t) {
+        for (int q = rec0; q < rec1; ++q) {
+          const EpiRec d = b.rec[q];
+          float* row = d.p + static_cast<int64_t>(o) * d.ld - d.c0;
+          if (d.scalar) {
+            if (i >= d.c0 && i < d.c1) row[i] = t.x;
+            if (i + 1 >= d.c0 && i + 1 < d.c1) row[i + 1] = t.y;
+          } else if (i >= d.c0 && i < d.c1) {
+            *reinterpret_cast<float2*>(row + i) = t;
+          }
+        }
+      },
+      [&](int e, float t) {
+        for (int q = db0; q < db1; ++q) b.db[q][e] = t;
+      });
+}
+
+__device__ __forceinline__ void epi_colsum(const EpiSum& c, const int block) {
+  __shared__ float sm[32][33];
+  const int col = threadIdx.x & 31, g8 = threadIdx.x >> 5;
+  const int width = 2 * c.H, n_rows = c.n_rows;
+  const int j = block * 32 + col;
+  float s[4] = {0.f, 0.f, 0.f, 0.f};
+  if (j < width) {
+    for (int w00 = 0; w00 < n_rows; w00 += 32 * 32) {
+#pragma unroll
+      for (int q = 0; q < 4; ++q) {
+        const int w0 = w00 + g8 + 8 * q;
+        if (w0 >= n_rows) continue;
+        float v[32];
+#pragma unroll
+        for (int k = 0; k < 32; ++k) {
+          const int w = w0 + 32 * k;
+          v[k] = w < n_rows ? c.part[static_cast<int64_t>(w) * width + j] : 0.f;
+        }
+#pragma unroll
+        for (int k = 0; k < 32; ++k) s[q] += v[k];
+      }
+    }
+  }
+#pragma unroll
+  for (int q = 0; q < 4; ++q) sm[g8 + 8 * q][col] = s[q];
+  __syncthreads();
+  if (g8 == 0 && j < width) {
+    float t = sm[0][col];
+#pragma unroll
+    for (int k = 1; k < 32; ++k) t += sm[k][col];
+    if (j < c.H) c.dgamma[j] = t; else c.dbeta[j - c.H] = t;
+  }
+}
+
+__global__ __launch_bounds__(256) void k_grad_epilogue(EpiBatch b) {
+  int i = 0;
+  const int blk = blockIdx.x;
+  while (i + 1 < b.n_all && blk >= b.first[i + 1]) ++i;
+  const int local = blk - b.first[i];
+  if (i < b.n_items) epi_product(b, b.it[i], local, b.first[i + 1] - b.first[i]);
+  else epi_colsum(b.sum[i - b.n_items], local);
+}
+
+struct EpiSpan {
+  const float* p;
+  int64_t ld;
+  int32_t rows, cols;
+  int32_t item, c0, c1;
+};
+
+bool spans_overlap(const EpiSpan& a, const EpiSpan& b) {
+  const float* a_end = a.p + static_cast<int64_t>(a.rows - 1) * a.ld + a.cols;
+  const float* b_end = b.p + static_cast<int64_t>(b.rows - 1) * b.ld + b.cols;
+  if (a_end <= b.p || b_end <= a.p) return false;
+  if (a.rows > 1 && b.rows > 1 && a.ld == b.ld) {
+    int64_t r = (b.p - a.p) % a.ld;
+    if (r < 0) r += a.ld;
+    if (r >= a.cols && r + b.cols <= a.ld) return false;
+  }
+  return true;
+}
+
+}
+
+static void epi_as_wgrad(int32_t n_items, const agnn_grad_item_t* items, agnn_wgrad_item_t* out) {
+  for (int i = 0; i < n_items; ++i) {
+    const agnn_grad_item_t& g = items[i];
+    out[i] = agnn_wgrad_item_t{g.dy, g.x, nullptr, nullptr, g.ld_dy, g.ld_x, g.in_f, g.n, g.out_f, g.in_f};
+  }
+}
+
+extern "C" size_t agnn_grad_epilogue_workspace_bytes(int32_t n_items, const agnn_grad_item_t* items) {
+  if (n_items <= 0 || n_items > kWgBatchMax || !items) return 0;
+  agnn_wgrad_item_t w[kWgBatchMax];
+  epi_as_wgrad(n_items, items, w);
+  return agnn_wgrad_batch_workspace_bytes(n_items, w);
+}
+
+extern "C" int agnn_grad_epilogue_f32(int32_t n_items, const agnn_grad_item_t* items, int32_t n_sums, const agnn_colsum_item_t* sums,
+                                      void* workspace, size_t workspace_bytes, agnn_stream_t stream_) {
+  using namespace agnn;
+  if (n_items < 0 || n_items > kWgBatchMax || (n_items > 0 && !items)) return fail(AGNN_EINVAL, "grad_epilogue: %d products (0 .. %d)", n_items, kWgBatchMax);
+  if (n_sums < 0 || n_sums > kEpiSumMax || (n_sums > 0 && !sums)) return fail(AGNN_EINVAL, "grad_epilogue: %d column sums (0 .. %d)", n_sums, kEpiSumMax);
+  if (n_items == 0 && n_sums == 0) return AGNN_OK;
+  BatchPlan bp;
+  bp.n = 0;
+  bp.total_floats = 0;
+  float* ws = nullptr;
+  if (n_items > 0) {
+    agnn_wgrad_item_t w[kWgBatchMax];
+    epi_as_wgrad(n_items, items, w);
+    if (int rc = batch_plan(n_items, w, bp)) return rc;
+    if (!workspace || workspace_bytes < bp.total_floats * sizeof(float) + 256) return fail(AGNN_ENOMEM, "grad_epilogue: workspace too small");
+    ws = reinterpret_cast<float*>((reinterpret_cast<uintptr_t>(workspace) + 255) & ~uintptr_t{255});
+  }
+  static thread_local EpiSpan spans[kWgBatchMax * 2 * AGNN_PACK_MAX_SRC + 2 * kEpiSumMax];
+  int n_spans = 0;
+  for (int i = 0; i < n_items; ++i) {
+    const agnn_grad_item_t& it = items[i];
+    if ((it.out_f & 1) || (it.in_f & 1) || (it.ld_dy & 1) || (it.ld_x & 1)) return fail(AGNN_EALIGN, "grad_epilogue: item %d: widths and leading dimensions must be even", i);
+    if (!it.dy || !it.x) return fail(AGNN_EINVAL, "grad_epilogue: item %d: null argument", i);
+    if ((reinterpret_cast<uintptr_t>(it.dy) | reinterpret_cast<uintptr_t>(it.x)) & 7u) return fail(AGNN_EALIGN, "grad_epilogue: item %d: pointers must be 8-byte aligned", i);
+    if (it.ld_dy < it.out_f || it.ld_x < it.in_f) return fail(AGNN_EINVAL, "grad_epilogue: item %d: leading dimension smaller than the width", i);
+    if ((static_cast<int64_t>(bp.rps[i]) + 128) * (it.ld_dy > it.ld_x ? it.ld_dy : it.ld_x) * 4 >= (int64_t{1} << 32))
+      return fail(AGNN_EINVAL, "grad_epilogue: item %d: a row slice (%d rows x ld) exceeds the kernel's 32-bit byte offsets", i, bp.rps[i]);
+    if (it.n_dw < 0 || it.n_dw > AGNN_PACK_MAX_SRC || it.n_db < 0 || it.n_db > AGNN_PACK_MAX_SRC || it.n_dw + it.n_db == 0)
+      return fail(AGNN_EINVAL, "grad_epilogue: item %d: %d weight and %d bias destinations (0 .. %d each, one at least)", i, it.n_dw, it.n_db, AGNN_PACK_MAX_SRC);
+    for (int k = 0; k < it.n_dw; ++k) {
+      const agnn_grad_dst_t& d = it.dw[k];
+      const int cols = d.c1 - d.c0;
+      if (!d.p || d.c0 < 0 || cols <= 0 || d.c1 > it.in_f || d.ld < cols || d.ld >= (int64_t{1} << 31))
+        return fail(AGNN_EINVAL, "grad_epilogue: item %d: destination %d: columns [%d, %d) of %d, ld %lld", i, k, d.c0, d.c1, it.in_f, (long long)d.ld);
+      if (reinterpret_cast<uintptr_t>(d.p) & 3u) return fail(AGNN_EALIGN, "grad_epilogue: item %d: destination %d is not a float pointer", i, k);
+      if (!(cols & 1) && ((d.c0 & 1) || (d.ld & 1) || (reinterpret_cast<uintptr_t>(d.p) & 7u)))
+        return fail(AGNN_EALIGN, "grad_epilogue: item %d: destination %d: an even column block needs an even c0, an even ld and an 8-byte aligned pointer", i, k);
+      spans[n_spans++] = EpiSpan{d.p, d.ld, it.out_f, cols, i, d.c0, d.c1};
+    }
+    for (int k = 0; k < it.n_db; ++k) {
+      if (!it.db[k]) return fail(AGNN_EINVAL, "grad_epilogue: item %d: null bias destination %d", i, k);
+      if (reinterpret_cast<uintptr_t>(it.db[k]) & 3u) return fail(AGNN_EALIGN, "grad_epilogue: item %d: bias destination %d is not a float pointer", i, k);
+      spans[n_spans++] = EpiSpan{it.db[k], it.out_f, 1, it.out_f, -1, 0, 0};
+    }
+  }
+  for (int i = 0; i < n_sums; ++i) {
+    const agnn_colsum_item_t& it = sums[i];
+    if (it.n <= 0 || it.H <= 0 || (it.H & 3) || it.H > 2048 || !it.workspace || !it.dgamma || !it.dbeta)
+      return fail(AGNN_EINVAL, "grad_epilogue: column sum %d: bad sizes or null argument", i);
+    if (it.workspace_bytes < static_cast<size_t>(kEpiPartRows) * 2 * it.H * sizeof(float)) return fail(AGNN_ENOMEM, "grad_epilogue: column sum %d: workspace too small", i);
+    if ((reinterpret_cast<uintptr_t>(it.dgamma) | reinterpret_cast<uintptr_t>(it.dbeta) | reinterpret_cast<uintptr_t>(it.workspace)) & 3u)
+      return fail(AGNN_EALIGN, "grad_epilogue: column sum %d: misaligned", i);
+    spans[n_spans++] = EpiSpan{it.dgamma, it.H, 1, it.H, -1, 0, 0};
+    spans[n_spans++] = EpiSpan{it.dbeta, it.H, 1, it.H, -1, 0, 0};
+  }
+  for (int a = 0; a < n_spans; ++a)
+    for (int c = a + 1; c < n_spans; ++c) {
+      const EpiSpan &sa = spans[a], &sc = spans[c];
+      if (sa.item >= 0 && sa.item == sc.item && sa.c0 == sc.c0 && sa.c1 == sc.c1 && sa.p == sc.p && sa.ld == sc.ld) continue;
+      if (spans_overlap(sa, sc)) return fail(AGNN_EINVAL, "grad_epilogue: destinations %d and %d of the call overlap", a, c);
+    }
+  hipStream_t s = static_cast<hipStream_t>(stream_);
+  if (n_items > 0) {
+    WgBatch wb{};
+    wb.n = n_items;
+    int wg = 0;
+    for (int i = 0; i < n_items; ++i) {
+      const agnn_grad_item_t& it = items[i];
+      const int out_pad = bp.tiles_out[i] * 128, in_pad = bp.tiles_in[i] * 128;
+      wb.it[i] = WgArgs{it.dy, it.x, it.ld_dy, it.ld_x, static_cast<int32_t>(it.n), it.out_f, it.in_f, bp.rps[i], bp.tiles_in[i], ws + bp.slab_off[i],
+                        it.n_db > 0 ? ws + bp.slabb_off[i] : nullptr, out_pad, in_pad};
+      wb.tiles[i] = bp.tiles_out[i] * bp.tiles_in[i];
+      wb.first[i] = wg;
+      wg += wb.tiles[i] * bp.S[i];
+    }
+    wb.first[n_items] = wg;
+    hipLaunchKernelGGL(k_wgrad_batch, dim3(static_cast<unsigned>(wg)), dim3(256), 0, s, wb);
+    if (int rc = check_launch("grad_epilogue(products)")) return rc;
+  }
+  int at = 0;
+  do {
+    EpiBatch eb{};
+    int n = 0, n_rec = 0, n_db = 0, blocks = 0;
+    while (at < n_items && n_rec + items[at].n_dw <= kEpiRecMax && n_db + items[at].n_db <= kEpiDbMax) {
+      const agnn_grad_item_t& it = items[at];
+      EpiItem& e = eb.it[n];
+      e.slab = ws + bp.slab_off[at];
+      e.slab_b = it.n_db > 0 ? ws + bp.slabb_off[at] : nullptr;
+      e.S = bp.S[at];
+      e.out_f = it.out_f;
+      e.in_f = it.in_f;
+      e.out_pad = bp.tiles_out[at] * 128;
+      e.in_pad = bp.tiles_in[at] * 128;
+      e.rec0 = static_cast<int16_t>(n_rec);
+      for (int k = 0; k < it.n_dw; ++k) {
+        const agnn_grad_dst_t& d = it.dw[k];
+        eb.rec[n_rec++] = EpiRec{d.p, static_cast<int32_t>(d.ld), d.c0, d.c1, (d.c1 - d.c0) & 1};
+      }
+      e.rec1 = static_cast<int16_t>(n_rec);
+      e.db0 = static_cast<int16_t>(n_db);
+      for (int k = 0; k < it.n_db; ++k) eb.db[n_db++] = it.db[k];
+      e.db1 = static_cast<int16_t>(n_db);
+      eb.first[n] = blocks;
+      int64_t rb = (static_cast<int64_t>(it.out_f) * (it.in_f >> 1) + 31) / 32;
+      if (rb > 1024) rb = 1024;
+      blocks += static_cast<int>(rb);
+      ++n;
+      ++at;
+    }
+    eb.n_items = n;
+    if (at == n_items)
+      for (int i = 0; i < n_sums; ++i) {
+        const agnn_colsum_item_t& it = sums[i];
+        int nb = static_cast<int>((it.n + 3) / 4);
+        if (nb > kEpiPartRows) nb = kEpiPartRows;
+        eb.sum[i] = EpiSum{static_cast<const float*>(it.workspace), it.dgamma, it.dbeta, nb, it.H};
+        eb.first[n++] = blocks;
+        blocks += (2 * it.H + 31) / 32;
+      }
+    eb.first[n] = blocks;
+    eb.n_all = n;
+    if (blocks > 0) {
+      hipLaunchKernelGGL(k_grad_epilogue, dim3(static_cast<unsigned>(blocks)), dim3(256), 0, s, eb);
+      if (int rc = check_launch("grad_epilogue(reduce)")) return rc;
+    }
+  } while (at < n_items);
+  return AGNN_OK;
+}
diff --git a/analysisgnn_amd/dp.py b/analysisgnn_amd/dp.py
--- a/analysisgnn_amd/dp.py
+++ b/analysisgnn_amd/dp.py
@@ -61,6 +61,11 @@
                 seen.add(id(p))
                 params.append(p)
     return params, tight
+
+
+def _grad_in_place() -> bool:
+    from . import linear
+    return bool(linear.GRAD_IN_PLACE)
 
 
 class FlatGradBuffer:
@@ -91,6 +96,15 @@
         self.cut = self.offsets[self.n_early]
         if views:
             self._assign_views()
+        elif dev.type == "cuda":
+            import weakref
+            from . import linear
+            linear.register_grad_slots(self, self.params, self.flat, self.offsets)
+            weakref.finalize(self, linear.unregister_grad_slots, id(self))
+
+    def close(self) -> None:
+        from . import linear
+        linear.unregister_grad_slots(id(self))
 
     def _assign_views(self) -> None:
         for p, k, o in zip(self.params, self.sizes, self.offsets):
@@ -103,6 +117,9 @@
             for p in self.params:
                 p.grad = None
             self._packed = set()
+            if self.flat.is_cuda:
+                from .linear import reset_grad_slots
+                reset_grad_slots(self.params)
 
     def pack(self, part: Optional[str] = None) -> None:
         from .linear import join_wgrad
@@ -116,18 +133,55 @@
             if (part is not None and part != name) or name in done or lo == hi:
                 done.add(name) if lo == hi else None
                 continue
-            parts = []
-            for i in range(lo, hi):
-                p, k, o, o_next = self.params[i], self.sizes[i], self.offsets[i], self.offsets[i + 1]
-                parts.append(p.grad.reshape(-1) if p.grad is not None else self._none[:k])
-                if o_next - o > k:
-                    parts.append(self._pad[: o_next - o - k])
-            torch.cat(parts, out=self.flat[self.offsets[lo]:self.offsets[hi]])
+            if self.flat.is_cuda and _grad_in_place():
+                self._pack_native(lo, hi)
+            else:
+                parts = []
+                for i in range(lo, hi):
+                    p, k, o, o_next = self.params[i], self.sizes[i], self.offsets[i], self.offsets[i + 1]
+                    parts.append(p.grad.reshape(-1) if p.grad is not None else self._none[:k])
+                    if o_next - o > k:
+                        parts.append(self._pad[: o_next - o - k])
+                torch.cat(parts, out=self.flat[self.offsets[lo]:self.offsets[hi]])
             for i in range(lo, hi):
                 p, k, o = self.params[i], self.sizes[i], self.offsets[i]
                 p.grad = self.flat[o:o + k].view_as(p)
             done.add(name)
         self._packed = done
+
+    def _pack_native(self, lo: int, hi: int) -> None:
+        from . import _lib
+        from .linear import reset_grad_slots
+        from .params import pack
+        items = []
+        for i in range(lo, hi):
+            p, k, o, o_next = self.params[i], self.sizes[i], self.offsets[i], self.offsets[i + 1]
+            g = p.grad
+            if o_next - o > k:
+                items.append((self.flat[o + k:o_next].view(1, -1), []))
+            if k == 0:
+                continue
+            slot = self.flat[o:o + k]
+            if g is None:
+                items.append((slot.view(1, -1), []))
+                continue
+            if g.data_ptr() == slot.data_ptr() and g.shape == p.shape and g.is_contiguous():
+                continue
+            if g.dtype != torch.float32 or g.device != self.flat.device:
+                raise ValueError("FlatGradBuffer.pack: fp32 gradients on the buffer's device expected")
+            items.append((slot.view(1, -1), [g.contiguous().view(1, -1)]))
+        if len(items) <= _lib.PACK_MAX_ITEMS:
+            if items:
+                pack(items, self.flat.device)
+        else:
+            arr = (_lib.GatherItem * len(items))()
+            keep = []
+            for a, (dst, srcs) in zip(arr, items):
+                a.dst, a.n = dst.data_ptr(), dst.numel()
+                a.src = srcs[0].data_ptr() if srcs else None
+                keep.extend(srcs)
+            _lib.check(_lib.load().agnn_gather_f32(len(items), arr, _lib.stream_ptr(self.flat.device)), "agnn_gather_f32")
+        reset_grad_slots(self.params[lo:hi])
 
     def all_reduce_mean(self, world: Optional[int] = None) -> None:
         self.pack()
diff --git a/analysisgnn_amd/fused.py b/analysisgnn_amd/fused.py
--- a/analysisgnn_amd/fused.py
+++ b/analysisgnn_amd/fused.py
@@ -8,7 +8,7 @@
 import torch.nn.functional as F
 
 from . import _lib, resident
-from .linear import ColsumItem, all_steal, defer, deferring, leaf_refs
+from .linear import ColsumItem, all_steal, defer, deferring, grad_slot_groups, leaf_refs, slot_group
 
 PRE_RELU, POST_RELU = 1, 2
 ENABLED = True
@@ -30,10 +30,11 @@
 
 class _NormAct(torch.autograd.Function):
     @staticmethod
-    def forward(ctx, x, gamma, beta, eps, p, flags, call_id, seg=0, defer_ok=False, steal_refs=None, pre=None):
+    def forward(ctx, x, gamma, beta, eps, p, flags, call_id, seg=0, defer_ok=False, steal_refs=None, pre=None, slot_groups=None):
         dev = _lib.require_gpu(x, gamma, beta)
         ctx.defer_ok = bool(defer_ok) or (gamma.is_leaf and beta.is_leaf)
         ctx.steal_refs = leaf_refs(gamma, beta) if steal_refs is None else tuple(steal_refs)
+        ctx.slot_groups = (slot_group(gamma), slot_group(beta)) if slot_groups is None else tuple(slot_groups)
         lib = _lib.load()
         x = x if (x.stride(1) == 1 and x.stride(0) % 4 == 0 and x.data_ptr() % 16 == 0) else x.contiguous()
         n, H = x.shape
@@ -63,12 +64,19 @@
         dy = dy if (dy.stride(1) == 1 and dy.stride(0) % 4 == 0 and dy.data_ptr() % 16 == 0) else dy.contiguous()
         n, H = x.shape
         dx = torch.empty_like(x)
-        dgamma = torch.empty_like(gamma)
-        dbeta = torch.empty_like(beta)
         nws = int(lib.agnn_norm_act_workspace_bytes(H))
         ws = torch.empty(nws, dtype=torch.uint8, device=dev)
         rng = used[0] if p > 0 else None
         later = ctx.defer_ok and deferring(dy) and all_steal(ctx.steal_refs)
+        own = None
+        if later and ctx.needs_input_grad[1] and ctx.needs_input_grad[2] and ctx.slot_groups[0] and ctx.slot_groups[1]:
+            own = grad_slot_groups(ctx.slot_groups, (gamma.shape, beta.shape))
+        if own is not None:
+            dgamma, dbeta = own
+            del own
+        else:
+            dgamma = torch.empty_like(gamma)
+            dbeta = torch.empty_like(beta)
         _lib.check(lib.agnn_norm_act_bwd_f32(x.data_ptr(), x.stride(0), gamma.data_ptr(), beta.data_ptr(), seg, n, H, eps, p, flags,
                                              _lib.ptr(rng), call_id, dy.data_ptr(), dy.stride(0), mean.data_ptr(), rstd.data_ptr(),
                                              dx.data_ptr(), dx.stride(0), None if later else dgamma.data_ptr(),
@@ -77,7 +85,7 @@
         if later:
             dg_k, db_k = dgamma.detach(), dbeta.detach()
             defer(ColsumItem(ws, n, H, dg_k, db_k), dev)
-        return dx, dgamma, dbeta, None, None, None, None, None, None, None, None
+        return dx, dgamma, dbeta, None, None, None, None, None, None, None, None, None
 
 
 def _ok16(t: torch.Tensor) -> bool:
@@ -180,7 +188,7 @@
         return F.layer_norm(y, (H,), None, None, eps) * gamma + beta
     view_only = all(t.is_leaf or getattr(t, "_agnn_wgrad_deferrable", False) for t in (gamma, beta))
     y = _NormAct.apply(x.reshape(N, W), gamma.reshape(W), beta.reshape(W), eps, 0.0, PRE_RELU if pre_relu else 0,
-                       next(_CALL_IDS) & 0xFFFFFFFF, H, view_only, leaf_refs(gamma, beta), pre)
+                       next(_CALL_IDS) & 0xFFFFFFFF, H, view_only, leaf_refs(gamma, beta), pre, (slot_group(gamma), slot_group(beta)))
     return y.view(N, G, H)
 
 
diff --git a/analysisgnn_amd/gru.py b/analysisgnn_amd/gru.py
--- a/analysisgnn_amd/gru.py
+++ b/analysisgnn_amd/gru.py
@@ -5,8 +5,8 @@
 import torch.nn.functional as F
 
 from . import _lib, resident
-from .linear import (WgItem, all_steal, defer, defer_home, deferring, leaf_refs, mark_wgrad_async, weight_grad, weight_grad_batch,
-                     wgrad_stream)
+from .linear import (WgItem, all_steal, defer, defer_home, deferring, grad_slot_groups, leaf_refs, mark_wgrad_async, slot_group, weight_grad,
+                     weight_grad_batch, wgrad_stream)
 
 KERNEL_HIDDEN = (64, 128)
 
@@ -59,6 +59,7 @@
         ctx.dims = (B, T, I, Hh)
         ctx.wg_async = all(getattr(t, "_agnn_wgrad_async", False) or t.is_leaf for t in (w_ih, w_hh, b_ih, b_hh))
         ctx.steal_refs = leaf_refs(w_ih, w_hh, b_ih, b_hh)
+        ctx.slot_groups = tuple(slot_group(t) for t in (w_ih, w_hh, b_ih, b_hh))
         return out
 
     @staticmethod
@@ -77,10 +78,19 @@
         dgi2 = dgi.view(B * T, 6 * Hh)
         wf = w_ih.reshape(6 * Hh, I)
         dx = (dgi2 @ wf).view(B, T, I) if ctx.needs_input_grad[0] else None
-        dw_ih = torch.empty((6 * Hh, I), dtype=torch.float32, device=dev)
-        db_ih = torch.empty((6 * Hh,), dtype=torch.float32, device=dev)
-        dw_hh = torch.empty((2, 3 * Hh, Hh), dtype=torch.float32, device=dev)
-        db_hh = torch.empty((2, 3 * Hh), dtype=torch.float32, device=dev)
+        off_chain = ctx.wg_async and all_steal(ctx.steal_refs)
+        own = None
+        if off_chain and I % 2 == 0 and all(ctx.needs_input_grad[1:5]):
+            own = grad_slot_groups(ctx.slot_groups, ((6 * Hh, I), (2, 3 * Hh, Hh), (6 * Hh,), (2, 3 * Hh)),
+                                   lambda v: all(t is not None and t.data_ptr() % 8 == 0 for t in v))
+        if own is not None:
+            dw_ih, dw_hh, db_ih, db_hh = own
+            del own
+        else:
+            dw_ih = torch.empty((6 * Hh, I), dtype=torch.float32, device=dev)
+            db_ih = torch.empty((6 * Hh,), dtype=torch.float32, device=dev)
+            dw_hh = torch.empty((2, 3 * Hh, Hh), dtype=torch.float32, device=dev)
+            db_hh = torch.empty((2, 3 * Hh), dtype=torch.float32, device=dev)
 
         def weight_grads():
             items = []
@@ -94,8 +104,6 @@
             for d in range(2):
                 items.append(WgItem(dgh2[:, d * 3 * Hh:(d + 1) * 3 * Hh], hp2[:, d * Hh:(d + 1) * Hh], True, dw_hh[d], db_hh[d]))
             weight_grad_batch(items)
-
-        off_chain = ctx.wg_async and all_steal(ctx.steal_refs)
 
         def forked():
             with wgrad_stream(dev, dgi, dgh, y, x2, hp, dw_ih, db_ih, dw_hh, db_hh, active=off_chain, kind="sequence"):
diff --git a/analysisgnn_amd/heads.py b/analysisgnn_amd/heads.py
--- a/analysisgnn_amd/heads.py
+++ b/analysisgnn_amd/heads.py
@@ -8,7 +8,7 @@
 
 from . import _lib, resident
 from .fused import grouped_norm_act
-from .linear import all_steal, defer, deferring, leaf_refs, linear, mark_wgrad_async, wgrad_stream
+from .linear import all_steal, defer, deferring, grad_slot_groups, leaf_refs, linear, mark_wgrad_async, slot_group, wgrad_stream
 from .params import cat_rows, stack_rows
 
 
@@ -98,6 +98,7 @@
         ctx._wg_async_in = all(t is None or t.is_leaf or getattr(t, "_agnn_wgrad_async", False) for t in (w, b))
         ctx._wg_defer_in = all(t is None or t.is_leaf or getattr(t, "_agnn_wgrad_deferrable", False) for t in (w, b))
         ctx.steal_refs = leaf_refs(w, b)
+        ctx.slot_groups = (slot_group(w), slot_group(b))
         a = _lib.f32c(a)
         w = _lib.f32c(w)
         if w.data_ptr() % 16:
@@ -131,8 +132,16 @@
         need_w = ctx.needs_input_grad[1] or (has_b and ctx.needs_input_grad[2])
         dw = db = None
         if need_w:
-            dw = torch.empty_like(w)
-            db = torch.empty((sum_c,), dtype=torch.float32, device=dev) if has_b else None
+            off_chain = ctx.wg_async and all_steal(ctx.steal_refs)
+            own = None
+            if off_chain and ctx.needs_input_grad[1] and ctx.needs_input_grad[2] == has_b and ctx.slot_groups[0]:
+                own = grad_slot_groups(ctx.slot_groups, (w.shape, (sum_c,)), lambda v: v[0].data_ptr() % 8 == 0)
+            if own is not None:
+                dw, db = own
+                del own
+            else:
+                dw = torch.empty_like(w)
+                db = torch.empty((sum_c,), dtype=torch.float32, device=dev) if has_b else None
             dw_k, db_k = dw.detach(), (db.detach() if db is not None else None)
 
             def weight_grads():
@@ -141,7 +150,6 @@
                 _lib.check(lib.agnn_gproj_bwd_f32(dout.data_ptr(), dout.stride(0), a.data_ptr(), a.stride(0), w.data_ptr(),
                                                   offs_t.data_ptr(), G, K, tiles, sum_c, N, None, 0, dw_k.data_ptr(), _lib.ptr(db_k),
                                                   ws.data_ptr(), nws, _lib.stream_ptr(dev)), "agnn_gproj_bwd_f32")
-            off_chain = ctx.wg_async and all_steal(ctx.steal_refs)
             if off_chain and ctx.wg_defer and deferring(dout):
                 defer(weight_grads, dev)
             else:
diff --git a/analysisgnn_amd/linear.py b/analysisgnn_amd/linear.py
--- a/analysisgnn_amd/linear.py
+++ b/analysisgnn_amd/linear.py
@@ -161,10 +161,13 @@
                 if t is not None:
                     t.record_stream(here)
     with torch.no_grad():
-        if items:
-            weight_grad_batch(items)
-        if sums:
-            colsum_batch(sums)
+        if GRAD_IN_PLACE and BATCH and (items or sums):
+            grad_epilogue(items, sums)
+        else:
+            if items:
+                weight_grad_batch(items)
+            if sums:
+                colsum_batch(sums)
         for fn in fns:
             if not isinstance(fn, (WgItem, ColsumItem)):
                 fn()
@@ -246,6 +249,94 @@
     _WG.get("join", {}).clear()
 
 
+GRAD_IN_PLACE = True
+_SLOTS = {}
+_HANDED = set()
+
+
+def register_grad_slots(owner, params, flat: torch.Tensor, offsets) -> None:
+    import weakref
+    for p, o in zip(params, offsets):
+        _SLOTS[id(p)] = (id(owner), weakref.ref(p), flat, int(o), p.numel())
+
+
+def unregister_grad_slots(owner_id: int) -> None:
+    for k in [k for k, e in _SLOTS.items() if e[0] == owner_id]:
+        del _SLOTS[k]
+        _HANDED.discard(k)
+
+
+def reset_grad_slots(params=None) -> None:
+    if params is None:
+        _HANDED.clear()
+    else:
+        _HANDED.difference_update(id(p) for p in params)
+
+
+def grad_slot_of(p: torch.Tensor) -> Optional[torch.Tensor]:
+    e = _SLOTS.get(id(p))
+    if e is None or e[1]() is not p:
+        return None
+    return e[2][e[3]:e[3] + e[4]].view_as(p)
+
+
+def grad_slots(leaves, ok=None):
+    if not GRAD_IN_PLACE:
+        return None
+    leaves = list(leaves)
+    ids = [id(p) for p in leaves]
+    if len(set(ids)) != len(ids) or any(i in _HANDED for i in ids):
+        return None
+    views = []
+    for p in leaves:
+        v = grad_slot_of(p) if (p.is_leaf and p.is_cuda and p.grad is None and p.is_contiguous()) else None
+        if v is None:
+            return None
+        views.append(v)
+    if ok is not None and not ok(views):
+        return None
+    _HANDED.update(ids)
+    return views
+
+
+def slot_group(t: Optional[torch.Tensor]):
+    if t is None:
+        return []
+    if t.is_leaf:
+        return [t]
+    members = getattr(t, "_agnn_rowcat", None)
+    return list(members) if members else None
+
+
+def grad_slot_groups(groups, shapes, ok=None):
+    if any(g is None for g in groups):
+        return None
+    from .params import adjacent
+    merged = []
+
+    def build(views):
+        it = iter(views)
+        for g, shape in zip(groups, shapes):
+            vs = [next(it) for _ in g]
+            if not vs:
+                merged.append(None)
+                continue
+            n = 1
+            for d in shape:
+                n *= int(d)
+            if sum(v.numel() for v in vs) != n or (len(vs) > 1 and not adjacent(vs)):
+                return False
+            strides, acc = [], 1
+            for d in reversed(shape):
+                strides.append(acc)
+                acc *= int(d)
+            merged.append(vs[0].as_strided(tuple(int(d) for d in shape), tuple(reversed(strides)), vs[0].storage_offset()))
+        return ok is None or bool(ok(merged))
+    if grad_slots([p for g in groups for p in g], build) is None:
+        return None
+    return merged
+
+
 def _ok(t: torch.Tensor) -> bool:
     return (t.dtype == torch.float32 and t.dim() == 2 and t.stride(1) == 1 and t.stride(0) % 2 == 0
             and t.shape[1] % 2 == 0 and t.data_ptr() % 8 == 0)
@@ -289,17 +380,31 @@
 
 
 class WgItem:
-    __slots__ = ("dy", "x", "want_bias", "dw_out", "db_out", "event", "follows")
-
-    def __init__(self, dy, x, want_bias, dw_out, db_out, follows=False):
+    __slots__ = ("dy", "x", "want_bias", "dw_out", "db_out", "event", "follows", "dsts", "db_dsts")
+
+    def __init__(self, dy, x, want_bias, dw_out, db_out, follows=False, dsts=None, db_dsts=()):
         self.dy, self.x, self.want_bias, self.dw_out, self.db_out, self.event = dy, x, bool(want_bias), dw_out, db_out, None
         self.follows = bool(follows)
+        self.dsts, self.db_dsts = dsts, tuple(db_dsts)
 
     def tensors(self):
+        if self.dsts is not None:
+            return (self.dy, self.x, *[d for _, _, d in self.dsts], *self.db_dsts)
         return (self.dy, self.x, self.dw_out, self.db_out)
 
+    def destinations(self):
+        if self.dsts is not None:
+            return self.dsts, self.db_dsts
+        return [(0, self.x.shape[1], self.dw_out)], ((self.db_out,) if self.want_bias else ())
+
     def __call__(self):
-        weight_grad(self.dy, self.x, self.want_bias, dw_out=self.dw_out, db_out=self.db_out)
+        if self.dsts is None:
+            weight_grad(self.dy, self.x, self.want_bias, dw_out=self.dw_out, db_out=self.db_out)
+            return
+        from .params import pack
+        dw, db = weight_grad(self.dy, self.x, self.want_bias)
+        items = [(d, [dw[:, c0:c1]]) for c0, c1, d in self.dsts] + [(d.view(1, -1), [db.view(1, -1)]) for d in self.db_dsts]
+        pack(items, self.dy.device)
 
 
 class ColsumItem:
@@ -377,6 +482,85 @@
         run(group)
 
 
+def _dst_ok(d: torch.Tensor, out_f: int, c0: int, c1: int) -> bool:
+    cols = c1 - c0
+    if d.dtype != torch.float32 or d.dim() != 2 or tuple(d.shape) != (out_f, cols) or d.stride(1) != 1 or d.stride(0) < cols:
+        return False
+    return d.data_ptr() % 4 == 0 if cols & 1 else (c0 % 2 == 0 and d.stride(0) % 2 == 0 and d.data_ptr() % 8 == 0)
+
+
+def grad_epilogue(items, sums) -> None:
+    lib = _lib.load()
+
+    def fits(it):
+        n, out_f = it.dy.shape
+        in_f = it.x.shape[1]
+        dsts, dbs = it.destinations()
+        return (ENABLED and it.dy.is_cuda and it.dy.dim() == 2 and it.x.dim() == 2 and n >= MIN_ROWS and out_f * in_f <= MAX_OUT_IN and in_f % 2 == 0
+                and _ok(it.dy) and _ok(it.x) and 0 < len(dsts) <= _lib.PACK_MAX_SRC and len(dbs) <= _lib.PACK_MAX_SRC
+                and all(d is not None and _dst_ok(d, out_f, c0, c1) for c0, c1, d in dsts) and bool(dbs) == it.want_bias
+                and all(d is not None and d.is_contiguous() and tuple(d.shape) == (out_f,) for d in dbs)
+                and (it.dsts is not None or all(d.data_ptr() % 8 == 0 for d in dbs)))
+
+    groups, group, products = [], [], 0
+    for it in items:
+        if fits(it):
+            joins = it.follows and group and group[-1].dy is it.dy
+            if group and ((products == _lib.WGRAD_BATCH_MAX and not joins) or len(group) == _lib.WGRAD_BATCH_MAX_ITEMS):
+                groups.append(group)
+                group, products, joins = [], 0, False
+            group.append(it)
+            products += 0 if joins else 1
+        else:
+            it()
+    if group:
+        groups.append(group)
+    sums = list(sums)
+    batched = [g for g in groups if len(g) > 1]
+    for g in groups:
+        if len(g) == 1:
+            g[0]()
+            continue
+        take, sums = (sums[:_lib.GRAD_MAX_SUMS], sums[_lib.GRAD_MAX_SUMS:]) if g is batched[-1] else ([], sums)
+        _epilogue_call(lib, g, take)
+    while sums:
+        _epilogue_call(lib, [], sums[:_lib.GRAD_MAX_SUMS])
+        sums = sums[_lib.GRAD_MAX_SUMS:]
+
+
+def _epilogue_call(lib, group, sums) -> None:
+    dev = (group[0].dy if group else sums[0].ws).device
+    arr = (_lib.GradItem * max(len(group), 1))()
+    for a, it in zip(arr, group):
+        dsts, dbs = it.destinations()
+        a.dy, a.x = it.dy.data_ptr(), it.x.data_ptr()
+        a.ld_dy, a.ld_x, a.n = it.dy.stride(0), it.x.stride(0), it.dy.shape[0]
+        a.out_f, a.in_f = it.dy.shape[1], it.x.shape[1]
+        a.n_dw, a.n_db = len(dsts), len(dbs)
+        for k, (c0, c1, d) in enumerate(dsts):
+            a.dw[k].p, a.dw[k].ld, a.dw[k].c0, a.dw[k].c1 = d.data_ptr(), (d.stride(0) if d.shape[0] > 1 else max(d.shape[1], d.stride(0))), c0, c1
+        for k, d in enumerate(dbs):
+            a.db[k] = d.data_ptr()
+    sarr = (_lib.ColsumItem * max(len(sums), 1))()
+    for a, it in zip(sarr, sums):
+        a.workspace, a.workspace_bytes, a.n, a.H = it.ws.data_ptr(), it.ws.numel(), it.n, it.H
+        a.dgamma, a.dbeta = it.dgamma.data_ptr(), it.dbeta.data_ptr()
+    nws = int(lib.agnn_grad_epilogue_workspace_bytes(len(group), arr)) if group else 0
+    ws = torch.empty(nws, dtype=torch.uint8, device=dev) if group else None
+    _lib.check(lib.agnn_grad_epilogue_f32(len(group), arr, len(sums), sarr, _lib.ptr(ws), nws, _lib.stream_ptr(dev)), "agnn_grad_epilogue_f32")
+
+
+def _leaf_slots(groups, out_f: int, in_f: int, odd_ok: bool = False):
+    if groups is None or not groups[0]:
+        return None
+
+    def ok(v):
+        dw, db = v
+        return (_dw_ok(dw) or (odd_ok and dw.shape[1] & 1 and dw.stride(1) == 1)) and (db is None or db.data_ptr() % 8 == 0)
+    v = grad_slot_groups(groups, ((out_f, in_f), (out_f,)), ok)
+    return None if v is None else (v[0], v[1])
+
+
 HAND_GEMM = True
 HAND_GEMM_DX = False
 HAND_GEMM_MIN_ROWS = 4096
@@ -411,6 +595,11 @@
         ctx.wg_async = _async_ok(w) and _async_ok(b)
         ctx.wg_defer = _deferrable(w) and _deferrable(b)
         ctx.steal_refs = leaf_refs(w, b)
+        ctx.slot_groups = (slot_group(w), slot_group(b))
+        box = getattr(w, "_agnn_grad_box", None)
+        if box is not None:
+            box["uses"] += 1 if ((b is None and not box["b"]) or (b is not None and getattr(b, "_agnn_grad_box", None) is box)) else 2
+        ctx.grad_box = box
         ctx.grad_cols = getattr(x, "_agnn_grad_cols", None) if x.dim() == 2 else None
         ctx.set_materialize_grads(False)
         if pre is not None:
@@ -434,18 +623,49 @@
         in_f = x.shape[1]
         padded = bool(in_f & 1) and x.dim() == 2 and x.stride(1) == 1 and x.stride(0) > in_f
         if want_w and steals and ctx.wg_defer and (in_f % 2 == 0 or padded) and deferring(dy):
-            dw = torch.empty((dy.shape[1], in_f), dtype=torch.float32, device=dy.device)
-            db = torch.empty((dy.shape[1],), dtype=torch.float32, device=dy.device) if want_b else None
-            dw_k, db_k = dw.detach(), (db.detach() if db is not None else None)
-            if padded:
-                dw_wide = torch.empty((dy.shape[1], in_f + 1), dtype=torch.float32, device=dy.device)
-                defer(WgItem(dy, x.as_strided((x.shape[0], in_f + 1), (x.stride(0), 1), x.storage_offset()), want_b, dw_wide, db_k), dy.device, here=True)
-                defer(lambda: dw_k.copy_(dw_wide[:, :in_f]), dy.device)
+            box = ctx.grad_box
+            boxed = None
+            if box is not None and box["uses"] == 1 and not padded and ctx.needs_input_grad[1] and want_b == bool(box["b"]):
+                boxed = grad_slots(box["leaves"], lambda v: all((_dw_ok(t) if t.dim() == 2 else t.is_contiguous()) for t in v))
+            own = None
+            if boxed is None and ctx.needs_input_grad[1] and want_b == ctx.has_bias:
+                own = _leaf_slots(ctx.slot_groups, dy.shape[1], in_f, odd_ok=padded)
+            if boxed is not None:
+                by = {id(p): v.detach() for p, v in zip(box["leaves"], boxed)}
+                box["slots"] = boxed
+                zero = resident.value(dy.device, ("grad_box_zero",), lambda: torch.zeros(1, dtype=torch.float32, device=dy.device), fill=True)
+                dw = zero.expand(dy.shape[1], in_f)
+                db = zero.expand(dy.shape[1]) if want_b else None
+                defer(WgItem(dy, x, want_b, None, None, dsts=[(c0, c1, by[id(p)]) for c0, c1, p in box["w"]],
+                             db_dsts=[by[id(p)] for p in box["b"]]), dy.device)
+                del boxed, by
             else:
-                defer(WgItem(dy, x, want_b, dw_k, db_k), dy.device)
+                if own is not None:
+                    dw, db = own
+                    del own
+                else:
+                    dw = torch.empty((dy.shape[1], in_f), dtype=torch.float32, device=dy.device)
+                    db = torch.empty((dy.shape[1],), dtype=torch.float32, device=dy.device) if want_b else None
+                dw_k, db_k = dw.detach(), (db.detach() if db is not None else None)
+                if padded and GRAD_IN_PLACE and BATCH:
+                    defer(WgItem(dy, x.as_strided((x.shape[0], in_f + 1), (x.stride(0), 1), x.storage_offset()), want_b, None, None,
+                                 dsts=[(0, in_f, dw_k)], db_dsts=([db_k] if want_b else [])), dy.device, here=True)
+                elif padded:
+                    dw_wide = torch.empty((dy.shape[1], in_f + 1), dtype=torch.float32, device=dy.device)
+                    defer(WgItem(dy, x.as_strided((x.shape[0], in_f + 1), (x.stride(0), 1), x.storage_offset()), want_b, dw_wide, db_k), dy.device, here=True)
+                    defer(lambda: dw_k.copy_(dw_wide[:, :in_f]), dy.device)
+                else:
+                    defer(WgItem(dy, x, want_b, dw_k, db_k), dy.device)
         elif want_w:
+            own = None
+            if steals and in_f % 2 == 0 and ctx.needs_input_grad[1] and want_b == ctx.has_bias and dy.is_cuda and dy.dim() == 2:
+                own = _leaf_slots(ctx.slot_groups, dy.shape[1], in_f)
             with wgrad_stream(dy.device, dy, x, active=steals):
-                dw, db = weight_grad(dy, x, want_b)
+                if own is not None:
+                    dw, db = weight_grad(dy, x, want_b, dw_out=own[0], db_out=own[1])
+                    del own
+                else:
+                    dw, db = weight_grad(dy, x, want_b)
         dx = None
         if ctx.needs_input_grad[0]:
             gc = ctx.grad_cols
@@ -504,6 +724,7 @@
         ctx.wg_async = _async_ok(w) and _async_ok(b)
         ctx.wg_defer = _deferrable(w) and _deferrable(b)
         ctx.steal_refs = leaf_refs(w, b)
+        ctx.slot_groups = (slot_group(w), slot_group(b))
         ctx.set_materialize_grads(False)
         return hand_gemm2(x0, x1, w, b)
 
@@ -518,8 +739,13 @@
         want_b = ctx.has_bias and ctx.needs_input_grad[3]
         steals = ctx.wg_async and all_steal(ctx.steal_refs)
         if want_w:
-            dw = torch.empty((dy.shape[1], w.shape[1]), dtype=torch.float32, device=dy.device)
-            db = torch.empty((dy.shape[1],), dtype=torch.float32, device=dy.device) if want_b else None
+            own = _leaf_slots(ctx.slot_groups, dy.shape[1], w.shape[1]) if (steals and ctx.needs_input_grad[2] and want_b == ctx.has_bias and k0 % 2 == 0) else None
+            if own is not None:
+                dw, db = own
+                del own
+            else:
+                dw = torch.empty((dy.shape[1], w.shape[1]), dtype=torch.float32, device=dy.device)
+                db = torch.empty((dy.shape[1],), dtype=torch.float32, device=dy.device) if want_b else None
             dw_k, db_k = dw.detach(), (db.detach() if db is not None else None)
             if steals and ctx.wg_defer and deferring(dy):
                 defer(WgItem(dy, x0, want_b, dw_k[:, :k0], db_k), dy.device)
diff --git a/analysisgnn_amd/params.py b/analysisgnn_amd/params.py
--- a/analysisgnn_amd/params.py
+++ b/analysisgnn_amd/params.py
@@ -33,9 +33,10 @@
 class _SageOperands(torch.autograd.Function):
 
     @staticmethod
-    def forward(ctx, R: int, *params):
+    def forward(ctx, R: int, boxes, *params):
         w_l, b_l, w_r = params[:R], params[R:2 * R], params[2 * R:]
         dev = _lib.require_gpu(*params)
+        ctx.boxes = boxes
         out_f, in_f = w_l[0].shape
         W_l = torch.empty((out_f, R * in_f), dtype=torch.float32, device=dev)
         b = torch.empty((out_f,), dtype=torch.float32, device=dev)
@@ -55,16 +56,30 @@
         R = ctx.R
         out_f, in_f = ctx.shape
         dev = dW_l.device
-        G_l = torch.empty((R, out_f, in_f), dtype=torch.float32, device=dev)
-        G_b = torch.empty((R, out_f), dtype=torch.float32, device=dev)
-        G_r = torch.empty((R, out_f, in_f), dtype=torch.float32, device=dev)
+        sl_l = ctx.boxes[0].pop("slots", None) if ctx.boxes is not None else None
+        sl_r = ctx.boxes[1].pop("slots", None) if ctx.boxes is not None else None
+        if sl_l is not None and sl_r is not None:
+            out = (None, None, *sl_l, *sl_r)
+            del sl_l, sl_r
+            return out
+        G_l = G_b = G_r = None
+        if sl_l is None:
+            G_l = torch.empty((R, out_f, in_f), dtype=torch.float32, device=dev)
+            G_b = torch.empty((R, out_f), dtype=torch.float32, device=dev)
+        if sl_r is None:
+            G_r = torch.empty((R, out_f, in_f), dtype=torch.float32, device=dev)
+
         def fan_out():
-            dW_l_, db_, dW_r_ = _lib.f32c(dW_l), db.contiguous(), _lib.f32c(dW_r)
             items = []
-            for r in range(R):
-                items.append((G_l[r], [dW_l_[:, r * in_f:(r + 1) * in_f]]))
-                items.append((G_b[r].view(1, -1), [db_.view(1, -1)]))
-                items.append((G_r[r], [dW_r_]))
+            if G_l is not None:
+                dW_l_, db_ = _lib.f32c(dW_l), db.contiguous()
+                for r in range(R):
+                    items.append((G_l[r], [dW_l_[:, r * in_f:(r + 1) * in_f]]))
+                    items.append((G_b[r].view(1, -1), [db_.view(1, -1)]))
+            if G_r is not None:
+                dW_r_ = _lib.f32c(dW_r)
+                for r in range(R):
+                    items.append((G_r[r], [dW_r_]))
             pack(items, dev)
         off_chain = ctx.leaves and all_steal(ctx.param_refs)
         if off_chain and deferring(dW_l):
@@ -72,15 +87,19 @@
         else:
             with wgrad_stream(dev, dW_l, db, dW_r, active=off_chain):
                 fan_out()
-        return (None, *G_l.unbind(0), *G_b.unbind(0), *G_r.unbind(0))
+        g_lb = (*G_l.unbind(0), *G_b.unbind(0)) if sl_l is None else tuple(sl_l)
+        g_r = G_r.unbind(0) if sl_r is None else tuple(sl_r)
+        del sl_l, sl_r
+        return (None, None, *g_lb, *g_r)
 
 
 class _SageOperandsCat(torch.autograd.Function):
 
     @staticmethod
-    def forward(ctx, R: int, with_l: bool, *params):
+    def forward(ctx, R: int, with_l: bool, box, *params):
         w_l, b_l, w_r = params[:R], params[R:2 * R], params[2 * R:]
         dev = _lib.require_gpu(*params)
+        ctx.box = box
         out_f, in_f = w_r[0].shape
         nl = R if with_l else 0
         W = torch.empty((out_f, (nl + 1) * in_f), dtype=torch.float32, device=dev)
@@ -100,6 +119,14 @@
         R, nl = ctx.R, ctx.nl
         out_f, in_f = ctx.shape
         dev = dW.device
+        slots = ctx.box.pop("slots", None) if ctx.box is not None else None
+        if slots is not None:
+            by = {id(p): v for p, v in zip(ctx.box["leaves"], slots)}
+            w_l, b_l, w_r = ctx.param_refs[:R], ctx.param_refs[R:2 * R], ctx.param_refs[2 * R:]
+            g_l = [by[id(p)] for p in w_l] if nl else list(torch.zeros((R, out_f, in_f), dtype=torch.float32, device=dev).unbind(0))
+            out = (None, None, None, *g_l, *[by[id(p)] for p in b_l], *[by[id(p)] for p in w_r])
+            del slots, by, g_l
+            return out
         G_l = torch.empty((nl, out_f, in_f), dtype=torch.float32, device=dev)
         G_b = torch.empty((R, out_f), dtype=torch.float32, device=dev)
         G_r = torch.empty((R, out_f, in_f), dtype=torch.float32, device=dev)
@@ -121,7 +148,7 @@
         else:
             with wgrad_stream(dev, dW, db, active=off_chain):
                 fan_out()
-        return (None, None, *G_l.unbind(0), *G_b.unbind(0), *G_r.unbind(0))
+        return (None, None, None, *G_l.unbind(0), *G_b.unbind(0), *G_r.unbind(0))
 
 
 def sage_operands_cat(w_l: List[torch.Tensor], b_l: List[torch.Tensor], w_r: List[torch.Tensor], with_l: bool = True):
@@ -130,10 +157,21 @@
           and all(t.shape == w_l[0].shape and t.is_contiguous() for t in (*w_l, *w_r)))
     if not ok:
         return None
-    ops_ = _SageOperandsCat.apply(R, with_l, *w_l, *b_l, *w_r)
-    if all(t.is_leaf for t in (*w_l, *b_l, *w_r)):
+    leaves_ok = all(t.is_leaf for t in (*w_l, *b_l, *w_r))
+    box = None
+    if leaves_ok:
+        in_f = w_r[0].shape[1]
+        nl = R if with_l else 0
+        box = {"uses": 0, "leaves": (*(w_l if with_l else ()), *b_l, *w_r), "b": tuple(b_l),
+               "w": tuple([(r * in_f, (r + 1) * in_f, w_l[r]) for r in range(nl)] + [(nl * in_f, (nl + 1) * in_f, t) for t in w_r])}
+        if nl + R > _lib.PACK_MAX_SRC:
+            box = None
+    ops_ = _SageOperandsCat.apply(R, with_l, box, *w_l, *b_l, *w_r)
+    if leaves_ok:
         for t in ops_:
             mark_wgrad_async(t, deferrable=True, leaves=(*w_l, *b_l, *w_r))
+            if box is not None:
+                t._agnn_grad_box = box
     return ops_
 
 
@@ -143,10 +181,17 @@
           and all(t.shape == w_l[0].shape and t.is_contiguous() for t in (*w_l, *w_r)))
     if not ok:
         return torch.cat(w_l, dim=1), (sum(b_l) if all(t is not None for t in b_l) else None), sum(w_r)
-    ops_ = _SageOperands.apply(R, *w_l, *b_l, *w_r)
-    if all(t.is_leaf for t in (*w_l, *b_l, *w_r)):
-        for t in ops_:
+    leaves_ok = all(t.is_leaf for t in (*w_l, *b_l, *w_r))
+    boxes = None
+    if leaves_ok:
+        in_f = w_l[0].shape[1]
+        boxes = ({"uses": 0, "leaves": (*w_l, *b_l), "b": tuple(b_l), "w": tuple((r * in_f, (r + 1) * in_f, w_l[r]) for r in range(R))},
+                 {"uses": 0, "leaves": tuple(w_r), "b": (), "w": tuple((0, in_f, t) for t in w_r)})
+    ops_ = _SageOperands.apply(R, boxes, *w_l, *b_l, *w_r)
+    if leaves_ok:
+        for t, box in zip(ops_, (boxes[0], boxes[0], boxes[1])):
             mark_wgrad_async(t, deferrable=True, leaves=(*w_l, *b_l, *w_r))
+            t._agnn_grad_box = box
     return ops_
 
 
@@ -177,13 +222,19 @@
         return tuple(g.split(ctx.rows, dim=0))
 
 
+def _rowcat(t: torch.Tensor, params) -> torch.Tensor:
+    if all(p.is_leaf for p in params):
+        t._agnn_rowcat = tuple(params)
+    return t
+
+
 def cat_rows(params: Sequence[torch.Tensor]) -> torch.Tensor:
     if len(params) > 1 and all(p.shape[1:] == params[0].shape[1:] for p in params) and adjacent(params):
-        return _AdjacentCat.apply(*params)
+        return _rowcat(_AdjacentCat.apply(*params), params)
     return torch.cat(list(params), dim=0)
 
 
 def stack_rows(params: Sequence[torch.Tensor]) -> torch.Tensor:
     if len(params) > 1 and all(p.shape == params[0].shape for p in params) and adjacent(params):
-        return _AdjacentCat.apply(*[p.unsqueeze(0) for p in params])
+        return _rowcat(_AdjacentCat.apply(*[p.unsqueeze(0) for p in params]), params)
     return torch.stack(list(params))
diff --git a/include/agnn.h b/include/agnn.h
--- a/include/agnn.h
+++ b/include/agnn.h
@@ -239,6 +239,33 @@
   int32_t rows, cols, n_src, vec_ok;
 } agnn_pack_item_t;
 int agnn_pack_f32(int32_t n_items, const agnn_pack_item_t* items , agnn_stream_t stream);
+
+#define AGNN_GRAD_MAX_SUMS 16
+typedef struct {
+  float* p;
+  int64_t ld;
+  int32_t c0, c1;
+} agnn_grad_dst_t;
+typedef struct {
+  const float* dy;
+  const float* x;
+  int64_t ld_dy, ld_x, n;
+  int32_t out_f, in_f;
+  int32_t n_dw, n_db;
+  agnn_grad_dst_t dw[AGNN_PACK_MAX_SRC];
+  float* db[AGNN_PACK_MAX_SRC];
+} agnn_grad_item_t;
+size_t agnn_grad_epilogue_workspace_bytes(int32_t n_items, const agnn_grad_item_t* items );
+int agnn_grad_epilogue_f32(int32_t n_items, const agnn_grad_item_t* items , int32_t n_sums,
+                           const agnn_colsum_item_t* sums , void* workspace, size_t workspace_bytes, agnn_stream_t stream);
+
+#define AGNN_GATHER_MAX_ITEMS 128
+typedef struct {
+  float* dst;
+  const float* src;
+  int64_t n;
+} agnn_gather_item_t;
+int agnn_gather_f32(int32_t n_items, const agnn_gather_item_t* items , agnn_stream_t stream);
 
 int agnn_debug_stamp(uint64_t* slot , agnn_stream_t stream);
 
```
